# flash4242/Promptable-Counterfactual-GAN

Hardware: AMD Instinct MI355X
Metric: images/sec (G+D step) MNIST-28 cDCGAN bs512 @1/2/4/8 MI355X; % MFMA roofline (higher is better)
Workload: dtype f32

## Files before the change

include/pcgan_hip.h:

```cpp
#ifndef PCGAN_HIP_H
#define PCGAN_HIP_H

#include <stddef.h>
#include <stdint.h>

#ifdef __cplusplus
extern "C" {
#endif

typedef void* pcg_stream_t;

typedef enum pcg_status {
  PCG_OK = 0,
  PCG_ERR_INVALID = -1,
  PCG_ERR_WORKSPACE = -2,
  PCG_ERR_LAUNCH = -3,
  PCG_ERR_UNSUPPORTED = -4
} pcg_status;

typedef enum pcg_act {
  PCG_ACT_NONE = 0,
  PCG_ACT_RELU = 1,
  PCG_ACT_LRELU = 2,
  PCG_ACT_TANH = 3,
// ... 408 lines not shown
  int32_t B;
  const float* const* w_stored;
  const float* a1; const float* a2; const float* a3; const float* a4;
  float* dx;
} pcg_house_cls_bwd_args;
int pcg_house_classifier_fwd(const pcg_house_cls_fwd_args* args, const pcg_sn_bwd_batch* rider , pcg_stream_t stream);
int pcg_house_classifier_bwd(const pcg_house_cls_bwd_args* args, const pcg_sn_fwd_batch* rider , pcg_stream_t stream);

typedef struct pcg_house_cf_eval_args {
  int64_t N; int32_t T, group, clamp_cls, mask_rows;
  const float* g_flat; int32_t nG;
  const float* bn_mean[10]; const float* bn_var[10];
  float bn_eps, tau, res_scale;
  int32_t col_src[17];
  const float* norm_vals;
  const float* const* c_w_kmajor; const float* const* c_bias;
  const float* x; const int64_t* y;
  const int64_t* target; const float* mask; const float* noise;
  float* cont; float* logits; int32_t* chosen;
  float* masked; float* x_cf; float* x_cf_raw;
  float* logits_cf; float* logits_x;
  int64_t* pred_cf; int64_t* pred_x;
  float* gain;
  float* tile_sums; float* class_sums; float* class_counts;
} pcg_house_cf_eval_args;
int pcg_house_cf_eval(const pcg_house_g_desc* desc, const pcg_house_cf_eval_args* args, pcg_stream_t stream);

enum { PCG_MASK_SHARED = 0,
       PCG_MASK_PER_ROW = 1,
       PCG_MASK_PER_QUERY = 2 };

typedef struct pcg_patch_mask_bits_args {
  const uint64_t* bits;
  float* mask;
  int32_t n, H, W, ps;
} pcg_patch_mask_bits_args;
int pcg_patch_mask_bits(const pcg_patch_mask_bits_args* args, pcg_stream_t stream);

typedef struct pcg_mnist_cf_entry_args {
  const float* x;
  const float* table;
  const float* mask;
  const int64_t* target;
  float* out;
  int32_t B, T, HW, K, mask_mode, q0, nq;
} pcg_mnist_cf_entry_args;
int pcg_mnist_cf_entry(const pcg_mnist_cf_entry_args* args, pcg_stream_t stream);

typedef struct pcg_mnist_cf_tail_args {
  const float* c;
  const float* x;
  const float* mask;
  float* x_cf;
  float* raw; float* masked;
  float* sums;
  float scale;
  int32_t B, T, HW, mask_mode, q0, nq;
} pcg_mnist_cf_tail_args;
int pcg_mnist_cf_tail(const pcg_mnist_cf_tail_args* args, pcg_stream_t stream);

#define PCG_MNIST_CF_GROUP_SUMS 8
typedef struct pcg_mnist_cf_score_args {
  const float* logits_cf;
  const float* logits_orig;
  const int64_t* target;
  const int64_t* y_true;
  const float* tail_sums;
  int64_t* pred; float* conf; float* p_target; float* p_true; float* p_orig_true; float* flip;
  float* group_sums;
  int32_t B, T, K, ld, group_rows, q0, nq;
} pcg_mnist_cf_score_args;
int pcg_mnist_cf_score(const pcg_mnist_cf_score_args* args, pcg_stream_t stream);

int pcg_house_losses(const float* d_real, const float* d_fake, const float* d_fake_g, int64_t n, const float* g_cls, const float* am,
                     const float* pen, float lambda_cls, float w_reg, float lambda_mask, float w_reg_log, float* out5, pcg_stream_t stream);

typedef struct pcg_house_res_fwd_args {
  const float* cont; int32_t ncont;
  const float* samples; const int32_t* seg_dev; int32_t T;
  const float* norm; const float* x; const float* mask;
  const int32_t* col_src;
  int32_t D, B;
  float* res; float* masked; float* x_cf; float* partial512; int32_t* ticket; float* pen_out; float* am_out;
} pcg_house_res_fwd_args;
typedef struct pcg_house_res_bwd_args {
  const float* res; const float* masked; const float* mask; const float* gx_a; const float* gx_b;
  float w_pen, w_am;
  int32_t ncont; const int32_t* cont_idx_dev; const int32_t* seg_dev; int32_t S, T;
  const int32_t* cat_idx_dev; const float* norm;
  int32_t D, B;
  float* dcont; float* dsamples;
} pcg_house_res_bwd_args;
typedef struct pcg_house_loss_args {
  const float* d_real; const float* d_fake; const float* d_fake_g; int32_t n;
  const float* g_cls;
  const float* am; const float* pen;
  float lambda_cls, w_reg, lambda_mask, w_reg_log;
  const float* ce_row_loss;
  int32_t n_ce;
  float* out6;
} pcg_house_loss_args;
typedef struct pcg_house_diag_args {
  const float* logits_cf; const float* logits_orig;
  const int64_t* src_rows;
  const int64_t* target_y; const float* masked;
  int32_t B, nc, D;
  float eps;
  float* out4;
  double* acc;
} pcg_house_diag_args;
int pcg_house_residual_fwd(const pcg_house_res_fwd_args* args, const pcg_sn_fwd_batch* rider , pcg_stream_t stream);
int pcg_house_residual_bwd(const pcg_house_res_bwd_args* args, const pcg_house_loss_args* losses ,
                           const pcg_house_diag_args* diag , pcg_stream_t stream);
int pcg_house_diag(const pcg_house_diag_args* args, pcg_stream_t stream);
int pcg_house_draws(int64_t* target_y, int32_t B, int32_t num_classes, const int64_t* y, uint64_t offset_target, float* mask, int32_t D,
                    const int32_t* zero_cols, int32_t n_zero_cols, uint64_t offset_mask, float* noise, int32_t T, uint64_t offset_noise,
                    uint64_t seed, float* onehot_target, float* onehot_y, pcg_stream_t stream);
int pcg_house_draws_counter(int64_t* target_y, int32_t B, int32_t num_classes, const int64_t* y, float* mask, int32_t D,
                            const int32_t* zero_cols, int32_t n_zero_cols, float* noise, int32_t T, uint64_t seed, float* onehot_target,
                            float* onehot_y, uint64_t* counter, pcg_stream_t stream);
int pcg_house_batch_draws_counter(int64_t* target_y, int32_t B, int32_t num_classes, const float* X, const int64_t* Y,
                                  const int64_t* perm, int64_t n_perm, int64_t n_rows, float* x_out, int64_t* y_out,
                                  int64_t* src_out , float* mask, int32_t D, const int32_t* zero_cols, int32_t n_zero_cols,
                                  float* noise, int32_t T, uint64_t seed, float* onehot_target , float* onehot_y ,
                                  uint64_t* counter, pcg_stream_t stream);

int pcg_dp_barrier(pcg_stream_t stream);
int32_t pcg_dp_rccl_version(void);

#define PCG_DP_UNIQUE_ID_BYTES 128
int pcg_dp_unique_id(void* id_out );
int pcg_dp_init(const void* id , int32_t rank, int32_t world);
int32_t pcg_dp_world(void);
int32_t pcg_dp_rank(void);
pcg_stream_t pcg_dp_side_stream(void);
int pcg_dp_allreduce(float* buf, int64_t n, pcg_stream_t stream);
int pcg_dp_allreduce_begin(float* buf, int64_t n, int32_t slot, pcg_stream_t producer_stream);
int pcg_dp_record(int32_t slot);
int pcg_dp_allreduce_wait(int32_t slot, pcg_stream_t consumer_stream);
int pcg_dp_allreduce_sum_f64(double* buf, int64_t n, pcg_stream_t stream);
int pcg_dp_broadcast(void* buf, int64_t nbytes, int32_t root, pcg_stream_t stream);
int pcg_dp_sync_batchnorm(int32_t enable);
int pcg_dp_shutdown(void);

int pcg_tune_set(const char* name, int32_t value);

int pcg_conv_plan_describe(const pcg_conv_geom* g, int32_t op, int32_t assume_scratch, char* out, size_t out_bytes);
size_t pcg_conv_scratch_parts_bytes(void);
size_t pcg_conv_scratch_arrivals_bytes(void);
int pcg_conv_set_scratch(pcg_stream_t stream, void* parts, size_t parts_bytes, void* arrivals, size_t arrivals_bytes);
int pcg_conv_reset_scratch(pcg_stream_t stream);
size_t pcg_conv_pixtab_bytes(const pcg_conv_geom* g);
int pcg_conv_pixtab_register(const pcg_conv_geom* g, void* host_out, size_t bytes, const void* device_table);
int pcg_debug_stamp_buffer(void* buf, int64_t bytes);

typedef struct pcg_moons_cf_desc {
  int32_t hidden, clf_hidden, B, N;
  int32_t nG, nD, nC, nG_adam, nD_adam;
  int32_t g_off[14], d_off[8], c_off[6];
  double lr_G, lr_D, beta1, beta2, adam_eps;
  float bn_eps, bn_momentum, sn_eps, slope;
  float lambda_cls, lambda_l1, lambda_l2, lambda_mask;
} pcg_moons_cf_desc;

typedef struct pcg_moons_cf_train_args {
  const float* X; const int64_t* Y;
  const int64_t* rows;
  const int64_t* target_y;
  const float* mask;
  float* g_flat; float* d_flat; const float* c_flat;
  float* g_exp_avg; float* g_exp_avg_sq; int64_t* g_step;
  float* d_exp_avg; float* d_exp_avg_sq; int64_t* d_step;
  float* bn_mean[3]; float* bn_var[3]; int64_t* bn_nbt[3];
  float* sn_u[4]; float* sn_v[4];
  float* logs;
  float* scratch; size_t scratch_bytes;
} pcg_moons_cf_train_args;

size_t pcg_moons_cf_scratch_bytes(const pcg_moons_cf_desc* desc, int32_t forward);
int pcg_moons_cf_train_steps(const pcg_moons_cf_desc* desc, const pcg_moons_cf_train_args* args, int32_t n_steps, pcg_stream_t stream);

typedef struct pcg_moons_cf_fwd_args {
  int32_t which, train, B;
  const float* x; const float* onehot; const float* mask;
  float* params;
  float* bn_mean[3]; float* bn_var[3]; int64_t* bn_nbt[3];
  float* sn_u[4]; float* sn_v[4];
  float* out0; float* out1;
  float* scratch; size_t scratch_bytes;
} pcg_moons_cf_fwd_args;
int pcg_moons_cf_forward(const pcg_moons_cf_desc* desc, const pcg_moons_cf_fwd_args* args, pcg_stream_t stream);

typedef struct pcg_moons_cf_eval_args {
  int64_t N; int32_t M, T, group;
  const float* x; const int64_t* y;
  const float* masks;
  const int64_t* target; const float* row_mask;
  const float* g_flat; const float* c_flat;
  const float* bn_mean[3]; const float* bn_var[3];
  float* raw; float* masked; float* x_cf;
  float* logits_cf; float* logits_x;
  int64_t* pred_cf; int64_t* pred_x;
  float* gain;
  float* sums;
} pcg_moons_cf_eval_args;
int pcg_moons_cf_eval(const pcg_moons_cf_desc* desc, const pcg_moons_cf_eval_args* args, pcg_stream_t stream);

typedef struct {
  const float* gamma;
  const float* beta;
  float* running_mean;
  float* running_var;
  int64_t* num_batches_tracked;
  float* save_mean;
  float* save_invstd;
  float* xhat;
  float eps;
  float momentum;
  int32_t training;
} pcg_dense_bn;
typedef struct {
  const float* xhat;
  const float* gamma;
  const float* invstd;
  float* dgamma;
  float* dbeta;
  int32_t accumulate;
} pcg_dense_bn_bwd;
int pcg_dense_rows_fwd(const float* x, const float* W, const float* bias , int32_t R, int32_t I, int32_t O,
                       const pcg_dense_bn* bn , int act, float slope, float* y, pcg_stream_t stream);
int pcg_dense_rows_dgrad(const float* dz, const float* W, int32_t R, int32_t O, int32_t I, int below_act, float below_slope,
                         const float* y_below , const pcg_dense_bn_bwd* bn , float* dx,
                         pcg_stream_t stream);
int pcg_dense_rows_wgrad(const float* dz, const float* x, int32_t R, int32_t O, int32_t I, float* dW, float* db ,
                         int accumulate, pcg_stream_t stream);

typedef struct pcg_moons_gan_desc {
  int32_t hidden, z_dim, label_dim, B, N;
  int32_t nG, nD, nG_adam, nD_adam;
  int32_t g_off[4], d_off[4];
  double lr_G, lr_D, beta1, beta2, adam_eps;
} pcg_moons_gan_desc;

typedef struct pcg_moons_gan_train_args {
  const float* X; const int64_t* Y;
  const int64_t* rows;
  const float* z;
  const int64_t* labels;
  float* g_flat; float* d_flat;
  float* g_exp_avg; float* g_exp_avg_sq; int64_t* g_step;
  float* d_exp_avg; float* d_exp_avg_sq; int64_t* d_step;
  float* logs;
  float* scratch; size_t scratch_bytes;
} pcg_moons_gan_train_args;

size_t pcg_moons_gan_scratch_bytes(const pcg_moons_gan_desc* desc);
int pcg_moons_gan_train_steps(const pcg_moons_gan_desc* desc, const pcg_moons_gan_train_args* args, int32_t n_steps, pcg_stream_t stream);

typedef struct pcg_moons_gan_fwd_args {
  int32_t which; int64_t R;
  const float* x; const float* onehot; const float* params;
  float* out;
} pcg_moons_gan_fwd_args;
int pcg_moons_gan_forward(const pcg_moons_gan_desc* desc, const pcg_moons_gan_fwd_args* args, pcg_stream_t stream);

int32_t pcg_calib_mfma_blocks(int32_t rounds);
size_t pcg_calib_mfma_workspace_bytes(int32_t rounds);
int pcg_calib_mfma(int32_t iters, int32_t rounds, void* workspace, size_t workspace_bytes, double* flop_out ,
                   uint64_t** stamps_out , pcg_stream_t stream);
int pcg_calib_copy(const void* src, void* dst, int64_t nbytes, pcg_stream_t stream);

#ifdef __cplusplus
}
#endif
#endif
```

promptable-counterfactual-gan_amd/_lib.py:

```python
import ctypes
import os

import torch

_HERE = os.path.dirname(os.path.abspath(__file__))
LIB_PATH = os.environ.get("PCG_LIB") or os.path.join(_HERE, "libpcgan_hip.so")

PCG_OK = 0
ACT_NONE, ACT_RELU, ACT_LRELU, ACT_TANH, ACT_SIGMOID = 0, 1, 2, 3, 4


class PcgError(RuntimeError):
    pass


class ConvGeom(ctypes.Structure):

    _fields_ = [(n, ctypes.c_int32) for n in ("B", "IH", "IW", "Cin", "OH", "OW", "Cout", "KH", "KW", "stride", "pad")]

    def key(self):
        return tuple(getattr(self, n) for n, _ in self._fields_)


_I, _P = ctypes.c_int32, ctypes.c_void_p
# ... 45 lines not shown


class MoonsCfFwdArgs(ctypes.Structure):
    _fields_ = ([(n, _I) for n in ("which", "train", "B")] + [(n, _P) for n in ("x", "onehot", "mask", "params")] +
                [("bn_mean", _P * 3), ("bn_var", _P * 3), ("bn_nbt", _P * 3), ("sn_u", _P * 4), ("sn_v", _P * 4)] +
                [("out0", _P), ("out1", _P), ("scratch", _P), ("scratch_bytes", ctypes.c_size_t)])


class MoonsCfEvalArgs(ctypes.Structure):
    _fields_ = ([("N", ctypes.c_int64), ("M", _I), ("T", _I), ("group", _I)] +
                [(n, _P) for n in ("x", "y", "masks", "target", "row_mask", "g_flat", "c_flat")] + [("bn_mean", _P * 3), ("bn_var", _P * 3)] +
                [(n, _P) for n in ("raw", "masked", "x_cf", "logits_cf", "logits_x", "pred_cf", "pred_x", "gain", "sums")])


class HouseCfEvalArgs(ctypes.Structure):
    _fields_ = ([("N", ctypes.c_int64)] + [(n, _I) for n in ("T", "group", "clamp_cls", "mask_rows")] + [("g_flat", _P), ("nG", _I)] +
                [("bn_mean", _P * 10), ("bn_var", _P * 10)] + [(n, ctypes.c_float) for n in ("bn_eps", "tau", "res_scale")] +
                [("col_src", _I * 17), ("norm_vals", _P), ("c_w_kmajor", ctypes.POINTER(ctypes.c_void_p)), ("c_bias", ctypes.POINTER(ctypes.c_void_p))] +
                [(n, _P) for n in ("x", "y", "target", "mask", "noise", "cont", "logits", "chosen", "masked", "x_cf", "x_cf_raw", "logits_cf",
                                   "logits_x", "pred_cf", "pred_x", "gain", "tile_sums", "class_sums", "class_counts")])


class PatchMaskBitsArgs(ctypes.Structure):
    _fields_ = [("bits", _P), ("mask", _P)] + [(n, _I) for n in ("n", "H", "W", "ps")]


class MnistCfEntryArgs(ctypes.Structure):
    _fields_ = [(n, _P) for n in ("x", "table", "mask", "target", "out")] + [(n, _I) for n in ("B", "T", "HW", "K", "mask_mode", "q0", "nq")]


class MnistCfTailArgs(ctypes.Structure):
    _fields_ = ([(n, _P) for n in ("c", "x", "mask", "x_cf", "raw", "masked", "sums")] + [("scale", ctypes.c_float)] +
                [(n, _I) for n in ("B", "T", "HW", "mask_mode", "q0", "nq")])


class MnistCfScoreArgs(ctypes.Structure):
    _fields_ = ([(n, _P) for n in ("logits_cf", "logits_orig", "target", "y_true", "tail_sums", "pred", "conf", "p_target", "p_true",
                                   "p_orig_true", "flip", "group_sums")] + [(n, _I) for n in ("B", "T", "K", "ld", "group_rows", "q0", "nq")])


MASK_SHARED, MASK_PER_ROW, MASK_PER_QUERY = 0, 1, 2
MNIST_CF_GROUP_SUMS = 8


class MoonsGanDesc(ctypes.Structure):
    _fields_ = ([(n, _I) for n in ("hidden", "z_dim", "label_dim", "B", "N", "nG", "nD", "nG_adam", "nD_adam")] +
                [("g_off", _I * 4), ("d_off", _I * 4)] + [(n, ctypes.c_double) for n in ("lr_G", "lr_D", "beta1", "beta2", "adam_eps")])


class MoonsGanTrainArgs(ctypes.Structure):
    _fields_ = ([(n, _P) for n in ("X", "Y", "rows", "z", "labels", "g_flat", "d_flat", "g_exp_avg", "g_exp_avg_sq", "g_step",
                                   "d_exp_avg", "d_exp_avg_sq", "d_step", "logs", "scratch")] + [("scratch_bytes", ctypes.c_size_t)])


class MoonsGanFwdArgs(ctypes.Structure):
    _fields_ = [("which", _I), ("R", ctypes.c_int64)] + [(n, _P) for n in ("x", "onehot", "params", "out")]


class DenseBn(ctypes.Structure):
    _fields_ = ([(n, _P) for n in ("gamma", "beta", "running_mean", "running_var", "num_batches_tracked", "save_mean", "save_invstd", "xhat")] +
                [("eps", ctypes.c_float), ("momentum", ctypes.c_float), ("training", _I)])


class DenseBnBwd(ctypes.Structure):
    _fields_ = [(n, _P) for n in ("xhat", "gamma", "invstd", "dgamma", "dbeta")] + [("accumulate", _I)]


_PP, _PI, _F = ctypes.POINTER(ctypes.c_void_p), ctypes.POINTER(ctypes.c_int32), ctypes.c_float


class SnFwdBatch(ctypes.Structure):
    _fields_ = ([("n", _I), ("reps", _I), ("power_iteration", _I), ("eps", _F), ("w_orig", _PP), ("out_features", _PI), ("in_features", _PI)] +
                [(n, _PP) for n in ("u", "v", "w_bar", "sigma", "u_used", "v_used")])


class SnBwdBatch(ctypes.Structure):
    _fields_ = [("n", _I), ("passes", _I), ("dw_bar", _PP), ("w_bar", _PP), ("out_features", _PI), ("in_features", _PI), ("u", _PP), ("v", _PP),
                ("sigma", _PP), ("dw_orig", _PP), ("accumulate", _PI), ("db_dst", _PP), ("db_src", _PP)]


class HouseCriticFwdArgs(ctypes.Structure):
    _fields_ = ([(n, _I) for n in ("n_pass", "B", "D", "NC")] + [("slope", _F)] +
                [(n, _PP) for n in ("x", "onehot", "w_bar", "bias", "a0", "a1", "a2", "a3", "out")])


class HouseCriticBwdArgs(ctypes.Structure):
    _fields_ = ([(n, _I) for n in ("n_pass", "B", "D")] + [("slope", _F)] +
                [(n, _PP) for n in ("dout", "w_bar", "a1", "a2", "a3", "d3", "d2", "d1", "dx")])


class HouseClsFwdArgs(ctypes.Structure):
    _fields_ = ([("x", _P), ("B", _I), ("w_kmajor", _PP), ("bias", _PP)] + [(n, _P) for n in ("a1", "a2", "a3", "a4", "logits", "ce_target")] +
                [("ce_grad_scale", _F), ("ce_dlogits", _P), ("ce_row_loss", _P)])


class HouseClsBwdArgs(ctypes.Structure):
    _fields_ = [("dlogits", _P), ("B", _I), ("w_stored", _PP)] + [(n, _P) for n in ("a1", "a2", "a3", "a4", "dx")]


class HouseResFwdArgs(ctypes.Structure):
    _fields_ = ([("cont", _P), ("ncont", _I), ("samples", _P), ("seg_dev", _P), ("T", _I), ("norm", _P), ("x", _P), ("mask", _P), ("col_src", _PI),
                 ("D", _I), ("B", _I)] + [(n, _P) for n in ("res", "masked", "x_cf", "partial512", "ticket", "pen_out", "am_out")])


class HouseResBwdArgs(ctypes.Structure):
    _fields_ = ([(n, _P) for n in ("res", "masked", "mask", "gx_a", "gx_b")] + [("w_pen", _F), ("w_am", _F), ("ncont", _I), ("cont_idx_dev", _P),
                ("seg_dev", _P), ("S", _I), ("T", _I), ("cat_idx_dev", _P), ("norm", _P), ("D", _I), ("B", _I), ("dcont", _P), ("dsamples", _P)])


class HouseLossArgs(ctypes.Structure):
    _fields_ = ([("d_real", _P), ("d_fake", _P), ("d_fake_g", _P), ("n", _I), ("g_cls", _P), ("am", _P), ("pen", _P)] +
                [(n, _F) for n in ("lambda_cls", "w_reg", "lambda_mask", "w_reg_log")] + [("ce_row_loss", _P), ("n_ce", _I), ("out6", _P)])


class HouseDiagArgs(ctypes.Structure):
    _fields_ = ([(n, _P) for n in ("logits_cf", "logits_orig", "src_rows", "target_y", "masked")] + [("B", _I), ("nc", _I), ("D", _I), ("eps", _F),
                ("out4", _P), ("acc", _P)])


STRUCTS = {"pcg_conv_geom": ConvGeom, "pcg_in_xform": InXform, "pcg_wgrad_item": WgradItem, "pcg_sn_fwd_batch": SnFwdBatch,
           "pcg_sn_bwd_batch": SnBwdBatch, "pcg_house_g_desc": HouseGDesc, "pcg_house_g_fwd_args": HouseGFwdArgs,
           "pcg_house_g_bwd_args": HouseGBwdArgs, "pcg_house_critic_fwd_args": HouseCriticFwdArgs,
           "pcg_house_critic_bwd_args": HouseCriticBwdArgs, "pcg_house_cls_fwd_args": HouseClsFwdArgs, "pcg_house_cls_bwd_args": HouseClsBwdArgs,
           "pcg_house_res_fwd_args": HouseResFwdArgs, "pcg_house_res_bwd_args": HouseResBwdArgs, "pcg_house_loss_args": HouseLossArgs,
           "pcg_house_diag_args": HouseDiagArgs, "pcg_moons_cf_desc": MoonsCfDesc, "pcg_moons_cf_train_args": MoonsCfTrainArgs,
           "pcg_moons_cf_fwd_args": MoonsCfFwdArgs, "pcg_moons_cf_eval_args": MoonsCfEvalArgs,
           "pcg_house_cf_eval_args": HouseCfEvalArgs, "pcg_patch_mask_bits_args": PatchMaskBitsArgs,
           "pcg_mnist_cf_entry_args": MnistCfEntryArgs, "pcg_mnist_cf_tail_args": MnistCfTailArgs,
           "pcg_mnist_cf_score_args": MnistCfScoreArgs, "pcg_dense_bn": DenseBn,
           "pcg_dense_bn_bwd": DenseBnBwd, "pcg_moons_gan_desc": MoonsGanDesc, "pcg_moons_gan_train_args": MoonsGanTrainArgs,
           "pcg_moons_gan_fwd_args": MoonsGanFwdArgs}

_c = ctypes
_vp, _f, _i, _i64, _sz = _c.c_void_p, _c.c_float, _c.c_int, _c.c_int64, _c.c_size_t
_d = _c.c_double
_i32 = _c.c_int32
_gp = _c.POINTER(ConvGeom)
_xp = _c.POINTER(InXform)

PROTOTYPES = {
    "pcg_abi_version": (_i, []),
    "pcg_abi_struct_bytes": (_sz, [_c.c_char_p]),
    "pcg_last_error": (_c.c_char_p, []),
    "pcg_target_arch": (_c.c_char_p, []),
    "pcg_tune_set": (_i, [_c.c_char_p, _i32]),
    "pcg_debug_stamp_buffer": (_i, [_vp, _i64]),
    "pcg_conv_plan_describe": (_i, [_c.POINTER(ConvGeom), _i32, _i32, _c.c_char_p, _sz]),
    "pcg_conv_scratch_parts_bytes": (_sz, []),
    "pcg_conv_scratch_arrivals_bytes": (_sz, []),
    "pcg_conv_set_scratch": (_i, [_vp, _vp, _sz, _vp, _sz]),
    "pcg_conv_reset_scratch": (_i, [_vp]),
    "pcg_conv_pixtab_bytes": (_sz, [_gp]),
    "pcg_conv_pixtab_register": (_i, [_gp, _vp, _sz, _vp]),
    "pcg_conv2d_fwd_bn_g": (_i, [_gp, _vp, _vp, _vp, _vp, _f, _f, _vp, _vp, _vp, _vp, _vp, _i32, _vp, _sz, _vp]),
    "pcg_bn_apply_act_g": (_i, [_vp, _i64, _i32, _vp, _vp, _vp, _vp, _i, _f, _vp, _i32, _vp]),
    "pcg_conv2d_dgrad_bn_phases": (_i32, [_gp]),
    "pcg_conv2d_dgrad_bnbwd_g": (_i, [_gp, _vp, _vp, _vp, _vp, _vp, _vp, _vp, _i, _f, _vp, _vp, _sz, _i32, _vp]),
    "pcg_bn_bwd_partial_g_workspace_bytes": (_sz, [_i32, _i32]),
    "pcg_bn_bwd_partial_g": (_i, [_vp, _vp, _i64, _i32, _vp, _vp, _vp, _vp, _i32, _i32, _vp, _vp, _vp, _i, _i32, _vp, _sz, _vp]),
    "pcg_bn_act_bwd_g_workspace_bytes": (_sz, [_i64, _i32, _i32]),
    "pcg_bn_act_bwd_premask_g": (_i, [_vp, _vp, _i64, _i32, _vp, _vp, _vp, _vp, _i, _f, _vp, _vp, _vp, _i, _i32, _vp, _sz, _vp]),
    "pcg_bce_pair": (_i, [_vp, _i64, _f, _f, _vp, _vp, _vp, _vp, _vp, _vp]),
    "pcg_conv2d_fwd_bnbwd_thin_ok": (_i32, [_gp]),
    "pcg_conv2d_fwd_bnbwd_thin_workspace_bytes": (_sz, [_gp]),
    "pcg_conv2d_fwd_bnbwd_thin": (_i, [_gp, _vp, _vp, _vp, _vp, _vp, _vp, _vp, _i, _f, _vp, _vp, _vp, _i, _vp, _sz, _vp]),
    "pcg_conv2d_bnin_full_ok": (_i32, [_gp, _i32]),
    "pcg_conv2d_fwd_bnin_full": (_i, [_gp, _vp, _vp, _vp, _vp, _vp, _i, _f, _i32, _vp, _vp, _i, _f, _vp, _vp]),
    "pcg_conv2d_wgrad_bnin_full": (_i, [_gp, _vp, _vp, _vp, _vp, _vp, _i, _f, _i32, _vp, _vp, _i, _vp, _sz, _vp]),
    "pcg_conv_precision_set": (_i, [_i32]),
    "pcg_conv_precision_get": (_i32, []),
    "pcg_slab_defer_begin": (_i, [_vp]),
    "pcg_slab_defer_flush": (_i, [_vp]),
    "pcg_slab_defer_pending": (_i32, []),
    "pcg_conv2d_dgrad_bnbwd_full_ok": (_i32, [_gp, _i32]),
    "pcg_conv2d_dgrad_bnbwd_full_workspace_bytes": (_sz, [_gp, _i32]),
    "pcg_conv2d_dgrad_bnbwd_full": (_i, [_gp, _vp, _vp, _vp, _vp, _vp, _vp, _vp, _i, _f, _vp, _vp, _vp, _i, _i32, _vp, _sz, _vp]),
    "pcg_calib_mfma_blocks": (_i32, [_i32]),
    "pcg_calib_mfma_workspace_bytes": (_sz, [_i32]),
    "pcg_calib_mfma": (_i, [_i32, _i32, _vp, _sz, _c.POINTER(_d), _c.POINTER(_c.c_uint64), _vp]),
    "pcg_calib_copy": (_i, [_vp, _vp, _i64, _vp]),
    "pcg_conv2d_fwd_workspace_bytes": (_sz, [_gp]),
    "pcg_conv2d_dgrad_workspace_bytes": (_sz, [_gp]),
    "pcg_conv2d_fwd": (_i, [_gp, _vp, _vp, _vp, _vp, _vp, _sz, _vp]),
    "pcg_conv2d_dgrad": (_i, [_gp, _vp, _vp, _vp, _vp, _vp, _sz, _vp]),
    "pcg_conv2d_fwd_act": (_i, [_gp, _vp, _vp, _vp, _i, _f, _vp, _vp, _sz, _vp]),
    "pcg_conv2d_dgrad_act": (_i, [_gp, _vp, _vp, _vp, _i, _f, _vp, _vp, _sz, _vp]),
    "pcg_conv2d_fwd_bn_workspace_bytes": (_sz, [_gp]),
    "pcg_conv2d_dgrad_bn_workspace_bytes": (_sz, [_gp]),
    "pcg_conv2d_fwd_bn": (_i, [_gp, _vp, _vp, _vp, _vp, _f, _f, _vp, _vp, _vp, _vp, _vp, _vp, _sz, _vp]),
    "pcg_conv2d_dgrad_bn": (_i, [_gp, _vp, _vp, _vp, _vp, _f, _f, _vp, _vp, _vp, _vp, _vp, _vp, _sz, _vp]),
    "pcg_conv2d_dgrad_mask": (_i, [_gp, _vp, _vp, _vp, _i, _f, _vp, _vp, _sz, _vp]),
    "pcg_conv2d_dgrad_mask_thin_ok": (_i32, [_gp]),
    "pcg_conv2d_xf_thin_ok": (_i32, [_gp]),
    "pcg_conv2d_fwd_add_mask": (_i, [_gp, _vp, _vp, _vp, _vp, _i, _f, _vp, _vp]),
    "pcg_conv2d_dgrad_add_mask": (_i, [_gp, _vp, _vp, _vp, _vp, _i, _f, _vp, _vp]),
    "pcg_conv2d_fwd_mask": (_i, [_gp, _vp, _vp, _vp, _i, _f, _vp, _vp, _sz, _vp]),
    "pcg_conv2d_dgrad_bnbwd": (_i, [_gp, _vp, _vp, _vp, _vp, _vp, _vp, _vp, _i, _f, _vp, _vp, _sz, _vp]),
    "pcg_conv2d_fwd_bnbwd": (_i, [_gp, _vp, _vp, _vp, _vp, _vp, _vp, _vp, _i, _f, _vp, _vp, _sz, _vp]),
    "pcg_conv2d_dgrad_add": (_i, [_gp, _vp, _vp, _vp, _vp, _vp, _sz, _vp]),
    "pcg_conv2d_fwd_bn_partial_rows": (_c.c_int32, [_gp]),
    "pcg_conv2d_dgrad_bn_partial_rows": (_c.c_int32, [_gp]),
    "pcg_bn_bwd_partial_workspace_bytes": (_sz, [_c.c_int32]),
    "pcg_bn_bwd_partial": (_i, [_vp, _vp, _i64, _c.c_int32, _vp, _vp, _vp, _vp, _c.c_int32, _vp, _vp, _vp, _i, _vp, _sz, _vp]),
    "pcg_conv2d_fwd_bn_xf": (_i, [_gp, _vp, _xp, _vp, _vp, _vp, _f, _f, _vp, _vp, _vp, _vp, _vp, _vp, _vp, _vp, _vp, _sz, _vp]),
    "pcg_conv2d_dgrad_bn_xf": (_i, [_gp, _vp, _xp, _vp, _vp, _vp, _f, _f, _vp, _vp, _vp, _vp, _vp, _vp, _vp, _vp, _vp, _sz, _vp]),
    "pcg_conv2d_fwd_xf": (_i, [_gp, _vp, _xp, _vp, _vp, _i, _f, _vp, _vp, _sz, _vp]),
    "pcg_conv2d_dgrad_xf": (_i, [_gp, _vp, _xp, _vp, _vp, _i, _f, _vp, _vp, _sz, _vp]),
    "pcg_conv2d_wgrad_xf": (_i, [_gp, _vp, _xp, _vp, _xp, _vp, _i, _vp, _sz, _vp]),
    "pcg_bn_train_stats_coef": (_i, [_vp, _i64, _c.c_int32, _f, _f, _vp, _vp, _vp, _vp, _vp, _vp, _vp, _vp, _vp, _sz, _vp]),
    "pcg_bn_db_workspace_bytes": (_sz, [_i64, _c.c_int32]),
    "pcg_bn_act_bwd_db": (_i, [_vp, _vp, _vp, _i64, _c.c_int32, _vp, _vp, _vp, _vp, _i, _f, _f, _vp, _vp, _vp, _i, _vp, _i, _vp, _sz, _vp]),
    "pcg_bn_bwd_partial_db_workspace_bytes": (_sz, [_c.c_int32]),
    "pcg_bn_bwd_partial_db": (_i, [_vp, _vp, _i64, _c.c_int32, _vp, _vp, _vp, _vp, _c.c_int32, _f, _vp, _vp, _vp, _i, _vp, _i, _vp, _sz, _vp]),
    "pcg_conv2d_dgrad_add_bnsum": (_i, [_gp, _vp, _vp, _vp, _vp, _vp, _vp, _f, _vp, _vp, _sz, _vp]),
    "pcg_conv2d_fwd_add": (_i, [_gp, _vp, _vp, _vp, _vp, _vp, _sz, _vp]),
    "pcg_conv2d_fwd_add_bnsum": (_i, [_gp, _vp, _vp, _vp, _vp, _vp, _vp, _f, _vp, _vp, _sz, _vp]),
    "pcg_conv_weight_adjoint": (_i, [_vp, _vp, _i32, _i32, _i32, _i32, _vp]),
    "pcg_conv_weight_adjoint_many": (_i, [_vp, _vp, _i32, _i32, _i32, _i32, _i32, _vp]),
    "pcg_house_losses": (_i, [_vp, _vp, _vp, _i64, _vp, _vp, _vp, _f, _f, _f, _f, _vp, _vp]),
    "pcg_dp_unique_id": (_i, [_vp]),
    "pcg_dp_init": (_i, [_vp, _i32, _i32]),
    "pcg_dp_world": (_i32, []),
    "pcg_dp_rank": (_i32, []),
    "pcg_dp_side_stream": (_vp, []),
    "pcg_dp_allreduce": (_i, [_vp, _i64, _vp]),
    "pcg_dp_allreduce_begin": (_i, [_vp, _i64, _i32, _vp]),
    "pcg_dp_record": (_i, [_i32]),
    "pcg_dp_allreduce_wait": (_i, [_i32, _vp]),
    "pcg_dp_allreduce_sum_f64": (_i, [_vp, _i64, _vp]),
    "pcg_dp_broadcast": (_i, [_vp, _i64, _i32, _vp]),
    "pcg_dp_sync_batchnorm": (_i, [_i32]),
    "pcg_dp_barrier": (_i, [_vp]),
    "pcg_dp_rccl_version": (_i32, []),
    "pcg_dp_shutdown": (_i, []),
    "pcg_conv2d_wgrad_workspace_bytes": (_sz, [_gp]),
    "pcg_conv2d_wgrad": (_i, [_gp, _vp, _vp, _vp, _i, _vp, _sz, _vp]),
    "pcg_colsum_workspace_bytes": (_sz, [_i64, _c.c_int32]),
    "pcg_colsum": (_i, [_vp, _i64, _c.c_int32, _vp, _i, _vp, _sz, _vp]),
    "pcg_bn_workspace_bytes": (_sz, [_i64, _c.c_int32]),
    "pcg_bn_train_stats": (_i, [_vp, _i64, _c.c_int32, _f, _f, _vp, _vp, _vp, _vp, _vp, _vp, _sz, _vp]),
    "pcg_bn_apply_act": (_i, [_vp, _i64, _c.c_int32, _vp, _vp, _f, _vp, _vp, _i, _f, _vp, _f, _vp, _vp]),
    "pcg_bn_act_bwd": (_i, [_vp, _vp, _vp, _i64, _c.c_int32, _vp, _vp, _vp, _i, _f, _f, _vp, _vp, _vp, _i, _vp, _sz, _vp]),
    "pcg_bn_act_bwd_premask": (_i, [_vp, _vp, _i64, _c.c_int32, _vp, _vp, _vp, _vp, _i, _f, _f, _vp, _vp, _vp, _i, _vp, _sz, _vp]),
    "pcg_embed_concat_fwd": (_i, [_vp, _vp, _vp, _vp, _vp, _c.c_int32, _c.c_int32, _c.c_int32, _c.c_int32, _vp]),
    "pcg_embed_concat_bwd": (_i, [_vp, _vp, _vp, _vp, _c.c_int32, _c.c_int32, _c.c_int32, _c.c_int32, _i, _vp]),
    "pcg_embed_table_grad": (_i, [_vp, _vp, _vp, _i32, _i32, _i32, _i32, _i32, _i, _vp]),
    "pcg_gather_channel": (_i, [_vp, _vp, _i32, _i32, _i32, _vp]),
    "pcg_axpby": (_i, [_vp, _f, _vp, _f, _vp, _i64, _vp]),
    "pcg_scale_mask_fwd": (_i, [_vp, _vp, _f, _vp, _vp, _i64, _vp]),
    "pcg_scale_mask_bwd": (_i, [_vp, _vp, _vp, _f, _vp, _i64, _vp]),
    "pcg_clamp_add_fwd": (_i, [_vp, _vp, _f, _f, _vp, _i64, _vp]),
    "pcg_clamp_add_bwd": (_i, [_vp, _vp, _vp, _f, _f, _vp, _i64, _vp]),
    "pcg_abs_mean_workspace_bytes": (_sz, []),
    "pcg_abs_mean_fwd": (_i, [_vp, _vp, _i, _i64, _vp, _vp, _sz, _vp]),
    "pcg_abs_mean_bwd": (_i, [_vp, _vp, _i, _i64, _vp, _f, _vp, _i, _vp]),
    "pcg_avgpool_fwd": (_i, [_vp, _vp, _c.c_int32, _c.c_int32, _c.c_int32, _vp]),
    "pcg_avgpool_bwd": (_i, [_vp, _vp, _c.c_int32, _c.c_int32, _c.c_int32, _vp]),
    "pcg_cross_entropy_fwd_bwd": (_i, [_vp, _vp, _c.c_int32, _c.c_int32, _f, _vp, _vp, _vp, _vp]),
    "pcg_act_fwd": (_i, [_vp, _i64, _i, _f, _vp, _vp]),
    "pcg_act_bwd": (_i, [_vp, _vp, _i64, _i, _f, _vp, _vp]),
    "pcg_bce_fwd_bwd": (_i, [_vp, _vp, _f, _i64, _f, _vp, _vp, _vp, _vp]),
    "pcg_bce_logits_fwd_bwd": (_i, [_vp, _f, _i64, _f, _vp, _vp, _vp, _vp]),
    "pcg_adam_step": (_i, [_vp, _vp, _vp, _vp, _i64, _d, _d, _d, _d, _d, _i, _i64, _vp]),
    "pcg_adam_step_capturable": (_i, [_vp, _vp, _vp, _vp, _i64, _d, _d, _d, _d, _d, _i, _vp, _vp, _vp]),
    "pcg_patch_mask": (_i, [_vp, _c.c_int32, _c.c_int32, _c.c_int32, _c.c_int32, _c.c_int32, _c.c_uint64, _c.c_uint64, _vp]),
    "pcg_randint": (_i, [_vp, _i64, _c.c_int32, _c.c_int32, _vp, _c.c_uint64, _c.c_uint64, _vp]),
    "pcg_randn": (_i, [_vp, _i64, _f, _f, _c.c_uint64, _c.c_uint64, _vp]),
    "pcg_fill": (_i, [_vp, _i64, _f, _vp]),
    "pcg_add_bias_rows": (_i, [_vp, _i64, _i32, _vp, _vp]),
    "pcg_sumsq": (_i, [_vp, _i64, _vp, _i, _vp]),
    "pcg_norm_sum": (_i, [_vp, _vp, _i32, _vp, _vp]),
    "pcg_instnorm_fwd": (_i, [_vp, _i32, _i32, _i32, _vp, _vp, _f, _i, _f, _vp, _vp, _vp, _vp]),
    "pcg_instnorm_bwd": (_i, [_vp, _vp, _i32, _i32, _i32, _vp, _vp, _vp, _vp, _vp, _vp, _vp]),
    "pcg_instnorm_bwd_bwd": (_i, [_vp, _vp, _vp, _i32, _i32, _i32, _vp, _vp, _vp, _vp, _vp, _vp, _vp]),
    "pcg_instnorm_bwd_fused": (_i, [_vp, _vp, _f, _vp, _i32, _i32, _i32, _vp, _vp, _vp, _vp, _vp, _vp, _vp, _vp, _vp, _vp]),
    "pcg_instnorm_bwd_bwd_act": (_i, [_vp, _vp, _vp, _i32, _i32, _i32, _vp, _vp, _vp, _vp, _f, _vp, _vp, _vp, _vp]),
    "pcg_rowsum3": (_i, [_i32, _vp, _vp, _i, _vp, _vp, _i, _vp, _vp, _i, _i32, _i32, _vp]),
    "pcg_nhwc_to_nchw_flat": (_i, [_vp, _vp, _i32, _i32, _i32, _i, _vp]),
    "pcg_interpolate": (_i, [_vp, _vp, _vp, _vp, _i32, _i32, _vp]),
    "pcg_interpolate_stack": (_i, [_vp, _vp, _vp, _vp, _i32, _i32, _vp]),
    "pcg_gradient_penalty_fwd": (_i, [_vp, _i32, _i32, _f, _vp, _vp, _vp]),
    "pcg_gradient_penalty_bwd": (_i, [_vp, _vp, _vp, _i32, _i32, _f, _vp, _vp]),
    "pcg_rand_uniform": (_i, [_vp, _i64, _c.c_uint64, _c.c_uint64, _vp]),
    "pcg_cross_entropy_weighted_fwd_bwd": (_i, [_vp, _vp, _vp, _i32, _i32, _f, _vp, _vp, _vp, _vp]),
    "pcg_dropout_apply": (_i, [_vp, _vp, _i64, _i32, _i32, _f, _vp, _vp]),
    "pcg_rand_bernoulli": (_i, [_vp, _i64, _f, _c.c_uint64, _c.c_uint64, _vp]),
    "pcg_resize8_normalize": (_i, [_vp, _i32, _i32, _i32, _i32, _i32, _vp, _vp, _i32, _vp, _vp, _i32, _f, _f, _vp, _vp]),
    "pcg_house_g_fwd": (_i, [_c.POINTER(HouseGDesc), _c.POINTER(HouseGFwdArgs), _vp]),
    "pcg_house_g_bwd": (_i, [_c.POINTER(HouseGDesc), _c.POINTER(HouseGBwdArgs), _vp]),
    "pcg_weighted_sum_fwd": (_i, [_i32, _vp, _vp, _vp, _vp]),
    "pcg_weighted_sum_bwd": (_i, [_i32, _vp, _vp, _vp, _vp]),
    "pcg_cf_metrics": (_i, [_vp, _vp, _vp, _vp, _i32, _i32, _vp, _vp]),
    "pcg_gemm": (_i, [_i, _i, _i32, _i32, _i32, _vp, _i32, _vp, _i32, _vp, _i32, _vp, _i, _vp]),
    "pcg_linear_wgrad_workspace_bytes": (_sz, [_i32, _i32, _i32]),
    "pcg_linear_wgrad_ticket_count": (_i32, []),
    "pcg_linear_wgrad": (_i, [_vp, _i32, _vp, _i32, _i32, _i32, _i32, _vp, _vp, _i, _i, _vp, _sz, _vp, _vp]),
    "pcg_spectral_norm_fwd_batched": (_i, [_c.POINTER(SnFwdBatch), _vp]),
    "pcg_spectral_norm_bwd_batched": (_i, [_c.POINTER(SnBwdBatch), _vp]),
    "pcg_house_critic_fwd": (_i, [_c.POINTER(HouseCriticFwdArgs), _vp]),
    "pcg_house_critic_bwd": (_i, [_c.POINTER(HouseCriticBwdArgs), _vp]),
    "pcg_house_classifier_fwd": (_i, [_c.POINTER(HouseClsFwdArgs), _c.POINTER(SnBwdBatch), _vp]),
    "pcg_house_classifier_bwd": (_i, [_c.POINTER(HouseClsBwdArgs), _c.POINTER(SnFwdBatch), _vp]),
    "pcg_house_cf_eval": (_i, [_c.POINTER(HouseGDesc), _c.POINTER(HouseCfEvalArgs), _vp]),
    "pcg_patch_mask_bits": (_i, [_c.POINTER(PatchMaskBitsArgs), _vp]),
    "pcg_mnist_cf_entry": (_i, [_c.POINTER(MnistCfEntryArgs), _vp]),
    "pcg_mnist_cf_tail": (_i, [_c.POINTER(MnistCfTailArgs), _vp]),
# ... 75 lines not shown
```

promptable-counterfactual-gan_amd/csrc/conv_igemm.hip:

```cpp
#include <string.h>
#include <mutex>
#include "conv_loaders.h"
#include "conv_pixtab.h"
#include "thin_conv.h"

namespace pcg {
namespace {

__device__ __forceinline__ int wave_id() { return __builtin_amdgcn_readfirstlane((int)(threadIdx.x >> 6)); }

__device__ __forceinline__ void prio_entry(const ConvP& p) { if (p.edge_prio & 1) __builtin_amdgcn_s_setprio(3); }
__device__ __forceinline__ void prio_epilogue(const ConvP& p) { if (p.edge_prio & 2) __builtin_amdgcn_s_setprio(3); }

__device__ __forceinline__ int epi_group_off(const ConvP& p, int m_block) {
  return p.epi.group_rows > 0 ? __builtin_amdgcn_readfirstlane(m_block / p.epi.group_rows) * p.N : 0;
}

template <class Cfg, bool XF>
__global__ void __launch_bounds__(IG_THREADS, Cfg::MINW) conv_fwd_kernel(ConvP p) {
  extern __shared__ __attribute__((aligned(16))) float smem[];
  prio_entry(p);
  const uint32_t tile = xcd_remap(blockIdx.x, gridDim.x);
  const int mt = tile / p.tilesN, nt = tile % p.tilesN;
  const int m_block = mt * Cfg::BM, n_block = nt * Cfg::BN;
  const int kt_begin = blockIdx.y * p.ktiles_per_split;
  int ktiles = p.ktiles - kt_begin;
  if (ktiles > p.ktiles_per_split) ktiles = p.ktiles_per_split;

  if (wave_id() >= 4) {
    const int tid = threadIdx.x - IG_LOADERS;
    FwdALoader<Cfg::BM, XF> la(p, m_block, tid);
    FwdBLoader<Cfg::BN> lb(p, n_block, tid);
    if (kt_begin) { la.seek(kt_begin); lb.seek(kt_begin); }
    igemm_produce<Cfg>(la, lb, ktiles, smem, tid, ClockStamp{p.stamps, p.stamp_slots});
    return;
  }
  f32x16 acc[Cfg::TM][Cfg::TN];
  ClockStamp cs{p.stamps, p.stamp_slots};
  cs.phase(0);
  igemm_consume<Cfg, true, true>(ktiles, acc, smem, cs);
  prio_epilogue(p);
  float* out = p.out + (size_t)blockIdx.y * (size_t)p.M * (size_t)p.N;
#ifdef PCG_ABL_NO_EPILOGUE
  if (acc[0][0][0] == 12345.678f) out[0] = acc[0][0][1];
  return;
#endif
  igemm_store_tile<Cfg>(acc, smem, n_block, p.N, blockIdx.y == 0 ? p.bias : nullptr, [&](int row) -> float* {
    const int m = m_block + row;
    return m < p.M ? out + (size_t)m * p.N + n_block : nullptr;
  }, p.stat_partial ? p.stat_partial + (size_t)mt * Cfg::WAVES_M * 2 * p.N : nullptr, p.act, p.slope, &p.epi, epi_group_off(p, m_block));
  cs.phase(3);
}

template <class Cfg, bool XF>
__global__ void __launch_bounds__(IG_THREADS, Cfg::MINW) conv_dgrad_kernel(ConvP p, DgradPhases phases) {
  extern __shared__ __attribute__((aligned(16))) float smem[];
  __shared__ int rowpix[Cfg::BM];
  prio_entry(p);
  uint32_t bx = blockIdx.x, py = blockIdx.y;
  if (phases.interleave) {
    const uint32_t l = xcd_remap(blockIdx.x, gridDim.x);
    py = l % (uint32_t)phases.interleave; bx = l / (uint32_t)phases.interleave;
  }
  const PhaseInfo& f = phases.p[py];
  const int tilesM = (f.Mp + Cfg::BM - 1) / Cfg::BM;
  const uint32_t ntiles = (uint32_t)tilesM * p.tilesN;
  if (bx >= ntiles) return;
  const uint32_t tile = phases.interleave ? bx : xcd_remap(bx, ntiles);
  const int mt = tile / p.tilesN, nt = tile % p.tilesN;
  const int m_block = mt * Cfg::BM, n_block = nt * Cfg::BN;
  const int ktiles = f.nth * f.ntw * ((p.Cout + IG_BK - 1) / IG_BK);

  if (wave_id() >= 4) {
    const int tid = threadIdx.x - IG_LOADERS;
    for (int r = tid; r < Cfg::BM; r += IG_LOADERS) {
      const int m = m_block + r;
      int pix = -1;
      if (m < f.Mp) {
        uint32_t t, cc, b, aa;
        f.dPHw.divmod((uint32_t)m, t, cc);
        f.dPHh.divmod(t, b, aa);
        pix = ((int)b * p.IH + (int)aa * p.stride + f.ph) * p.IW + (int)cc * p.stride + f.pw;
      }
      rowpix[r] = pix;
    }
    DgradALoader<Cfg::BM, XF> la(p, f, m_block, tid);
    DgradBLoader<Cfg::BN> lb(p, f, n_block, tid);
    igemm_produce<Cfg>(la, lb, ktiles, smem, tid, ClockStamp{p.stamps, p.stamp_slots});
    return;
  }
  f32x16 acc[Cfg::TM][Cfg::TN];
  ClockStamp cs{p.stamps, p.stamp_slots};
  cs.phase(0);
  igemm_consume<Cfg, true, false>(ktiles, acc, smem, cs);
  prio_epilogue(p);
  igemm_store_tile<Cfg>(acc, smem, n_block, p.N, p.bias, [&](int row) -> float* {
    const int pix = rowpix[row];
    return pix >= 0 ? p.out + (size_t)pix * p.Cin + n_block : nullptr;
  }, p.stat_partial ? p.stat_partial + (size_t)(f.prow0 + mt * Cfg::WAVES_M) * 2 * p.N : nullptr, p.act, p.slope, &p.epi, epi_group_off(p, m_block));
  cs.phase(3);
}

struct SkPlan {
  int dp_tiles, sk_tiles, sk_blocks, ktiles;
  float* parts;
  int* arrivals;
};
struct SkSeg { int tile, kt_begin, nkt, nparts, first_block; };

__device__ __forceinline__ int sk_start(int g, const SkPlan& sk) {
  return __builtin_amdgcn_readfirstlane((int)((uint32_t)g * (uint32_t)(sk.sk_tiles * sk.ktiles) / (uint32_t)sk.sk_blocks));
}
__device__ __forceinline__ int sk_owner(int x, const SkPlan& sk) {
  return __builtin_amdgcn_readfirstlane((int)((((uint32_t)x + 1u) * (uint32_t)sk.sk_blocks - 1u) / (uint32_t)(sk.sk_tiles * sk.ktiles)));
}
__device__ __forceinline__ int sk_segments(const SkPlan& sk, SkSeg& s0, SkSeg& s1) {
  const int b = blockIdx.x;
  if (b < sk.dp_tiles) { s0 = SkSeg{(int)xcd_remap((uint32_t)b, (uint32_t)sk.dp_tiles), 0, sk.ktiles, 1, 0}; return 1; }
  const int g = (int)xcd_remap((uint32_t)(b - sk.dp_tiles), (uint32_t)sk.sk_blocks), KT = sk.ktiles;
  const int it0 = sk_start(g, sk), it1 = sk_start(g + 1, sk);
  const int j0 = __builtin_amdgcn_readfirstlane(it0 / KT), e0 = it1 < (j0 + 1) * KT ? it1 : (j0 + 1) * KT;
  auto fill = [&](SkSeg& sg, int j, int from, int to) {
    const int f = sk_owner(j * KT, sk), l = sk_owner((j + 1) * KT - 1, sk);
    sg = SkSeg{sk.dp_tiles + j, from - j * KT, to - from, l - f + 1, f};
  };
  fill(s0, j0, it0, e0);
  if (it1 <= e0) return 1;
  fill(s1, j0 + 1, e0, it1);
  return 2;
}
#if defined(__HIP_DEVICE_COMPILE__) && !defined(__gfx950__)
#error "stream-K partial-tile exchange (sc1 stores + relaxed agent-scope counters) is written for gfx950 only"
#endif
__device__ __forceinline__ void sk_store4(rsrc_t r, uint32_t off, float a, float b, float c, float d) {
  const u32x4 v = {__float_as_uint(a), __float_as_uint(b), __float_as_uint(c), __float_as_uint(d)};
  __builtin_amdgcn_raw_buffer_store_b128(v, r, off, 0, 16);
}
__device__ __forceinline__ float4 sk_load4(rsrc_t r, uint32_t off) {
  const u32x4 v = __builtin_amdgcn_raw_buffer_load_b128(r, off, 0, 16);
  return make_float4(__uint_as_float(v.x), __uint_as_float(v.y), __uint_as_float(v.z), __uint_as_float(v.w));
}
template <class Cfg, class FirstOf>
__device__ __forceinline__ bool sk_combine_core(float* parts, int* arrivals, int nblocks, int g, int j, int nparts, int first_block,
                                                FirstOf first_of, f32x16 (&acc)[Cfg::TM][Cfg::TN]) {
  if (nparts == 1) return true;
  constexpr uint32_t TILE_BYTES = Cfg::BM * Cfg::BN * 4;
  auto slot_of = [&](int blk) { return (uint32_t)(2 * blk + (first_of(blk) ? 0 : 1)); };
  const rsrc_t rs = make_rsrc(parts, (uint32_t)(2 * nblocks) * TILE_BYTES);
  const uint32_t toff = threadIdx.x * 16u;
  const uint32_t mine = slot_of(g) * TILE_BYTES + toff;
#pragma unroll
  for (int i = 0; i < Cfg::TM; ++i)
#pragma unroll
    for (int jj = 0; jj < Cfg::TN; ++jj)
#pragma unroll
      for (int q = 0; q < 4; ++q)
        sk_store4(rs, mine + (uint32_t)(((i * Cfg::TN + jj) * 4 + q) * IG_LOADERS * 16),
                  acc[i][jj][4 * q], acc[i][jj][4 * q + 1], acc[i][jj][4 * q + 2], acc[i][jj][4 * q + 3]);
  asm volatile("s_waitcnt vmcnt(0)" ::: "memory");
  int* cnt = arrivals + j * 4 + (int)(threadIdx.x >> 6);
  int old = 0;
  if ((threadIdx.x & 63) == 0) old = __hip_atomic_fetch_add(cnt, 1, __ATOMIC_RELAXED, __HIP_MEMORY_SCOPE_AGENT);
  old = __builtin_amdgcn_readfirstlane(old);
  if (old != nparts - 1) return false;
  if ((threadIdx.x & 63) == 0) __hip_atomic_store(cnt, 0, __ATOMIC_RELAXED, __HIP_MEMORY_SCOPE_AGENT);
#pragma unroll
  for (int i = 0; i < Cfg::TM; ++i)
#pragma unroll
    for (int jj = 0; jj < Cfg::TN; ++jj)
#pragma unroll
      for (int r = 0; r < 16; ++r) acc[i][jj][r] = 0.f;
  for (int k = 0; k < nparts; ++k) {
    const uint32_t src = slot_of(first_block + k) * TILE_BYTES + toff;
#pragma unroll
    for (int i = 0; i < Cfg::TM; ++i)
#pragma unroll
      for (int jj = 0; jj < Cfg::TN; ++jj)
#pragma unroll
        for (int q = 0; q < 4; ++q) {
          const float4 v = sk_load4(rs, src + (uint32_t)(((i * Cfg::TN + jj) * 4 + q) * IG_LOADERS * 16));
          acc[i][jj][4 * q] += v.x; acc[i][jj][4 * q + 1] += v.y; acc[i][jj][4 * q + 2] += v.z; acc[i][jj][4 * q + 3] += v.w;
        }
  }
  return true;
}
template <class Cfg>
__device__ __forceinline__ bool sk_combine(const SkPlan& sk, const SkSeg& sg, f32x16 (&acc)[Cfg::TM][Cfg::TN]) {
  const int g = (int)xcd_remap((uint32_t)((int)blockIdx.x - sk.dp_tiles), (uint32_t)sk.sk_blocks), j = sg.tile - sk.dp_tiles, KT = sk.ktiles;
  return sk_combine_core<Cfg>(sk.parts, sk.arrivals, sk.sk_blocks, g, j, sg.nparts, sg.first_block,
                              [&](int blk) { return sk_start(blk, sk) >= j * KT; }, acc);
}

template <class Cfg, bool XF>
__device__ __forceinline__ void fwd_sk_segment(const ConvP& p, const SkPlan& sk, const SkSeg& sg, float* smem) {
  const int mt = __builtin_amdgcn_readfirstlane(sg.tile / p.tilesN), nt = sg.tile - mt * p.tilesN;
  const int m_block = mt * Cfg::BM, n_block = nt * Cfg::BN;
  if (wave_id() >= 4) {
    const int tid = threadIdx.x - IG_LOADERS;
    FwdALoader<Cfg::BM, XF> la(p, m_block, tid);
    FwdBLoader<Cfg::BN> lb(p, n_block, tid);
    if (sg.kt_begin) { la.seek(sg.kt_begin); lb.seek(sg.kt_begin); }
    igemm_produce<Cfg>(la, lb, sg.nkt, smem, tid, ClockStamp{nullptr, 0});
    return;
  }
  f32x16 acc[Cfg::TM][Cfg::TN];
  igemm_consume<Cfg, true, true>(sg.nkt, acc, smem);
  if (sk_combine<Cfg>(sk, sg, acc))
    igemm_store_tile<Cfg>(acc, smem, n_block, p.N, p.bias, [&](int row) -> float* {
      const int m = m_block + row;
      return m < p.M ? p.out + (size_t)m * p.N + n_block : nullptr;
    }, p.stat_partial ? p.stat_partial + (size_t)mt * Cfg::WAVES_M * 2 * p.N : nullptr, p.act, p.slope, &p.epi, epi_group_off(p, m_block));
}
template <class Cfg, bool XF>
__global__ void __launch_bounds__(IG_THREADS, Cfg::MINW) conv_fwd_sk_kernel(ConvP p, SkPlan sk) {
  extern __shared__ __attribute__((aligned(16))) float smem[];
  SkSeg s0, s1{};
  const int nseg = sk_segments(sk, s0, s1);
  fwd_sk_segment<Cfg, XF>(p, sk, s0, smem);
  if (nseg == 1) return;
  lds_barrier();
  fwd_sk_segment<Cfg, XF>(p, sk, s1, smem);
}

template <class Cfg, bool XF>
__device__ __forceinline__ void dgrad_sk_segment(const ConvP& p, const DgradPhases& phases, const SkPlan& sk, const SkSeg& sg, int tiles_per_phase,
                                                 float* smem, int* rowpix) {
  const int py = __builtin_amdgcn_readfirstlane(sg.tile / tiles_per_phase), tile = sg.tile - py * tiles_per_phase;
  const PhaseInfo& f = phases.p[py];
  const int mt = __builtin_amdgcn_readfirstlane(tile / p.tilesN), nt = tile - mt * p.tilesN;
  const int m_block = mt * Cfg::BM, n_block = nt * Cfg::BN;
  if (wave_id() >= 4) {
    const int tid = threadIdx.x - IG_LOADERS;
    for (int r = tid; r < Cfg::BM; r += IG_LOADERS) {
      const int m = m_block + r;
      int pix = -1;
      if (m < f.Mp) {
        uint32_t t, cc, b, aa;
        f.dPHw.divmod((uint32_t)m, t, cc);
        f.dPHh.divmod(t, b, aa);
        pix = ((int)b * p.IH + (int)aa * p.stride + f.ph) * p.IW + (int)cc * p.stride + f.pw;
      }
      rowpix[r] = pix;
    }
    DgradALoader<Cfg::BM, XF> la(p, f, m_block, tid);
    DgradBLoader<Cfg::BN> lb(p, f, n_block, tid);
    if (sg.kt_begin) { la.seek(sg.kt_begin); lb.seek(sg.kt_begin); }
    igemm_produce<Cfg>(la, lb, sg.nkt, smem, tid, ClockStamp{nullptr, 0});
    return;
  }
  f32x16 acc[Cfg::TM][Cfg::TN];
  igemm_consume<Cfg, true, false>(sg.nkt, acc, smem);
  if (sk_combine<Cfg>(sk, sg, acc))
    igemm_store_tile<Cfg>(acc, smem, n_block, p.N, p.bias, [&](int row) -> float* {
      const int pix = rowpix[row];
      return pix >= 0 ? p.out + (size_t)pix * p.Cin + n_block : nullptr;
    }, p.stat_partial ? p.stat_partial + (size_t)(f.prow0 + mt * Cfg::WAVES_M) * 2 * p.N : nullptr, p.act, p.slope, &p.epi, epi_group_off(p, m_block));
}
template <class Cfg, bool XF>
__global__ void __launch_bounds__(IG_THREADS, Cfg::MINW) conv_dgrad_sk_kernel(ConvP p, DgradPhases phases, SkPlan sk, int tiles_per_phase) {
  extern __shared__ __attribute__((aligned(16))) float smem[];
  __shared__ int rowpix[Cfg::BM];
  SkSeg s0, s1{};
  const int nseg = sk_segments(sk, s0, s1);
  dgrad_sk_segment<Cfg, XF>(p, phases, sk, s0, tiles_per_phase, smem, rowpix);
  if (nseg == 1) return;
  lds_barrier();
  dgrad_sk_segment<Cfg, XF>(p, phases, sk, s1, tiles_per_phase, smem, rowpix);
}

template <class Cfg, bool XFA, bool XFB, bool TAB = false>
__global__ void __launch_bounds__(IG_THREADS, 4) conv_wgrad_kernel(ConvP p, int ktiles_total, int ktiles_per_split, int tiles,
                                                                   int slice_major) {
  extern __shared__ __attribute__((aligned(16))) float smem[];
  prio_entry(p);
  uint32_t tile, split;
  if (slice_major) {
    const uint32_t l = xcd_remap(blockIdx.x, gridDim.x);
    split = l / (uint32_t)tiles; tile = l - split * (uint32_t)tiles;
  } else {
    tile = xcd_remap(blockIdx.x, gridDim.x); split = blockIdx.y;
  }
  const int mt = tile / p.tilesN, nt = tile % p.tilesN;
  const int m_block = mt * Cfg::BM, n_block = nt * Cfg::BN;
  const int kt_begin = split * ktiles_per_split;
  int ktiles = ktiles_total - kt_begin;
  if (ktiles > ktiles_per_split) ktiles = ktiles_per_split;

  if (wave_id() >= 4) {
    const int tid = threadIdx.x - IG_LOADERS;
    WgradALoader<Cfg::BM, XFA> la(p, m_block, kt_begin, tid);
    WgradBLoader<Cfg::BN, XFB, TAB> lb(p, n_block, kt_begin, tid);
    igemm_produce<Cfg>(la, lb, ktiles, smem, tid, ClockStamp{p.stamps, p.stamp_slots});
    return;
  }
  f32x16 acc[Cfg::TM][Cfg::TN];
  igemm_consume<Cfg, false, false>(ktiles, acc, smem, ClockStamp{p.stamps, p.stamp_slots});
  prio_epilogue(p);
  float* slab = p.out + (size_t)split * (size_t)p.M * (size_t)p.N;
  igemm_store_tile<Cfg>(acc, smem, n_block, p.N, nullptr, [&](int row) -> float* {
    const int m = m_block + row;
    return m < p.M ? slab + (size_t)m * p.N + n_block : nullptr;
  });
}


struct SkNPlan {
  int nph, blocks, total;
  int tile0[5], it0[5], kt[4];
  float* parts; int* arrivals;
};
__device__ __forceinline__ int skn_start(int g, const SkNPlan& sk) {
  return __builtin_amdgcn_readfirstlane((int)((uint32_t)g * (uint32_t)sk.total / (uint32_t)sk.blocks));
}
__device__ __forceinline__ int skn_owner(int x, const SkNPlan& sk) {
  return __builtin_amdgcn_readfirstlane((int)((((uint32_t)x + 1u) * (uint32_t)sk.blocks - 1u) / (uint32_t)sk.total));
}
struct SkNSeg { int py, tin, t_begin, e, kt_begin, nkt, fb, nparts, mt, nt; };
__device__ __forceinline__ SkNSeg skn_segment(int it, int it1, const SkNPlan& sk, int tilesN) {
  SkNSeg s;
  s.py = 0;
  if (sk.nph > 1 && it >= sk.it0[1]) s.py = 1;
  if (sk.nph > 2 && it >= sk.it0[2]) s.py = 2;
  if (sk.nph > 3 && it >= sk.it0[3]) s.py = 3;
  const int KT = sk.kt[s.py], local = it - sk.it0[s.py];
  s.tin = __builtin_amdgcn_readfirstlane(local / KT);
  s.t_begin = sk.it0[s.py] + s.tin * KT;
  const int t_end = s.t_begin + KT;
  s.e = it1 < t_end ? it1 : t_end;
  s.kt_begin = it - s.t_begin; s.nkt = s.e - it;
  s.fb = skn_owner(s.t_begin, sk); s.nparts = skn_owner(t_end - 1, sk) - s.fb + 1;
  s.mt = __builtin_amdgcn_readfirstlane(s.tin / tilesN); s.nt = s.tin - s.mt * tilesN;
  return s;
}
template <class Cfg, bool XF>
__global__ void __launch_bounds__(IG_THREADS, Cfg::MINW) conv_dgrad_skn_kernel(ConvP p, DgradPhases phases, SkNPlan sk) {
  extern __shared__ __attribute__((aligned(16))) float smem[];
  __shared__ int rowpix[Cfg::BM];
  const int g = (int)xcd_remap(blockIdx.x, (uint32_t)sk.blocks);
  const int it1 = skn_start(g + 1, sk);
  if (wave_id() >= 4) {
    const int tid = threadIdx.x - IG_LOADERS;
#pragma unroll 1
    for (int it = skn_start(g, sk); it < it1;) {
      const SkNSeg sg = skn_segment(it, it1, sk, p.tilesN);
      const PhaseInfo& f = phases.p[sg.py];
      const int m_block = sg.mt * Cfg::BM, n_block = sg.nt * Cfg::BN;
      for (int r = tid; r < Cfg::BM; r += IG_LOADERS) {
        const int m = m_block + r;
        int pix = -1;
        if (m < f.Mp) {
          uint32_t t, cc, b, aa;
          f.dPHw.divmod((uint32_t)m, t, cc);
          f.dPHh.divmod(t, b, aa);
          pix = ((int)b * p.IH + (int)aa * p.stride + f.ph) * p.IW + (int)cc * p.stride + f.pw;
        }
        rowpix[r] = pix;
      }
      DgradALoader<Cfg::BM, XF> la(p, f, m_block, tid);
      DgradBLoader<Cfg::BN> lb(p, f, n_block, tid);
      if (sg.kt_begin) { la.seek(sg.kt_begin); lb.seek(sg.kt_begin); }
      igemm_produce<Cfg>(la, lb, sg.nkt, smem, tid, ClockStamp{nullptr, 0});
      it = sg.e;
      if (it < it1) lds_barrier();
    }
    return;
  }
#pragma unroll 1
  for (int it = skn_start(g, sk); it < it1;) {
    const SkNSeg sg = skn_segment(it, it1, sk, p.tilesN);
    const PhaseInfo& f = phases.p[sg.py];
    const int m_block = sg.mt * Cfg::BM, n_block = sg.nt * Cfg::BN;
    {
      f32x16 acc[Cfg::TM][Cfg::TN];
      igemm_consume<Cfg, true, false>(sg.nkt, acc, smem);
      const int t_begin = sg.t_begin;
      if (sk_combine_core<Cfg>(sk.parts, sk.arrivals, sk.blocks, g, sk.tile0[sg.py] + sg.tin, sg.nparts, sg.fb,
                               [&](int blk) { return skn_start(blk, sk) >= t_begin; }, acc))
        igemm_store_tile<Cfg>(acc, smem, n_block, p.N, p.bias, [&](int row) -> float* {
          const int pix = rowpix[row];
          return pix >= 0 ? p.out + (size_t)pix * p.Cin + n_block : nullptr;
        }, p.stat_partial ? p.stat_partial + (size_t)(f.prow0 + sg.mt * Cfg::WAVES_M) * 2 * p.N : nullptr, p.act, p.slope, &p.epi, epi_group_off(p, m_block));
    }
    it = sg.e;
    if (it < it1) lds_barrier();
  }
}

template <class Cfg, bool XFA, bool XFB, bool TAB>
__device__ __forceinline__ void wgrad_sk_segment(const ConvP& p, const SkPlan& sk, const SkSeg& sg, float* smem) {
  const int mt = __builtin_amdgcn_readfirstlane(sg.tile / p.tilesN), nt = sg.tile - mt * p.tilesN;
  const int m_block = mt * Cfg::BM, n_block = nt * Cfg::BN;
  if (wave_id() >= 4) {
    const int tid = threadIdx.x - IG_LOADERS;
    WgradALoader<Cfg::BM, XFA> la(p, m_block, sg.kt_begin, tid);
    WgradBLoader<Cfg::BN, XFB, TAB> lb(p, n_block, sg.kt_begin, tid);
    igemm_produce<Cfg>(la, lb, sg.nkt, smem, tid, ClockStamp{nullptr, 0});
    return;
  }
  f32x16 acc[Cfg::TM][Cfg::TN];
  igemm_consume<Cfg, false, false>(sg.nkt, acc, smem);
  if (sk_combine<Cfg>(sk, sg, acc))
    igemm_store_tile<Cfg>(acc, smem, n_block, p.N, nullptr, [&](int row) -> float* {
      const int m = m_block + row;
      return m < p.M ? p.out + (size_t)m * p.N + n_block : nullptr;
    }, nullptr, PCG_ACT_NONE, 0.f, &p.epi);
}
template <class Cfg, bool XFA, bool XFB, bool TAB = false>
__global__ void __launch_bounds__(IG_THREADS, 4) conv_wgrad_sk_kernel(ConvP p, SkPlan sk) {
  extern __shared__ __attribute__((aligned(16))) float smem[];
  SkSeg s0, s1{};
  const int nseg = sk_segments(sk, s0, s1);
  wgrad_sk_segment<Cfg, XFA, XFB, TAB>(p, sk, s0, smem);
  if (nseg == 1) return;
  lds_barrier();
  wgrad_sk_segment<Cfg, XFA, XFB, TAB>(p, sk, s1, smem);
}

using Cfg64x192 = TileCfg<64, 192, 2, 2>;
template <class Cfg, bool TAB = false>
__global__ void __launch_bounds__(IG_THREADS, 4) conv_wgrad192_kernel(ConvP p, int ktiles_total, int ktiles_per_split, int tiles,
                                                                      int slice_major) {
  static_assert(Cfg::BM == 64 && Cfg::BN == 192, "the 192-column weight-gradient tile");
  extern __shared__ __attribute__((aligned(16))) float smem[];
  prio_entry(p);
  uint32_t tile, split;
  if (slice_major) {
    const uint32_t l = xcd_remap(blockIdx.x, gridDim.x);
    split = l / (uint32_t)tiles; tile = l - split * (uint32_t)tiles;
  } else {
    tile = xcd_remap(blockIdx.x, gridDim.x); split = blockIdx.y;
  }
  const int mt = tile / p.tilesN, nt = tile % p.tilesN;
  const int m_block = mt * Cfg::BM, n_block = nt * Cfg::BN;
  const int kt_begin = split * ktiles_per_split;
  int ktiles = ktiles_total - kt_begin;
  if (ktiles > ktiles_per_split) ktiles = ktiles_per_split;
  if (wave_id() >= 4) {
    const int tid = threadIdx.x - IG_LOADERS;
    WgradALoader<Cfg::BM, false> la(p, m_block, kt_begin, tid);
    WgradBLoader192<TAB> lb(p, n_block, kt_begin, tid);
    igemm_produce<Cfg>(la, lb, ktiles, smem, tid);
    return;
  }
  f32x16 acc[Cfg::TM][Cfg::TN];
  igemm_consume<Cfg, false, false>(ktiles, acc, smem, ClockStamp{p.stamps, p.stamp_slots});
  prio_epilogue(p);
  float* slab = p.out + (size_t)split * (size_t)p.M * (size_t)p.N;
  igemm_store_tile<Cfg>(acc, smem, n_block, p.N, nullptr, [&](int row) -> float* {
    const int m = m_block + row;
    return m < p.M ? slab + (size_t)m * p.N + n_block : nullptr;
  });
}

__global__ void __launch_bounds__(256) col2im_kernel(const float4* __restrict__ dcol, float4* __restrict__ dx, const float* __restrict__ bias,
                                                     int B, int IH, int IW, int CQ, int OH, int OW, int KH, int KW, int stride, int pad,
                                                     FastDiv dCQ, FastDiv dIW, FastDiv dIH, int act, float neg) {
  const uint32_t total = (uint32_t)B * IH * IW * CQ;
  for (uint32_t idx = blockIdx.x * 256u + threadIdx.x; idx < total; idx += gridDim.x * 256u) {
    uint32_t pix, cq, t, iw, b, ih;
    dCQ.divmod(idx, pix, cq);
    dIW.divmod(pix, t, iw);
    dIH.divmod(t, b, ih);
    float4 acc = bias ? *reinterpret_cast<const float4*>(bias + 4 * cq) : make_float4(0.f, 0.f, 0.f, 0.f);
    for (int kh = 0; kh < KH; ++kh) {
      const int th = (int)ih + pad - kh;
      if (th < 0 || th % stride) continue;
      const int oh = th / stride;
      if (oh >= OH) continue;
      for (int kw = 0; kw < KW; ++kw) {
        const int tw = (int)iw + pad - kw;
        if (tw < 0 || tw % stride) continue;
        const int ow = tw / stride;
        if (ow >= OW) continue;
        const float4 v = dcol[((size_t)(((int)b * OH + oh) * OW + ow) * (KH * KW) + (kh * KW + kw)) * CQ + cq];
        acc.x += v.x; acc.y += v.y; acc.z += v.z; acc.w += v.w;
      }
    }
    if (act != PCG_ACT_NONE) {
      acc.x = act_neg_scale(acc.x, neg); acc.y = act_neg_scale(acc.y, neg); acc.z = act_neg_scale(acc.z, neg); acc.w = act_neg_scale(acc.w, neg);
    }
    dx[idx] = acc;
  }
}

using Cfg128x128 = TileCfg<128, 128, 2, 2>;
#ifndef PCG_TILE64_SWZ
#define PCG_TILE64_SWZ 1
#endif
using Cfg128x64P = TileCfg<128, 64, 2, 2>;
#if PCG_TILE64_SWZ
using Cfg128x64 = TileCfg<128, 64, 2, 2, true, 6, 1>;
#else
using Cfg128x64 = Cfg128x64P;
#endif

template <class C>
using Bf16Twin = TileCfg<C::BM, C::BN, C::WAVES_M, C::WAVES_N, false, C::MINW, C::PF, true>;


int check_geom(const pcg_conv_geom* g) {
  PCG_REQUIRE(g != nullptr, "conv geometry is null");
  PCG_REQUIRE(g->B > 0 && g->IH > 0 && g->IW > 0 && g->Cin > 0 && g->OH > 0 && g->OW > 0 && g->Cout > 0,
              "conv geometry: non-positive extent");
  PCG_REQUIRE(g->KH > 0 && g->KW > 0 && g->stride > 0 && g->pad >= 0, "conv geometry: bad kernel/stride/pad");
  PCG_REQUIRE(g->OH == (g->IH + 2 * g->pad - g->KH) / g->stride + 1 && g->OW == (g->IW + 2 * g->pad - g->KW) / g->stride + 1,
              "conv geometry: OH/OW inconsistent with IH/IW, kernel %dx%d stride %d pad %d", g->KH, g->KW, g->stride, g->pad);
  PCG_REQUIRE((int64_t)g->B * g->IH * g->IW * g->Cin * 4 < (1ll << 31) && (int64_t)g->B * g->OH * g->OW * g->Cout * 4 < (1ll << 31) &&
                  (int64_t)g->Cout * g->KH * g->KW * g->Cin * 4 < (1ll << 31),
              "conv geometry: an operand tensor reaches 2 GiB (32-bit buffer offsets); split the batch");
  PCG_REQUIRE(g->KH * g->KW <= 32, "conv geometry: more than 32 taps (%dx%d) unsupported", g->KH, g->KW);
  return PCG_OK;
}

struct Tune { int edge_prio = -1, dgrad_swz3 = -1, wgrad_rounds = -1, korder = -1, wgrad_order = -1, dgrad_interleave = -1, fwd_splits = -1, stream_k = -1, sk_blocks = -1, dgrad_gemm = -1, t64 = -1, wgrad_pixtab = -1; unsigned long long* stamps = nullptr; int stamp_slots = 0; };
Tune g_tune;

ConvP make_params(const pcg_conv_geom* g) {
  ConvP p{};
  static const int korder_env = getenv("PCG_KORDER") ? atoi(getenv("PCG_KORDER")) : 1;
  p.korder = g_tune.korder >= 0 ? g_tune.korder : korder_env;
  static const int edge_env = getenv("PCG_EDGE_PRIO") ? atoi(getenv("PCG_EDGE_PRIO")) : 2;
  p.edge_prio = g_tune.edge_prio >= 0 ? g_tune.edge_prio : edge_env;
  p.stamps = g_tune.stamps; p.stamp_slots = g_tune.stamp_slots;
  p.B = g->B; p.IH = g->IH; p.IW = g->IW; p.Cin = g->Cin; p.OH = g->OH; p.OW = g->OW; p.Cout = g->Cout;
  p.KH = g->KH; p.KW = g->KW; p.stride = g->stride; p.pad = g->pad;
  p.dOW = FastDiv((uint32_t)g->OW);
  p.dOH = FastDiv((uint32_t)g->OH);
  p.dOHW = FastDiv((uint32_t)(g->OH * g->OW));
  p.x_bytes = (uint32_t)((int64_t)g->B * g->IH * g->IW * g->Cin * 4);
  p.dy_bytes = (uint32_t)((int64_t)g->B * g->OH * g->OW * g->Cout * 4);
  p.w_bytes = (uint32_t)((int64_t)g->Cout * g->KH * g->KW * g->Cin * 4);
  return p;
}

int set_xform(const char* who, const pcg_in_xform* xf, int C, ConvP* p) {
  if (!xf || !xf->scale) return PCG_OK;
  PCG_REQUIRE(xf->shift != nullptr, "%s: input transform without shift", who);
  PCG_REQUIRE(xf->act == PCG_ACT_NONE || xf->act == PCG_ACT_RELU || xf->act == PCG_ACT_LRELU,
              "%s: input transform activation %d is not none / ReLU / LeakyReLU", who, xf->act);
  PCG_REQUIRE(C % 4 == 0 && (((uintptr_t)xf->scale | (uintptr_t)xf->shift) & 15) == 0,
              "%s: input transform needs a channel count %% 4 == 0 and 16-byte aligned scale / shift", who);
  p->in_sc = xf->scale; p->in_sh = xf->shift; p->in_neg = act_neg_of(xf->act, xf->slope); p->in_c_bytes = (uint32_t)C * 4u;
  return PCG_OK;
}

template <class Cfg, bool AK, bool BK_>
constexpr size_t smem_bytes() {
  constexpr int a = igemm_smem_floats<Cfg, AK, BK_>(), b = epilogue_smem_floats<Cfg>();
  return sizeof(float) * (size_t)(a > b ? a : b);
}

template <class K>
int set_smem(K kernel, size_t bytes) {
  hipError_t e = hipFuncSetAttribute(reinterpret_cast<const void*>(kernel), hipFuncAttributeMaxDynamicSharedMemorySize, (int)bytes);
  if (e != hipSuccess) { set_error("hipFuncSetAttribute(max dynamic LDS=%zu): %s", bytes, hipGetErrorString(e)); return PCG_ERR_LAUNCH; }
  return PCG_OK;
}

constexpr int SK_MAX_BLOCKS = 512, SK_MAX_TILES = 4096;
constexpr size_t SK_PARTS_BYTES = (size_t)2 * SK_MAX_BLOCKS * 128 * 128 * sizeof(float);
constexpr size_t SK_ARRIVALS_BYTES = (size_t)SK_MAX_TILES * 4 * sizeof(int);
struct SkScratch { int device; hipStream_t stream; float* parts; int* arrivals; };
SkScratch g_sk_scratch[64];
int g_sk_scratch_n = 0;
std::mutex g_sk_mutex;
int current_device() { int d = 0; return hipGetDevice(&d) == hipSuccess ? d : 0; }
bool sk_scratch_of(hipStream_t s, SkPlan* sk) {
  const int dev = current_device();
  std::lock_guard<std::mutex> lock(g_sk_mutex);
  for (int i = 0; i < g_sk_scratch_n; ++i)
    if (g_sk_scratch[i].stream == s && g_sk_scratch[i].device == dev) {
      if (sk) { sk->parts = g_sk_scratch[i].parts; sk->arrivals = g_sk_scratch[i].arrivals; }
      return true;
    }
  return false;
}
struct PixTabReg { int device, IH, IW, OH, OW, stride, pad, KH, KW, Cin; const uint32_t* tab; };
constexpr int PIXTAB_MAX = 256;
PixTabReg g_pixtab[PIXTAB_MAX];
int g_pixtab_n = 0;
std::mutex g_pixtab_mutex;
bool pixtab_same(const PixTabReg& r, int dev, const pcg_conv_geom* g) {
  return r.device == dev && r.IH == g->IH && r.IW == g->IW && r.OH == g->OH && r.OW == g->OW && r.stride == g->stride && r.pad == g->pad &&
         r.KH == g->KH && r.KW == g->KW && r.Cin == g->Cin;
}
const uint32_t* pixtab_of(const pcg_conv_geom* g) {
  static const int env = getenv("PCG_WGRAD_PIXTAB") ? atoi(getenv("PCG_WGRAD_PIXTAB")) : 1;
  if (!(g_tune.wgrad_pixtab >= 0 ? g_tune.wgrad_pixtab : env)) return nullptr;
  std::lock_guard<std::mutex> lock(g_pixtab_mutex);
  if (g_pixtab_n == 0) return nullptr;
  const int dev = current_device();
  for (int i = 0; i < g_pixtab_n; ++i)
    if (pixtab_same(g_pixtab[i], dev, g)) return g_pixtab[i].tab;
  return nullptr;
}
int sk_mode() {
  static const int env = getenv("PCG_STREAM_K") ? atoi(getenv("PCG_STREAM_K")) : 1;
  return g_tune.stream_k >= 0 ? g_tune.stream_k : env;
}
bool plan_sk_shape(int tiles, int ktiles, SkPlan* sk) {
  const int mode = sk_mode();
  if (mode == 3) {
    sk->dp_tiles = tiles; sk->sk_tiles = 0; sk->sk_blocks = 0; sk->ktiles = ktiles;
    return true;
  }
  if (mode == 0 || ktiles < 8) return false;
  const int dp = tiles / 512 * 512, r = tiles - dp;
  if (r == 0 || r > SK_MAX_TILES || (int64_t)r * ktiles * 512 >= (1ll << 31)) return false;
  const double t_dp = (r <= 256 ? 2.2 : 3.5) * ktiles + 6.0;
  double best = 1e30;
  int bg = 0;
  for (int G = 512; G >= 64; G >>= 1) {
    if (g_tune.sk_blocks > 0 && G != g_tune.sk_blocks) continue;
    if (G < r) break;
    const int it = ceil_div(r * ktiles, G);
    if (it < 4) continue;
    const int parts = ceil_div(ktiles, it) + 1;
    if (parts > 8) continue;
    const double t = it * (G == 512 ? 3.5 : 2.2) + 2 * 12.0 + 3.0 + 1.5 * parts;
    if (t < best) { best = t; bg = G; }
  }
  if (!bg || (mode == 1 && best > 0.9 * t_dp)) return false;
  sk->dp_tiles = dp; sk->sk_tiles = r; sk->sk_blocks = bg; sk->ktiles = ktiles;
  return true;
}
bool plan_sk(int tiles, int ktiles, hipStream_t s, SkPlan* sk) { return plan_sk_shape(tiles, ktiles, sk) && sk_scratch_of(s, sk); }
bool have_sk_scratch() {
  if (sk_mode() == 0) return false;
  const int dev = current_device();
  std::lock_guard<std::mutex> lock(g_sk_mutex);
  for (int i = 0; i < g_sk_scratch_n; ++i) if (g_sk_scratch[i].device == dev) return true;
  return false;
}
int stream_has_sk(hipStream_t s) { return sk_mode() != 0 && sk_scratch_of(s, nullptr) ? 1 : 0; }

template <class Cfg, bool XF>
int launch_fwd_x(ConvP p, int splits, hipStream_t s) {
  p.tilesN = ceil_div(p.N, Cfg::BN);
  const int tilesM = ceil_div(p.M, Cfg::BM);
  constexpr size_t smem = smem_bytes<Cfg, true, true>();
  if constexpr (Cfg::BM == 128 && Cfg::BN == 128) {
    SkPlan sk{};
    if (splits == 1 && plan_sk(tilesM * p.tilesN, p.ktiles, s, &sk)) {
      static int once_sk = set_smem(conv_fwd_sk_kernel<Cfg, XF>, smem);
      if (once_sk != PCG_OK) return once_sk;
      hipLaunchKernelGGL((conv_fwd_sk_kernel<Cfg, XF>), dim3((unsigned)(sk.dp_tiles + sk.sk_blocks)), dim3(IG_THREADS), smem, s, p, sk);
      return launch_status("conv_fwd_sk_kernel");
    }
  }
  static int once = set_smem(conv_fwd_kernel<Cfg, XF>, smem);
  if (once != PCG_OK) return once;
  hipLaunchKernelGGL((conv_fwd_kernel<Cfg, XF>), dim3((unsigned)tilesM * p.tilesN, splits), dim3(IG_THREADS), smem, s, p);
  return launch_status("conv_fwd_kernel");
}
template <class Cfg>
int launch_fwd(const ConvP& p, int splits, hipStream_t s) {
  if (conv_bf16()) return p.in_sc ? launch_fwd_x<Bf16Twin<Cfg>, true>(p, splits, s) : launch_fwd_x<Bf16Twin<Cfg>, false>(p, splits, s);
  return p.in_sc ? launch_fwd_x<Cfg, true>(p, splits, s) : launch_fwd_x<Cfg, false>(p, splits, s);
}

struct FwdPlan { int splits, ktiles_per_split; };
FwdPlan plan_fwd(const pcg_conv_geom* g, int have_sk = -1) {
  if (have_sk < 0) have_sk = have_sk_scratch() ? 1 : 0;
  const int M = g->B * g->OH * g->OW, N = g->Cout;
  const int tiles = ceil_div(M, 128) * ceil_div(N, N > 64 ? 128 : 64);
  const int ktiles = g->KH * g->KW * ceil_div(g->Cin, IG_BK);
  FwdPlan f{1, ktiles};
  if (g_tune.fwd_splits > 0) {
    f.ktiles_per_split = ceil_div(ktiles, g_tune.fwd_splits);
    f.splits = ceil_div(ktiles, f.ktiles_per_split);
    return f;
  }
  if (tiles > 256 && tiles < 448 && ktiles >= 32 && !have_sk) {
    int best = 1;
    double bc = 2.0;
    for (int s = 2; s <= 4; ++s) {
      const double c = (double)ceil_div(tiles * s, 256) / s + 0.1 * s;
      if (c < bc - 1e-9) { bc = c; best = s; }
    }
    f.ktiles_per_split = ceil_div(ktiles, best);
    f.splits = ceil_div(ktiles, f.ktiles_per_split);
    return f;
  }
  if (tiles > 96 || ktiles < 32) return f;
  int splits = ceil_div(tiles >= 48 ? 512 : 384, tiles);
  if (splits > ktiles / 8) splits = ktiles / 8;
  if (splits < 2) return f;
  f.ktiles_per_split = ceil_div(ktiles, splits);
  f.splits = ceil_div(ktiles, f.ktiles_per_split);
  return f;
}

bool plan_skn_shape(const DgradPhases& ph, int nphases, int BM, int tilesN, int Cout, SkNPlan* sn) {
  if (sk_mode() == 0 || nphases < 2) return false;
  sn->nph = nphases;
  bool ok = true;
  int tiles = 0, total = 0, ktmax = 0;
  for (int i = 0; i < nphases && ok; ++i) {
    const int kt = ph.p[i].nth * ph.p[i].ntw * ceil_div(Cout, IG_BK), t = ceil_div(ph.p[i].Mp, BM) * tilesN;
    ok = ph.p[i].nth > 0 && ph.p[i].ntw > 0 && ph.p[i].Mp > 0 && kt > 0;
    sn->tile0[i] = tiles; sn->it0[i] = total; sn->kt[i] = kt;
    tiles += t; total += t * kt;
    if (kt > ktmax) ktmax = kt;
  }
  sn->tile0[nphases] = tiles; sn->it0[nphases] = total;
  int blocks = total / 512 >= 16 ? 512 : 256;
  if (g_tune.sk_blocks > 0) blocks = g_tune.sk_blocks;
  ok = ok && tiles <= SK_MAX_TILES && blocks <= SK_MAX_BLOCKS && total / blocks >= 8 && (int64_t)total * blocks < (1ll << 31) &&
       ktmax <= 8 * (total / blocks) && (sk_mode() == 2 || g_tune.sk_blocks > 0 || total >= 48 * tiles);
  sn->blocks = blocks; sn->total = total;
  return ok;
}

template <class Cfg, bool XF>
int launch_dgrad_x(ConvP p, const DgradPhases& ph, int nphases, int maxMp, hipStream_t s) {
  p.tilesN = ceil_div(p.N, Cfg::BN);
  const int tilesM = ceil_div(maxMp, Cfg::BM);
  constexpr size_t smem = smem_bytes<Cfg, true, false>();
  if constexpr (Cfg::BM == 128 && Cfg::BN == 128) {
    bool uniform = true;
    for (int i = 0; i < nphases; ++i)
      uniform = uniform && ph.p[i].Mp == ph.p[0].Mp && ph.p[i].nth * ph.p[i].ntw == ph.p[0].nth * ph.p[0].ntw && ph.p[i].nth > 0 && ph.p[i].ntw > 0;
    if (!uniform && nphases > 1 && sk_mode() != 0) {
      SkNPlan sn{};
      SkPlan scratch{};
      if (plan_skn_shape(ph, nphases, Cfg::BM, p.tilesN, p.Cout, &sn) && sk_scratch_of(s, &scratch)) {
        sn.parts = scratch.parts; sn.arrivals = scratch.arrivals;
        static int once_sn = set_smem(conv_dgrad_skn_kernel<Cfg, XF>, smem);
        if (once_sn != PCG_OK) return once_sn;
        DgradPhases phs = ph;
        phs.interleave = 0;
        hipLaunchKernelGGL((conv_dgrad_skn_kernel<Cfg, XF>), dim3((unsigned)sn.blocks), dim3(IG_THREADS), smem, s, p, phs, sn);
        return launch_status("conv_dgrad_skn_kernel");
      }
    }
    SkPlan sk{};
    const int tpp = tilesM * p.tilesN;
    if (uniform && plan_sk(tpp * nphases, ph.p[0].nth * ph.p[0].ntw * ceil_div(p.Cout, IG_BK), s, &sk)) {
      static int once_sk = set_smem(conv_dgrad_sk_kernel<Cfg, XF>, smem);
      if (once_sk != PCG_OK) return once_sk;
      DgradPhases phs = ph;
      phs.interleave = 0;
      hipLaunchKernelGGL((conv_dgrad_sk_kernel<Cfg, XF>), dim3((unsigned)(sk.dp_tiles + sk.sk_blocks)), dim3(IG_THREADS), smem, s, p, phs, sk, tpp);
      return launch_status("conv_dgrad_sk_kernel");
    }
  }
  static int once = set_smem(conv_dgrad_kernel<Cfg, XF>, smem);
  if (once != PCG_OK) return once;
  static const int il_env0 = getenv("PCG_DGRAD_INTERLEAVE") ? atoi(getenv("PCG_DGRAD_INTERLEAVE")) : 1;
  const int il_env = g_tune.dgrad_interleave >= 0 ? g_tune.dgrad_interleave : il_env0;
  DgradPhases phl = ph;
  bool same = nphases > 1 && il_env && p.w_bytes <= (1u << 20);
  for (int i = 1; i < nphases; ++i) same = same && ph.p[i].Mp == ph.p[0].Mp;
  phl.interleave = same ? nphases : 0;
  if (same)
    hipLaunchKernelGGL((conv_dgrad_kernel<Cfg, XF>), dim3((unsigned)tilesM * p.tilesN * nphases), dim3(IG_THREADS), smem, s, p, phl);
  else
    hipLaunchKernelGGL((conv_dgrad_kernel<Cfg, XF>), dim3((unsigned)tilesM * p.tilesN, nphases), dim3(IG_THREADS), smem, s, p, phl);
  return launch_status("conv_dgrad_kernel");
}
template <class Cfg>
int launch_dgrad(const ConvP& p, const DgradPhases& ph, int nphases, int maxMp, hipStream_t s) {
  if (conv_bf16())
    return p.in_sc ? launch_dgrad_x<Bf16Twin<Cfg>, true>(p, ph, nphases, maxMp, s) : launch_dgrad_x<Bf16Twin<Cfg>, false>(p, ph, nphases, maxMp, s);
  return p.in_sc ? launch_dgrad_x<Cfg, true>(p, ph, nphases, maxMp, s) : launch_dgrad_x<Cfg, false>(p, ph, nphases, maxMp, s);
}

struct WgradPlan { int splits, ktiles_total, ktiles_per_split, tiles; bool narrow, wide192; };

WgradPlan plan_wgrad(const pcg_conv_geom* g) {
  WgradPlan w{};
  const int M = g->Cout, N = g->KH * g->KW * g->Cin;
  w.narrow = (M <= 64);
  static const int t192_env = getenv("PCG_WGRAD_192") ? atoi(getenv("PCG_WGRAD_192")) : 1;
  w.wide192 = w.narrow && t192_env && N % 192 == 0 && (N % 128) != 0;
  const int BM = w.narrow ? 64 : 128;
  w.tiles = ceil_div(M, BM) * (w.wide192 ? N / 192 : ceil_div(N, 128));
  const int64_t K = (int64_t)g->B * g->OH * g->OW;
  w.ktiles_total = (int)ceil_div64(K, IG_BK);
  const int slots = 512 * (g_tune.wgrad_rounds > 0 ? g_tune.wgrad_rounds : 1);
  int splits = w.tiles <= slots ? slots / w.tiles : 1;
  const int max_splits = w.ktiles_total / 8 > 0 ? w.ktiles_total / 8 : 1;
  if (splits > max_splits) splits = max_splits;
  if (splits < 1) splits = 1;
  auto cost = [&](int s, int* s_eff) {
    const int kps = ceil_div(w.ktiles_total, s), se = ceil_div(w.ktiles_total, kps);
    const int n = ceil_div(w.tiles * se, 256);
    *s_eff = se;
    return (double)n * kps * (w.wide192 ? 1.5 : w.narrow ? 1.0 : 1.95) * (n == 1 ? 1.2 : 1.0) + (double)se * M * N * 8.0 / 4.0e6;
  };
  int se = 0;
  const double c0 = cost(splits, &se);
  double cb = c0;
  int sb = splits;
  for (int s = 1; s <= max_splits && s <= 64; ++s) {
    const double c = cost(s, &se);
    if (se == s && c < cb * 0.98) { cb = c; sb = s; }
  }
  if (cb < 0.95 * c0) splits = sb;
  w.ktiles_per_split = ceil_div(w.ktiles_total, splits);
  w.splits = ceil_div(w.ktiles_total, w.ktiles_per_split);
  return w;
}

}
}

using namespace pcg;

extern "C" size_t pcg_conv2d_fwd_workspace_bytes(const pcg_conv_geom* g) {
  if (check_geom(g) != PCG_OK) return 0;
  if (thin_is_cin(g) || thin_is_cout(g)) return thin_conv_fwd_workspace_bytes(g);
  const FwdPlan f = plan_fwd(g);
  return f.splits > 1 ? (size_t)f.splits * g->B * g->OH * g->OW * g->Cout * sizeof(float) : 0;
}
static bool dgrad_as_gemm(const pcg_conv_geom* g, int have_sk = -1) {
  if (have_sk < 0) have_sk = have_sk_scratch() ? 1 : 0;
  if (thin_is_cin(g) || thin_is_cout(g)) return false;
  if (g_tune.dgrad_gemm == 0) return false;
  if (g_tune.dgrad_gemm < 0 && have_sk && g->stride == 2) {
    int64_t phase_macs = 0;
    for (int a = 0; a < 2; ++a)
      for (int b = 0; b < 2; ++b) {
        const int PHh = a < g->IH ? (g->IH - a + 1) / 2 : 0, PHw = b < g->IW ? (g->IW - b + 1) / 2 : 0;
        const int kh0 = (a + g->pad) % 2, kw0 = (b + g->pad) % 2;
        const int nth = kh0 < g->KH ? (g->KH - kh0 + 1) / 2 : 0, ntw = kw0 < g->KW ? (g->KW - kw0 + 1) / 2 : 0;
        phase_macs += (int64_t)PHh * PHw * nth * ntw;
      }
    if (phase_macs * 20 <= (int64_t)g->OH * g->OW * g->KH * g->KW * 19) return false;
  }
  if (g->stride < 2 || (g->KH % g->stride == 0 && g->KW % g->stride == 0)) return false;
  if (g->Cout < 512 || g->Cin % 4 || g->Cout % 4) return false;
  const int64_t bytes = (int64_t)g->B * g->OH * g->OW * g->KH * g->KW * g->Cin * 4;
  return bytes < (1ll << 31);
}
static size_t dgrad_gemm_bytes(const pcg_conv_geom* g) { return (size_t)g->B * g->OH * g->OW * g->KH * g->KW * g->Cin * sizeof(float); }

extern "C" size_t pcg_conv_scratch_parts_bytes(void) { return pcg::SK_PARTS_BYTES; }
extern "C" size_t pcg_conv_scratch_arrivals_bytes(void) { return pcg::SK_ARRIVALS_BYTES; }
extern "C" int pcg_conv_set_scratch(pcg_stream_t stream, void* parts, size_t parts_bytes, void* arrivals, size_t arrivals_bytes) {
  using namespace pcg;
  hipStream_t s = (hipStream_t)stream;
  const int dev = current_device();
  std::lock_guard<std::mutex> lock(g_sk_mutex);
  int at = -1;
  for (int i = 0; i < g_sk_scratch_n; ++i) if (g_sk_scratch[i].stream == s && g_sk_scratch[i].device == dev) at = i;
  if (!parts) {
    if (at >= 0) g_sk_scratch[at] = g_sk_scratch[--g_sk_scratch_n];
    return PCG_OK;
  }
  PCG_REQUIRE(arrivals != nullptr && parts_bytes >= SK_PARTS_BYTES && arrivals_bytes >= SK_ARRIVALS_BYTES,
              "pcg_conv_set_scratch: parts %zu B (need %zu), arrivals %zu B (need %zu)", parts_bytes, SK_PARTS_BYTES, arrivals_bytes, SK_ARRIVALS_BYTES);
  PCG_REQUIRE((((uintptr_t)parts) & 15) == 0 && (((uintptr_t)arrivals) & 3) == 0, "pcg_conv_set_scratch: misaligned scratch");
  if (at < 0) {
    PCG_REQUIRE(g_sk_scratch_n < 64, "pcg_conv_set_scratch: more than 64 streams with scratch");
    at = g_sk_scratch_n++;
  }
  g_sk_scratch[at] = SkScratch{dev, s, (float*)parts, (int*)arrivals};
  return PCG_OK;
}
extern "C" int pcg_conv_reset_scratch(pcg_stream_t stream) {
  using namespace pcg;
  SkPlan sk{};
  if (!sk_scratch_of((hipStream_t)stream, &sk)) return PCG_OK;
  hipError_t e = hipMemsetAsync(sk.arrivals, 0, SK_ARRIVALS_BYTES, (hipStream_t)stream);
  if (e != hipSuccess) { set_error("pcg_conv_reset_scratch: %s", hipGetErrorString(e)); return PCG_ERR_LAUNCH; }
  return PCG_OK;
}

extern "C" size_t pcg_conv_pixtab_bytes(const pcg_conv_geom* g) {
  if (check_geom(g) != PCG_OK) return 0;
  return pcg::pixtab_entries(g->OH, g->OW) * 2 * sizeof(uint32_t);
}
extern "C" int pcg_conv_pixtab_register(const pcg_conv_geom* g, void* host_out, size_t bytes, const void* device_table) {
  using namespace pcg;
  if (int e = check_geom(g)) return e;
  if (host_out) {
    PCG_REQUIRE(bytes >= pcg_conv_pixtab_bytes(g) && (((uintptr_t)host_out) & 3) == 0, "pcg_conv_pixtab_register: host buffer %zu B (need %zu), 4-byte aligned",
                bytes, pcg_conv_pixtab_bytes(g));
    pixtab_build(g->IH, g->IW, g->OH, g->OW, g->stride, g->pad, g->KH, g->KW, g->Cin, static_cast<uint32_t*>(host_out));
    if (!device_table) return PCG_OK;
  }
  PCG_REQUIRE((((uintptr_t)device_table) & 7) == 0, "pcg_conv_pixtab_register: misaligned table");
  const int dev = current_device();
  std::lock_guard<std::mutex> lock(g_pixtab_mutex);
  int at = -1;
  for (int i = 0; i < g_pixtab_n; ++i) if (pixtab_same(g_pixtab[i], dev, g)) at = i;
  if (!device_table) {
    if (at >= 0) g_pixtab[at] = g_pixtab[--g_pixtab_n];
    return PCG_OK;
  }
  if (at < 0) {
    PCG_REQUIRE(g_pixtab_n < PIXTAB_MAX, "pcg_conv_pixtab_register: more than %d geometries with a table", PIXTAB_MAX);
    at = g_pixtab_n++;
  }
  g_pixtab[at] = PixTabReg{dev, g->IH, g->IW, g->OH, g->OW, g->stride, g->pad, g->KH, g->KW, g->Cin, static_cast<const uint32_t*>(device_table)};
  return PCG_OK;
}

extern "C" size_t pcg_conv2d_dgrad_workspace_bytes(const pcg_conv_geom* g) {
  if (check_geom(g) != PCG_OK) return 0;
  if (thin_is_cin(g) || thin_is_cout(g)) return thin_conv_dgrad_workspace_bytes(g);
  return dgrad_as_gemm(g) ? dgrad_gemm_bytes(g) : 0;
}

namespace pcg {
int launch_bn_stats_finalize(const double* partial, int nparts, int64_t rows, int C, float eps, float momentum, float* save_mean,
                             float* save_invstd, float* running_mean, float* running_var, int64_t* nbt, hipStream_t s,
                             bool has_presum_tail, const float* gamma = nullptr, const float* beta = nullptr, float* coef = nullptr);
size_t bn_partial_buffer_bytes(int nparts, int C);
int launch_bn_stats_finalize_g(const double* partial, int nparts, int nphases, int groups, int64_t rows_per_group, int C, float eps,
// ... 527 lines not shown
  }
  if constexpr (!TAB) {
    if (p.pixtab) return launch_wgrad_sk_x<Cfg, XFA, XFB, true>(p, sk, s);
  }
  constexpr size_t smem = smem_bytes<Cfg, false, false>();
  static int once = set_smem(conv_wgrad_sk_kernel<Cfg, XFA, XFB, TAB>, smem);
  if (once != PCG_OK) return once;
  hipLaunchKernelGGL((conv_wgrad_sk_kernel<Cfg, XFA, XFB, TAB>), dim3((unsigned)(sk.dp_tiles + sk.sk_blocks)), dim3(IG_THREADS), smem, s, p, sk);
  return launch_status("conv_wgrad_sk_kernel");
}
template <class Cfg, bool TAB = false>
static int launch_wgrad192(const ConvP& p, const WgradPlan& wp, int slice_major, hipStream_t s) {
  if constexpr (!TAB) {
    if (p.pixtab) return launch_wgrad192<Cfg, true>(p, wp, slice_major, s);
  }
  constexpr size_t smem = smem_bytes<Cfg, false, false>();
  static int once = set_smem(conv_wgrad192_kernel<Cfg, TAB>, smem);
  if (once != PCG_OK) return once;
  hipLaunchKernelGGL((conv_wgrad192_kernel<Cfg, TAB>), slice_major ? dim3((unsigned)wp.tiles * wp.splits) : dim3((unsigned)wp.tiles, wp.splits),
                     dim3(IG_THREADS), smem, s, p, wp.ktiles_total, wp.ktiles_per_split, wp.tiles, slice_major);
  return launch_status("conv_wgrad192_kernel");
}
template <class Cfg>
static int launch_wgrad(const ConvP& p, const WgradPlan& wp, int slice_major, int xf_side, hipStream_t s) {
  if constexpr (!Cfg::BF16) {
    if (conv_bf16()) return launch_wgrad<Bf16Twin<Cfg>>(p, wp, slice_major, xf_side, s);
  }
  if (xf_side == 1) return launch_wgrad_x<Cfg, false, true>(p, wp, slice_major, s);
  if (xf_side == 2) return launch_wgrad_x<Cfg, true, false>(p, wp, slice_major, s);
  return launch_wgrad_x<Cfg, false, false>(p, wp, slice_major, s);
}

extern "C" int pcg_conv2d_wgrad_xf(const pcg_conv_geom* g, const float* x, const pcg_in_xform* xf_x, const float* dy,
                                   const pcg_in_xform* xf_dy, float* dw, int accumulate, void* workspace, size_t workspace_bytes,
                                   pcg_stream_t stream) {
  if (int e = check_geom(g)) return e;
  PCG_REQUIRE(x && dy && dw, "pcg_conv2d_wgrad: null pointer");
  const bool hx = xf_x && xf_x->scale, hy = xf_dy && xf_dy->scale;
  PCG_REQUIRE(!(hx && hy), "pcg_conv2d_wgrad_xf: at most one operand can carry an input transform");
  if (thin_is_cin(g) || thin_is_cout(g)) {
    PCG_REQUIRE(!hx && (!hy || thin_conv_xf_ok(g)), "pcg_conv2d_wgrad: input transforms on the MFMA path (Cin > 3 and Cout > 3) and, on the dy side, on the thin forms of pcg_conv2d_xf_thin_ok only");
    PCG_REQUIRE(!hy || (xf_dy->act == PCG_ACT_NONE || xf_dy->act == PCG_ACT_RELU || xf_dy->act == PCG_ACT_LRELU), "pcg_conv2d_wgrad: transform activation %d", hy ? xf_dy->act : 0);
    const ThinXf tx{hy ? xf_dy->scale : nullptr, hy ? xf_dy->shift : nullptr, hy ? act_neg_of(xf_dy->act, xf_dy->slope) : 1.f};
    return thin_conv_wgrad(g, x, dy, dw, accumulate, workspace, workspace_bytes, (hipStream_t)stream, &tx);
  }
  PCG_REQUIRE(g->Cin % 4 == 0 && g->Cout % 4 == 0, "pcg_conv2d_wgrad: Cin=%d and Cout=%d must be multiples of 4", g->Cin, g->Cout);
  const WgradPlan wp = plan_wgrad(g);
  const size_t need = pcg_conv2d_wgrad_workspace_bytes(g);
  if (workspace == nullptr || workspace_bytes < need) {
    set_error("pcg_conv2d_wgrad: workspace %zu B < required %zu B", workspace_bytes, need);
    return PCG_ERR_WORKSPACE;
  }
  PCG_REQUIRE(((uintptr_t)workspace & 15) == 0 && ((uintptr_t)dw & 15) == 0, "pcg_conv2d_wgrad: workspace/dw must be 16-byte aligned");
  ConvP p = make_params(g);
  p.x = x; p.dy = dy; p.out = (float*)workspace;
  p.M = g->Cout; p.N = g->KH * g->KW * g->Cin;
  p.tilesN = ceil_div(p.N, 128);
  p.pixtab = pixtab_of(g);
  if (int e = hx ? set_xform("pcg_conv2d_wgrad_xf", xf_x, g->Cin, &p) : set_xform("pcg_conv2d_wgrad_xf", xf_dy, g->Cout, &p)) return e;
  hipStream_t s = (hipStream_t)stream;
  static const int order_env0 = getenv("PCG_WGRAD_ORDER") ? atoi(getenv("PCG_WGRAD_ORDER")) : -1;
  const int order_env = g_tune.wgrad_order >= 0 ? g_tune.wgrad_order : order_env0;
  const int slice_major = order_env >= 0 ? order_env : (wp.tiles <= 8 ? 1 : 0);
  const int side = hx ? 1 : hy ? 2 : 0;
  if (!wp.narrow && !wp.wide192 && wp.tiles > 96 && sk_mode() != 0) {
    SkPlan sk{};
    bool take = plan_sk(wp.tiles, wp.ktiles_total, s, &sk);
    if (!take && wp.splits == 1) { sk = SkPlan{wp.tiles, 0, 0, wp.ktiles_total, nullptr, nullptr}; take = true; }
    if (take) {
      p.out = dw;
      if (accumulate) { p.epi.mode = EPI_ADD; p.epi.neg = 1.f; p.epi.delta_bytes = 0; }
      return side == 1 ? launch_wgrad_sk_x<Cfg128x128, false, true>(p, sk, s)
           : side == 2 ? launch_wgrad_sk_x<Cfg128x128, true, false>(p, sk, s) : launch_wgrad_sk_x<Cfg128x128, false, false>(p, sk, s);
    }
  }
  int rc;
  if (wp.wide192 && side == 0) {
    p.tilesN = p.N / 192;
    rc = conv_bf16() ? launch_wgrad192<Bf16Twin<Cfg64x192>>(p, wp, slice_major, s) : launch_wgrad192<Cfg64x192>(p, wp, slice_major, s);
  } else {
    WgradPlan wq = wp;
    if (wp.wide192) {
      wq.wide192 = false;
      wq.tiles = ceil_div(p.M, 64) * ceil_div(p.N, 128);
    }
    rc = wq.narrow ? launch_wgrad<TileCfg<64, 128, 1, 4>>(p, wq, slice_major, side, s) : launch_wgrad<Cfg128x128>(p, wq, slice_major, side, s);
  }
  if (rc != PCG_OK) return rc;
  const size_t n = (size_t)p.M * p.N;
  return launch_slab_reduce((const float*)workspace, dw, n, n, wp.splits, accumulate, s, true);
}

extern "C" int pcg_conv2d_wgrad(const pcg_conv_geom* g, const float* x, const float* dy, float* dw, int accumulate,
                                void* workspace, size_t workspace_bytes, pcg_stream_t stream) {
  return pcg_conv2d_wgrad_xf(g, x, nullptr, dy, nullptr, dw, accumulate, workspace, workspace_bytes, stream);
}

extern "C" int pcg_conv_plan_describe(const pcg_conv_geom* g, int32_t op, int32_t assume_scratch, char* out, size_t out_bytes) {
  if (int e = check_geom(g)) return e;
  PCG_REQUIRE(out && out_bytes > 0 && op >= 0 && op <= 2, "pcg_conv_plan_describe: bad arguments");
  const int have = assume_scratch ? (sk_mode() != 0 ? 1 : 0) : (have_sk_scratch() ? 1 : 0);
  char buf[512];
  buf[0] = 0;
  auto say = [&](const char* fmt, auto... a) { snprintf(buf + strlen(buf), sizeof(buf) - strlen(buf), fmt, a...); };
  if (thin_is_cin(g) || thin_is_cout(g)) {
    say("%s", "thin (Cin or Cout <= 3): no matrix-core launch");
  } else if (op == 0) {
    const int M = g->B * g->OH * g->OW, N = g->Cout, kt = g->KH * g->KW * ceil_div(g->Cin, IG_BK);
    const FwdPlan f = plan_fwd(g, have);
    SkPlan sk{};
    if (N <= 64) say("128x64 tiles: %d", ceil_div(M, 128));
    else if (fwd_use_t64(M, N, f.splits)) say("64x128 tiles: %d", ceil_div(M, 64) * ceil_div(N, 128));
    else if (f.splits == 1 && have && plan_sk_shape(ceil_div(M, 128) * ceil_div(N, 128), kt, &sk))
      say("stream-K: %d whole tiles + %d tiles x %d k-tiles over %d ranges", sk.dp_tiles, sk.sk_tiles, kt, sk.sk_blocks);
    else if (f.splits > 1) say("128x128 tiles: %d x %d K-slices of %d k-tiles (slabs)", ceil_div(M, 128) * ceil_div(N, 128), f.splits, f.ktiles_per_split);
    else say("128x128 tiles: %d", ceil_div(M, 128) * ceil_div(N, 128));
  } else if (op == 1) {
    if (dgrad_as_gemm(g, have)) {
      const int M = g->B * g->OH * g->OW, N = g->KH * g->KW * g->Cin, kt = ceil_div(g->Cout, IG_BK), tiles = ceil_div(M, 128) * ceil_div(N, 128);
      SkPlan sk{};
      say("%s", "GEMM + col2im: ");
      if (have && plan_sk_shape(tiles, kt, &sk)) say("stream-K: %d whole tiles + %d tiles x %d k-tiles over %d ranges", sk.dp_tiles, sk.sk_tiles, kt, sk.sk_blocks);
      else say("128x128 tiles: %d", tiles);
    } else {
      DgradPhases ph{};
      int maxMp = 0;
      const int nph = build_phases(g, &ph, &maxMp);
      const int N = g->Cin, tilesN = ceil_div(N, N > 64 ? 128 : 64);
      bool uniform = true;
      for (int i = 0; i < nph; ++i)
        uniform = uniform && ph.p[i].Mp == ph.p[0].Mp && ph.p[i].nth * ph.p[i].ntw == ph.p[0].nth * ph.p[0].ntw && ph.p[i].nth > 0 && ph.p[i].ntw > 0;
      SkNPlan sn{};
      SkPlan sk{};
      say("%d phase%s: ", nph, nph == 1 ? "" : "s");
      if (N > 64 && have && !uniform && plan_skn_shape(ph, nph, 128, tilesN, g->Cout, &sn))
        say("stream-K over unequal phases: %d tiles, %d k-tile iterations over %d ranges", sn.tile0[nph], sn.total, sn.blocks);
      else if (N > 64 && have && uniform && nph > 0 &&
               plan_sk_shape(ceil_div(maxMp, 128) * tilesN * nph, ph.p[0].nth * ph.p[0].ntw * ceil_div(g->Cout, IG_BK), &sk))
        say("stream-K: %d whole tiles + %d tiles over %d ranges", sk.dp_tiles, sk.sk_tiles, sk.sk_blocks);
      else say("%s tiles: %d per phase", N > 64 ? "128x128" : "128x64", ceil_div(maxMp, 128) * tilesN);
    }
  } else {
    const WgradPlan w = plan_wgrad(g);
    SkPlan sk{};
    if (!w.narrow && !w.wide192 && w.tiles > 96 && have && plan_sk_shape(w.tiles, w.ktiles_total, &sk))
      say("stream-K: %d whole tiles + %d tiles x %d k-tiles over %d ranges, dw written by the epilogue", sk.dp_tiles, sk.sk_tiles, w.ktiles_total, sk.sk_blocks);
    else if (!w.narrow && !w.wide192 && w.tiles > 96 && w.splits == 1 && sk_mode() != 0) say("128x128 tiles: %d, dw written by the epilogue", w.tiles);
    else say("%s tiles: %d x %d K-slices of %d k-tiles (slabs + slab_reduce)", w.wide192 ? "64x192" : w.narrow ? "64x128" : "128x128", w.tiles, w.splits, w.ktiles_per_split);
  }
  snprintf(out, out_bytes, "%s", buf);
  return PCG_OK;
}

extern "C" int pcg_tune_set(const char* name, int32_t value) {
  PCG_REQUIRE(name != nullptr, "pcg_tune_set: null name");
  if (!strcmp(name, "korder")) g_tune.korder = value;
  else if (!strcmp(name, "edge_prio")) g_tune.edge_prio = value;
  else if (!strcmp(name, "dgrad_swz3")) g_tune.dgrad_swz3 = value;
  else if (!strcmp(name, "wgrad_rounds")) g_tune.wgrad_rounds = value;
  else if (!strcmp(name, "wgrad_order")) g_tune.wgrad_order = value;
  else if (!strcmp(name, "dgrad_interleave")) g_tune.dgrad_interleave = value;
  else if (!strcmp(name, "fwd_splits")) g_tune.fwd_splits = value;
  else if (!strcmp(name, "stream_k")) g_tune.stream_k = value;
  else if (!strcmp(name, "sk_blocks")) g_tune.sk_blocks = value;
  else if (!strcmp(name, "dgrad_gemm")) g_tune.dgrad_gemm = value;
  else if (!strcmp(name, "t64")) g_tune.t64 = value;
  else if (!strcmp(name, "wgrad_pixtab")) g_tune.wgrad_pixtab = value;
  else {
    set_error("pcg_tune_set: unknown switch '%s' (korder, edge_prio, dgrad_swz3, wgrad_rounds, wgrad_order, dgrad_interleave, fwd_splits, "
              "stream_k, sk_blocks, dgrad_gemm, t64); the loader switch wgrad_pixtab is accepted as well", name);
    return PCG_ERR_INVALID;
  }
  return PCG_OK;
}

extern "C" int pcg_debug_stamp_buffer(void* buf, int64_t bytes) {
  g_tune.stamps = static_cast<unsigned long long*>(buf);
  g_tune.stamp_slots = buf ? (int)(bytes / 16) : 0;
#ifdef PCG_CLOCK_STAMP
  return 1;
#else
  return 0;
#endif
}
```

promptable-counterfactual-gan_amd/csrc/conv_loaders.h:

```cpp
#pragma once
#include "igemm_core.h"

namespace pcg {

__device__ __forceinline__ uint32_t tap_mask(int lo_h, int hi_h, int nh, int lo_w, int hi_w, int nw) {
  lo_h = lo_h < 0 ? 0 : lo_h; hi_h = hi_h > nh ? nh : hi_h;
  lo_w = lo_w < 0 ? 0 : lo_w; hi_w = hi_w > nw ? nw : hi_w;
  if (lo_h >= hi_h || lo_w >= hi_w) return 0u;
  const uint32_t rowbits = ((1u << (hi_w - lo_w)) - 1u) << lo_w;
  uint32_t m = 0;
  for (int a = lo_h; a < hi_h; ++a) m |= rowbits << (a * nw);
  return (hi_w - lo_w) >= 32 ? 0xFFFFFFFFu : m;
}

struct ConvP {
  const float* x;
  const float* w;
  const float* bias;
  float* out;
  const float* dy;
  double* stat_partial;
  int act; float slope;
  EpiAux epi;
  const float* in_sc; const float* in_sh; float in_neg; uint32_t in_c_bytes;
// ... 159 lines not shown
struct FwdBLoader {
  static constexpr bool KMAJOR = true, XFORM = false;
  static constexpr int ROWS = ROWS_, NV = ROWS_ / 32;
  rsrc_t rs;
  uint32_t base[NV];
  int Cin, KW, kq4;
  FwdKIter it;

  __device__ __forceinline__ FwdBLoader(const ConvP& p, int n_block, int tid) {
    rs = make_rsrc(p.w, p.w_bytes);
    Cin = p.Cin; KW = p.KW; kq4 = (tid & 7) * 4;
    it.init(p);
    const int r0 = tid >> 3;
    const int Ktot = p.KH * p.KW * p.Cin;
#pragma unroll
    for (int i = 0; i < NV; ++i) {
      const int n = n_block + r0 + 32 * i;
      base[i] = n < p.N ? (uint32_t)((n * Ktot + kq4) * 4) : OOB_OFF;
    }
  }
  __device__ __forceinline__ void seek(int kt) { it.seek(kt); }
  __device__ __forceinline__ void load_next(float4 (&v)[NV]) {
    const int ci0 = it.ci0;
    const uint32_t delta = (uint32_t)(((it.kh() * KW + it.kw()) * Cin + ci0) * 4);
    const bool kok = kq4 < Cin - ci0;
#pragma unroll
    for (int i = 0; i < NV; ++i) v[i] = buf_load4(rs, kok ? base[i] + delta : OOB_OFF);
    it.advance();
  }
  __device__ __forceinline__ void transform(float4 (&)[NV]) {}
};

struct DgradTapIter {
  int Cout, nth, ntw, jw, co0, jh, mode;
  __device__ __forceinline__ void init(int Cout_, int nth_, int ntw_, int mode_) {
    Cout = Cout_; nth = nth_; ntw = ntw_; mode = mode_; jh = 0; jw = 0; co0 = 0;
  }
  __device__ __forceinline__ void advance() {
    if (mode == 0) {
      co0 += IG_BK;
      if (co0 >= Cout) { co0 = 0; if (++jw == ntw) { jw = 0; ++jh; } }
    } else {
      if (++jw < ntw) return;
      jw = 0;
      if (++jh < nth) return;
      jh = 0;
      co0 += IG_BK;
    }
  }
  __device__ __forceinline__ void seek(int kt) {
    const int ntaps = nth * ntw;
    int tap;
    if (mode == 0) {
      const int nchunks = (Cout + IG_BK - 1) / IG_BK;
      tap = kt / nchunks;
      co0 = (kt - tap * nchunks) * IG_BK;
    } else {
      const int c = kt / ntaps;
      tap = kt - c * ntaps;
      co0 = c * IG_BK;
    }
    jh = tap / ntw; jw = tap - jh * ntw;
  }
};

template <int ROWS_, bool XF = false>
struct DgradALoader {
  static constexpr bool KMAJOR = true, XFORM = XF;
  static constexpr int ROWS = ROWS_, NV = ROWS_ / 32;
  rsrc_t rs;
  uint32_t base[NV], mask[NV];
  int OW, Cout, kq4;
  DgradTapIter it;
  XfK xf;

  __device__ __forceinline__ DgradALoader(const ConvP& p, const PhaseInfo& f, int m_block, int tid) {
    if constexpr (XF) xf.init(p);
    rs = make_rsrc(p.dy, p.dy_bytes);
    OW = p.OW; Cout = p.Cout;
    kq4 = (tid & 7) * 4;
    const int r0 = tid >> 3;
#pragma unroll
    for (int i = 0; i < NV; ++i) {
      const int m = m_block + r0 + 32 * i;
      uint32_t mk = 0, bs = OOB_OFF;
      if (m < f.Mp) {
        uint32_t t, cc, b, aa;
        f.dPHw.divmod((uint32_t)m, t, cc);
        f.dPHh.divmod(t, b, aa);
        const int oh0 = (int)aa + f.dh0, ow0 = (int)cc + f.dw0;
        bs = (uint32_t)(((((int)b * p.OH + oh0) * OW + ow0) * Cout + kq4) * 4);
        mk = tap_mask(oh0 - p.OH + 1, oh0 + 1, f.nth, ow0 - OW + 1, ow0 + 1, f.ntw);
      }
      base[i] = bs; mask[i] = mk;
    }
    it.init(Cout, f.nth, f.ntw, p.korder);
  }
  __device__ __forceinline__ void seek(int kt) { it.seek(kt); }
  __device__ __forceinline__ void load_next(float4 (&v)[NV]) {
    const int tap = it.jh * it.ntw + it.jw;
    const uint32_t delta = (uint32_t)((it.co0 - (it.jh * OW + it.jw) * Cout) * 4);
    const bool kok = kq4 < Cout - it.co0;
    uint32_t okbits = 0;
#pragma unroll
    for (int i = 0; i < NV; ++i) {
      const bool ok = kok && ((mask[i] >> tap) & 1u);
      v[i] = buf_load4(rs, ok ? base[i] + delta : OOB_OFF);
      if constexpr (XF) okbits |= (ok ? 1u : 0u) << i;
    }
    if constexpr (XF) { xf.ok = okbits; xf.fetch((uint32_t)((it.co0 + kq4) * 4), kok); }
    it.advance();
  }
  __device__ __forceinline__ void transform(float4 (&v)[NV]) {
    if constexpr (XF) {
#pragma unroll
      for (int i = 0; i < NV; ++i) v[i] = xf_apply(v[i], xf.sc, xf.sh, xf.neg, (xf.ok >> i) & 1u);
    }
  }
};

template <int ROWS_>
struct DgradBLoader {
  static constexpr bool KMAJOR = false, XFORM = false;
  static constexpr int ROWS = ROWS_, NV = ROWS_ / 32;
  static constexpr int C4 = ROWS_ / 4, KR = IG_LOADERS / C4;
  rsrc_t rs;
  uint32_t base[NV];
  int Cin, KHKW, KW, stride, kh0, kw0, kr0;
  DgradTapIter it;

  __device__ __forceinline__ DgradBLoader(const ConvP& p, const PhaseInfo& f, int n_block, int tid) {
    rs = make_rsrc(p.w, p.w_bytes);
    Cin = p.Cin; KHKW = p.KH * p.KW; KW = p.KW; stride = p.stride; kh0 = f.kh0; kw0 = f.kw0;
    const int c4 = tid % C4;
    kr0 = tid / C4;
    const int n = n_block + 4 * c4;
#pragma unroll
    for (int i = 0; i < NV; ++i)
      base[i] = n < p.N ? (uint32_t)(((mn_krow<NV>(kr0, i) * KHKW) * Cin + n) * 4) : OOB_OFF;
    it.init(p.Cout, f.nth, f.ntw, p.korder);
  }
  __device__ __forceinline__ void seek(int kt) { it.seek(kt); }
  __device__ __forceinline__ void load_next(float4 (&v)[NV]) {
    const int tap = (kh0 + stride * it.jh) * KW + kw0 + stride * it.jw;
    const uint32_t delta = (uint32_t)(((it.co0 * KHKW + tap) * Cin) * 4);
    const int krem = it.Cout - it.co0;
#pragma unroll
    for (int i = 0; i < NV; ++i) v[i] = buf_load4(rs, mn_krow<NV>(kr0, i) < krem ? base[i] + delta : OOB_OFF);
    it.advance();
  }
  __device__ __forceinline__ void transform(float4 (&)[NV]) {}
};

template <int ROWS_, bool XF = false>
struct WgradALoader {
  static constexpr bool KMAJOR = false, XFORM = XF;
  static constexpr int ROWS = ROWS_, NV = ROWS_ / 32;
  static constexpr int C4 = ROWS_ / 4, KR = IG_LOADERS / C4;
  rsrc_t rs;
  uint32_t base[NV];
  int Cout, K, q0, kr0;
  float4 sc, sh; float neg; uint32_t okb; bool mok;

  __device__ __forceinline__ WgradALoader(const ConvP& p, int m_block, int kt_begin, int tid) {
    rs = make_rsrc(p.dy, p.dy_bytes);
    Cout = p.Cout; K = p.B * p.OH * p.OW;
    const int c4 = tid % C4;
    kr0 = tid / C4;
    const int m = m_block + 4 * c4;
    mok = m < p.M;
#pragma unroll
    for (int i = 0; i < NV; ++i) base[i] = mok ? (uint32_t)((mn_krow<NV>(kr0, i) * Cout + m) * 4) : OOB_OFF;
    q0 = kt_begin * IG_BK;
    if constexpr (XF) {
      neg = p.in_neg; okb = 0;
      sc = mok ? *reinterpret_cast<const float4*>(p.in_sc + m) : make_float4(0.f, 0.f, 0.f, 0.f);
      sh = mok ? *reinterpret_cast<const float4*>(p.in_sh + m) : make_float4(0.f, 0.f, 0.f, 0.f);
    }
  }
  __device__ __forceinline__ void load_next(float4 (&v)[NV]) {
    const uint32_t delta = (uint32_t)(q0 * Cout * 4);
    const int krem = K - q0;
    uint32_t okbits = 0;
#pragma unroll
    for (int i = 0; i < NV; ++i) {
      const bool ok = mn_krow<NV>(kr0, i) < krem;
      v[i] = buf_load4(rs, ok ? base[i] + delta : OOB_OFF);
      if constexpr (XF) okbits |= ((ok && mok) ? 1u : 0u) << i;
    }
    if constexpr (XF) okb = okbits;
    q0 += IG_BK;
  }
  __device__ __forceinline__ void transform(float4 (&v)[NV]) {
    if constexpr (XF) {
#pragma unroll
      for (int i = 0; i < NV; ++i) v[i] = xf_apply(v[i], sc, sh, neg, (okb >> i) & 1u);
    }
  }
};

typedef uint32_t u32x16 __attribute__((ext_vector_type(16)));
typedef u32x16 u32x16_dw __attribute__((aligned(4)));
struct PixDesc8 {
  struct Tile {
    u32x16 d; uint32_t base; int qd, K;
    __device__ __forceinline__ uint32_t off(int j) const { return base + d[2 * j]; }
    __device__ __forceinline__ uint32_t mask(int j) const { return qd + j < K ? d[2 * j + 1] : 0u; }
  };
  const __attribute__((address_space(4))) uint32_t* tab;
  FastDiv dOHW;
  uint32_t img_bytes;
  Tile t;
  __device__ __forceinline__ void init(const ConvP& p) {
    tab = (const __attribute__((address_space(4))) uint32_t*)p.pixtab;
    dOHW = p.dOHW; img_bytes = (uint32_t)(p.IH * p.IW * p.Cin * 4); t.K = p.B * p.OH * p.OW;
  }
  __device__ __forceinline__ void fetch(int qw) {
    qw = __builtin_amdgcn_readfirstlane(qw);
    uint32_t img, r;
    dOHW.divmod((uint32_t)qw, img, r);
    t.base = img * img_bytes; t.qd = qw;
    t.d = *reinterpret_cast<const __attribute__((address_space(4))) u32x16_dw*>(tab + 2 * r);
  }
  __device__ __forceinline__ static void landed() { __builtin_amdgcn_s_waitcnt(0xC07F); }
};
__device__ __forceinline__ uint32_t pick4(uint32_t a, uint32_t b, uint32_t c, uint32_t d, bool g1, bool g2) {
  return g2 ? (g1 ? d : c) : (g1 ? b : a);
}
__device__ __forceinline__ void pick_desc4(const PixDesc8::Tile& pd, int h, bool g1, bool g2, uint32_t& off, uint32_t& mask) {
  off = pick4(pd.off(h), pd.off(2 + h), pd.off(4 + h), pd.off(6 + h), g1, g2);
  mask = pick4(pd.mask(h), pd.mask(2 + h), pd.mask(4 + h), pd.mask(6 + h), g1, g2);
}

template <int ROWS_, bool XF = false, bool TAB = false>
struct WgradBLoader {
  static constexpr bool KMAJOR = false, XFORM = XF;
  static constexpr int ROWS = ROWS_, NV = ROWS_ / 32;
  static constexpr int C4 = ROWS_ / 4, KR = IG_LOADERS / C4;
  static constexpr bool SCALAR_PIX = C4 == 32;
  rsrc_t rs;
  int IH, IW, Cin, stride, K, q0, kr0, OH, OW, dh, dw, ci;
  int lane_off;
  bool nok;
  FastDiv dOW, dOH;
  float4 sc, sh; float neg; uint32_t okb;
  static_assert(!TAB || SCALAR_PIX, "the table loader is written for 128-column tiles");
  PixDesc8 pd;
  int qw0;
  uint32_t tab_off;
  uint32_t himask, tb_lo, tb_hi;

  __device__ __forceinline__ WgradBLoader(const ConvP& p, int n_block, int kt_begin, int tid) {
    rs = make_rsrc(p.x, p.x_bytes);
    IH = p.IH; IW = p.IW; Cin = p.Cin; stride = p.stride; K = p.B * p.OH * p.OW;
    dOW = p.dOW; dOH = p.dOH;
    const int c4 = tid % C4;
    const int n = n_block + 4 * c4;
    nok = n < p.N;
    const int tap = nok ? n / Cin : 0;
    ci = nok ? n - tap * Cin : 0;
    const int kh = tap / p.KW, kw = tap - kh * p.KW;
    dh = kh - p.pad; dw = kw - p.pad;
    lane_off = ((dh * IW + dw) * Cin + ci) * 4;
    q0 = kt_begin * IG_BK; kr0 = tid / C4; OH = p.OH; OW = p.OW;
    if constexpr (TAB) {
      pd.init(p);
      himask = (tid & 32) ? 0xFFFFFFFFu : 0u;
      const uint32_t tapbit = nok ? 1u << tap : 0u;
      tab_off = (uint32_t)(((kh * IW + kw) * Cin + ci) * 4);
      qw0 = __builtin_amdgcn_readfirstlane(8 * (tid >> 6));
      tb_lo = tapbit & ~himask; tb_hi = tapbit & himask;
      pd.fetch(q0 + qw0);
      PixDesc8::landed();
    }
    if constexpr (XF) {
      neg = p.in_neg; okb = 0;
      sc = nok ? *reinterpret_cast<const float4*>(p.in_sc + ci) : make_float4(0.f, 0.f, 0.f, 0.f);
      sh = nok ? *reinterpret_cast<const float4*>(p.in_sh + ci) : make_float4(0.f, 0.f, 0.f, 0.f);
    }
  }
  __device__ __forceinline__ void load_next(float4 (&v)[NV]) {
    uint32_t okbits = 0;
    if constexpr (TAB) {
      const PixDesc8::Tile cur = pd.t;
      pd.fetch(q0 + IG_BK + qw0);
      __builtin_amdgcn_sched_barrier(0);
#pragma unroll
      for (int i = 0; i < NV; ++i) {
        const uint32_t off = cur.off(i) + tab_off + (himask & (cur.off(NV + i) - cur.off(i)));
        const bool ok = ((cur.mask(i) & tb_lo) | (cur.mask(NV + i) & tb_hi)) != 0u;
        v[i] = buf_load4(rs, ok ? off : OOB_OFF);
        if constexpr (XF) okbits |= (ok ? 1u : 0u) << i;
      }
      PixDesc8::landed();
    } else if constexpr (SCALAR_PIX) {
      const bool hi = (threadIdx.x & 32) != 0;
      const int qw = __builtin_amdgcn_readfirstlane(q0 + NV * (kr0 & ~1));
      uint32_t t, ow[2], b[2], oh[2];
#pragma unroll
      for (int h = 0; h < 2; ++h) {
        dOW.divmod((uint32_t)(qw + NV * h), t, ow[h]);
        dOH.divmod(t, b[h], oh[h]);
      }
#pragma unroll
      for (int i = 0; i < NV; ++i) {
        int pix[2], ihs[2], iws[2];
// ... 124 lines not shown
```

promptable-counterfactual-gan_amd/csrc/igemm_core.h:

```cpp
#pragma once
#include "pcg_common.h"

namespace pcg {

typedef float f32x16 __attribute__((ext_vector_type(16)));

typedef unsigned int u32x4 __attribute__((ext_vector_type(4)));
using rsrc_t = __amdgpu_buffer_rsrc_t;
constexpr uint32_t OOB_OFF = 0x80000000u;

__device__ __forceinline__ rsrc_t make_rsrc(const void* p, uint32_t bytes) {
  return __builtin_amdgcn_make_buffer_rsrc(const_cast<void*>(p), 0, bytes, 0x00020000);
}
__device__ __forceinline__ float4 buf_load4(rsrc_t r, uint32_t off) {
  const u32x4 v = __builtin_amdgcn_raw_buffer_load_b128(r, off, 0, 0);
  return make_float4(__uint_as_float(v.x), __uint_as_float(v.y), __uint_as_float(v.z), __uint_as_float(v.w));
}

constexpr int IG_LOADERS = 256;
constexpr int IG_THREADS = 512;
constexpr int IG_BK = 32;
#ifndef PCG_PREFETCH_DEPTH
#define PCG_PREFETCH_DEPTH 2
#endif
#ifndef PCG_CONSUMER_PRIO
#define PCG_CONSUMER_PRIO 2
#endif
#ifndef PCG_CONSUMER_ALTERNATE
#define PCG_CONSUMER_ALTERNATE 256
#endif
#ifndef PCG_PRODUCER_PRIO
#define PCG_PRODUCER_PRIO 3
#endif
constexpr int IG_LDK = IG_BK + 4;

template <int NV>
__device__ __forceinline__ constexpr int mn_krow(int kr0, int i) { return NV * kr0 + i; }

template <int BM_, int BN_, int WAVES_M_, int WAVES_N_, bool SWZ_ = false, int MINW_ = 4, int PF_ = PCG_PREFETCH_DEPTH, bool BF16_ = false>
struct TileCfg {
  static constexpr int BM = BM_, BN = BN_, WAVES_M = WAVES_M_, WAVES_N = WAVES_N_;
  static constexpr bool SWZ = SWZ_;
  static constexpr bool BF16 = BF16_;
  static constexpr int MINW = MINW_, PF = PF_;
  static constexpr int WTM = BM / WAVES_M, WTN = BN / WAVES_N;
  static constexpr int TM = WTM / 32, TN = WTN / 32;
  static_assert(WAVES_M * WAVES_N == 4, "4 consumer waves per block");
  static_assert(WTM % 32 == 0 && WTN % 32 == 0, "wave tile must be a multiple of the 32x32 MFMA tile");
};

typedef __bf16 bf16x8 __attribute__((ext_vector_type(8)));
typedef __bf16 bf16x2 __attribute__((ext_vector_type(2)));
constexpr int IG_LDB = IG_BK + 8;
__device__ __forceinline__ uint32_t pack_bf16x2(float lo, float hi) {
  const bf16x2 v = {(__bf16)lo, (__bf16)hi};
  return __builtin_bit_cast(uint32_t, v);
}

template <int ROWS, bool KMAJOR, bool SWZ = false, bool BF = false>
struct LdsImage;

template <int ROWS, bool KMAJOR, bool SWZ>
struct LdsImage<ROWS, KMAJOR, SWZ, true> {
  static constexpr int FLOATS = ROWS * IG_LDB / 2;
  static constexpr int NV = ROWS / 32;
  __device__ static __forceinline__ void store(float* lds, const float4 (&v)[NV], int tid) {
    char* base = reinterpret_cast<char*>(lds);
    if constexpr (KMAJOR) {
      const int kq = tid & 7, r0 = tid >> 3;
#pragma unroll
      for (int p = 0; p < NV; ++p)
        *reinterpret_cast<uint2*>(base + (r0 + 32 * p) * (2 * IG_LDB) + 8 * kq) = make_uint2(pack_bf16x2(v[p].x, v[p].y), pack_bf16x2(v[p].z, v[p].w));
    } else if constexpr (IG_LOADERS % (ROWS / 4) == 0) {
      constexpr int C4 = ROWS / 4;
      const int c4 = tid % C4, kr0 = tid / C4;
      static_assert((IG_LOADERS / C4) * NV == IG_BK && (NV == 2 || NV == 4), "bf16 MN-major image: 2 or 4 k-rows per loader thread");
      char* col = base + 4 * c4 * (2 * IG_LDB) + 2 * NV * kr0;
      if constexpr (NV == 4) {
        *reinterpret_cast<uint2*>(col) = make_uint2(pack_bf16x2(v[0].x, v[1].x), pack_bf16x2(v[2].x, v[3].x));
        *reinterpret_cast<uint2*>(col + 2 * IG_LDB) = make_uint2(pack_bf16x2(v[0].y, v[1].y), pack_bf16x2(v[2].y, v[3].y));
        *reinterpret_cast<uint2*>(col + 4 * IG_LDB) = make_uint2(pack_bf16x2(v[0].z, v[1].z), pack_bf16x2(v[2].z, v[3].z));
        *reinterpret_cast<uint2*>(col + 6 * IG_LDB) = make_uint2(pack_bf16x2(v[0].w, v[1].w), pack_bf16x2(v[2].w, v[3].w));
      } else {
        *reinterpret_cast<uint32_t*>(col) = pack_bf16x2(v[0].x, v[1].x);
        *reinterpret_cast<uint32_t*>(col + 2 * IG_LDB) = pack_bf16x2(v[0].y, v[1].y);
        *reinterpret_cast<uint32_t*>(col + 4 * IG_LDB) = pack_bf16x2(v[0].z, v[1].z);
        *reinterpret_cast<uint32_t*>(col + 6 * IG_LDB) = pack_bf16x2(v[0].w, v[1].w);
      }
    } else {
      static_assert(ROWS % 64 == 0, "bf16 MN-major image: ROWS must divide the loader threads or be a multiple of 64");
      const int c4 = tid & 15, kr0 = tid >> 4;
#pragma unroll
      for (int s = 0; s < ROWS / 64; ++s) {
        char* col = base + (64 * s + 4 * c4) * (2 * IG_LDB) + 4 * kr0;
        *reinterpret_cast<uint32_t*>(col) = pack_bf16x2(v[2 * s].x, v[2 * s + 1].x);
        *reinterpret_cast<uint32_t*>(col + 2 * IG_LDB) = pack_bf16x2(v[2 * s].y, v[2 * s + 1].y);
        *reinterpret_cast<uint32_t*>(col + 4 * IG_LDB) = pack_bf16x2(v[2 * s].z, v[2 * s + 1].z);
        *reinterpret_cast<uint32_t*>(col + 6 * IG_LDB) = pack_bf16x2(v[2 * s].w, v[2 * s + 1].w);
      }
    }
  }
  __device__ static __forceinline__ void frag(const float* lds, int row0, int ks, int li, int lh, bf16x8& f) {
    f = *reinterpret_cast<const bf16x8*>(reinterpret_cast<const char*>(lds) + (row0 + li) * (2 * IG_LDB) + 32 * ks + 16 * lh);
  }
};

template <int ROWS, bool KMAJOR, bool SWZ>
struct LdsImage<ROWS, KMAJOR, SWZ, false> {
  static constexpr int LDM = ROWS + 4;
  static constexpr int LDKS = (KMAJOR && SWZ) ? IG_BK : IG_LDK;
  static constexpr int FLOATS = KMAJOR ? ROWS * LDKS : IG_BK * LDM;
  static constexpr int NV = ROWS / 32;

  __device__ static __forceinline__ void store(float* lds, const float4 (&v)[NV], int tid) {
    if constexpr (KMAJOR && SWZ) {
      const int kq = tid & 7, r0 = tid >> 3;
#pragma unroll
      for (int p = 0; p < NV; ++p)
        *reinterpret_cast<float4*>(lds + (r0 + 32 * p) * IG_BK + 4 * (kq ^ ((r0 >> 1) & 7))) = v[p];
    } else if constexpr (KMAJOR) {
      const int kq = tid & 7, r0 = tid >> 3;
#pragma unroll
      for (int p = 0; p < NV; ++p)
        *reinterpret_cast<float4*>(lds + (r0 + 32 * p) * IG_LDK + 4 * kq) = v[p];
    } else if constexpr (IG_LOADERS % (ROWS / 4) == 0) {
      constexpr int C4 = ROWS / 4;
      constexpr int KR = IG_LOADERS / C4;
      const int c4 = tid % C4, kr0 = tid / C4;
      static_assert(KR * NV == IG_BK, "MN-major image: loader threads x loads must cover the k-tile");
#pragma unroll
      for (int p = 0; p < NV; ++p)
        *reinterpret_cast<float4*>(lds + mn_krow<NV>(kr0, p) * LDM + 4 * c4) = v[p];
    } else {
      static_assert(ROWS % 64 == 0, "MN-major image: ROWS must divide the loader threads or be a multiple of 64");
      const int c4 = tid & 15, kr0 = tid >> 4;
#pragma unroll
      for (int s = 0; s < ROWS / 64; ++s)
#pragma unroll
        for (int h = 0; h < 2; ++h)
          *reinterpret_cast<float4*>(lds + mn_krow<2>(kr0, h) * LDM + 64 * s + 4 * c4) = v[2 * s + h];
    }
  }
  __device__ static __forceinline__ void frag(const float* lds, int row0, int ks, int li, int lh, float (&f)[4]) {
    if constexpr (KMAJOR && SWZ) {
      const int row = row0 + li;
      const float4 q = *reinterpret_cast<const float4*>(lds + row * IG_BK + 4 * ((2 * ks + lh) ^ ((row >> 1) & 7)));
      f[0] = q.x; f[1] = q.y; f[2] = q.z; f[3] = q.w;
    } else if constexpr (KMAJOR) {
      const float4 q = *reinterpret_cast<const float4*>(lds + (row0 + li) * IG_LDK + 8 * ks + 4 * lh);
      f[0] = q.x; f[1] = q.y; f[2] = q.z; f[3] = q.w;
    } else {
      const float* p = lds + (8 * ks + 4 * lh) * LDM + row0 + li;
      f[0] = p[0]; f[1] = p[LDM]; f[2] = p[2 * LDM]; f[3] = p[3 * LDM];
    }
  }
};

__device__ __forceinline__ int acc_row(int r, int lh) { return (r & 3) + 8 * (r >> 2) + 4 * lh; }

__device__ __forceinline__ void lds_barrier() {
  asm volatile("s_waitcnt lgkmcnt(0)" ::: "memory");
  __builtin_amdgcn_s_barrier();
  asm volatile("" ::: "memory");
}

template <class Cfg, bool AK, bool BK_>
constexpr int igemm_smem_floats() {
  return 2 * (LdsImage<Cfg::BM, AK, Cfg::SWZ, Cfg::BF16>::FLOATS + LdsImage<Cfg::BN, BK_, Cfg::SWZ, Cfg::BF16>::FLOATS);
}

struct ClockStamp {
  unsigned long long* out; int slots;
#ifdef PCG_CLOCK_STAMP
  unsigned long long t0, r0;
  __device__ __forceinline__ void begin() { t0 = __builtin_amdgcn_s_memtime(); r0 = __builtin_amdgcn_s_memrealtime(); }
  __device__ __forceinline__ void end() {
    const unsigned long long t1 = __builtin_amdgcn_s_memtime(), r1 = __builtin_amdgcn_s_memrealtime();
    const int b = blockIdx.x + gridDim.x * blockIdx.y;
    if (out && threadIdx.x == 0 && b < slots) { out[2 * b] = t1 - t0; out[2 * b + 1] = r1 - r0; }
  }
  __device__ __forceinline__ void phase(int k) {
    const int b = blockIdx.x + gridDim.x * blockIdx.y;
    if (out && threadIdx.x == 0 && b < slots / 8) out[(size_t)slots + (size_t)b * 4 + k] = __builtin_amdgcn_s_memrealtime();
  }
  unsigned long long bar_acc, bar_t, sec_acc[3], sec_t;
  __device__ __forceinline__ void sec_begin() { sec_t = __builtin_amdgcn_s_memtime(); }
  __device__ __forceinline__ void sec_end(int k) { const unsigned long long t = __builtin_amdgcn_s_memtime(); sec_acc[k] += t - sec_t; sec_t = t; }
  __device__ __forceinline__ void bar_begin() { bar_t = __builtin_amdgcn_s_memtime(); }
  __device__ __forceinline__ void bar_end() { bar_acc += __builtin_amdgcn_s_memtime() - bar_t; }
  __device__ __forceinline__ void bar_init() { bar_acc = 0; sec_acc[0] = sec_acc[1] = sec_acc[2] = 0; }
  __device__ __forceinline__ void bar_flush(int who, unsigned long long loop_cycles) {
    const int b = blockIdx.x + gridDim.x * blockIdx.y;
    if (out && (threadIdx.x & 63) == 0 && b < slots / 8) {
      out[(size_t)slots + (size_t)slots / 2 + (size_t)b * 4 + 2 * who] = bar_acc;
      out[(size_t)slots + (size_t)slots / 2 + (size_t)b * 4 + 2 * who + 1] = loop_cycles;
      if (who == 1 && b < slots / 16) {
        out[(size_t)slots + (size_t)slots / 2 + (size_t)slots / 4 + (size_t)b * 2] = sec_acc[0] | (sec_acc[2] << 32);
        out[(size_t)slots + (size_t)slots / 2 + (size_t)slots / 4 + (size_t)b * 2 + 1] = sec_acc[1];
      }
    }
  }
#else
  __device__ __forceinline__ void begin() {}
  __device__ __forceinline__ void end() {}
  __device__ __forceinline__ void phase(int) {}
  __device__ __forceinline__ void bar_begin() {}
  __device__ __forceinline__ void bar_end() {}
  __device__ __forceinline__ void bar_init() {}
  __device__ __forceinline__ void bar_flush(int, unsigned long long) {}
  __device__ __forceinline__ void sec_begin() {}
  __device__ __forceinline__ void sec_end(int) {}
#endif
};

template <class Cfg, class LA, class LB>
__device__ __forceinline__ void igemm_produce(LA& la, LB& lb, int ktiles, float* smem, int tid, ClockStamp cs = ClockStamp{nullptr, 0}) {
  using IA = LdsImage<Cfg::BM, LA::KMAJOR, Cfg::SWZ, Cfg::BF16>;
  using IB = LdsImage<Cfg::BN, LB::KMAJOR, Cfg::SWZ, Cfg::BF16>;
  static_assert(LA::ROWS == Cfg::BM && LB::ROWS == Cfg::BN, "loader/tile mismatch");
  float* As = smem;
  float* Bs = smem + 2 * IA::FLOATS;
  if (PCG_PRODUCER_PRIO) __builtin_amdgcn_s_setprio(PCG_PRODUCER_PRIO);
  if constexpr (Cfg::PF == 2 && !LA::XFORM && !LB::XFORM) {
  float4 ra[2][IA::NV], rb[2][IB::NV];
  if (ktiles > 0) {
    la.load_next(ra[0]); lb.load_next(rb[0]);
    if (ktiles > 1) { la.load_next(ra[1]); lb.load_next(rb[1]); }
    la.transform(ra[0]); lb.transform(rb[0]);
    IA::store(As, ra[0], tid);
    IB::store(Bs, rb[0], tid);
    if (ktiles > 2) { la.load_next(ra[0]); lb.load_next(rb[0]); }
  }
  lds_barrier();
  cs.bar_init();
#ifdef PCG_CLOCK_STAMP
  const unsigned long long loop_t0 = __builtin_amdgcn_s_memtime();
#endif
  int kt = 0;
  for (; kt + 4 < ktiles; kt += 2) {
    cs.sec_begin();
#ifdef PCG_CLOCK_STAMP
    asm volatile("s_waitcnt vmcnt(8)" ::: "memory");
    cs.sec_end(2);
#endif
    IA::store(As + IA::FLOATS, ra[1], tid);
    IB::store(Bs + IB::FLOATS, rb[1], tid);
    cs.sec_end(0);
    la.load_next(ra[1]); lb.load_next(rb[1]);
    cs.sec_end(1);
    cs.bar_begin(); lds_barrier(); cs.bar_end();
    cs.sec_begin();
#ifdef PCG_CLOCK_STAMP
    asm volatile("s_waitcnt vmcnt(8)" ::: "memory");
    cs.sec_end(2);
#endif
    IA::store(As, ra[0], tid);
    IB::store(Bs, rb[0], tid);
    cs.sec_end(0);
    la.load_next(ra[0]); lb.load_next(rb[0]);
    cs.sec_end(1);
    cs.bar_begin(); lds_barrier(); cs.bar_end();
  }
  for (; kt + 1 < ktiles; kt += 2) {
    la.transform(ra[1]); lb.transform(rb[1]);
    IA::store(As + IA::FLOATS, ra[1], tid);
    IB::store(Bs + IB::FLOATS, rb[1], tid);
    if (kt + 3 < ktiles) { la.load_next(ra[1]); lb.load_next(rb[1]); }
    cs.bar_begin(); lds_barrier(); cs.bar_end();
    if (kt + 2 < ktiles) {
      la.transform(ra[0]); lb.transform(rb[0]);
      IA::store(As, ra[0], tid);
      IB::store(Bs, rb[0], tid);
    }
    if (kt + 4 < ktiles) { la.load_next(ra[0]); lb.load_next(rb[0]); }
    cs.bar_begin(); lds_barrier(); cs.bar_end();
  }
  if (kt < ktiles) lds_barrier();
#ifdef PCG_CLOCK_STAMP
  cs.bar_flush(1, __builtin_amdgcn_s_memtime() - loop_t0);
#endif
  } else {
  float4 ra[IA::NV], rb[IB::NV];
  if (ktiles > 0) {
    la.load_next(ra);
    lb.load_next(rb);
    la.transform(ra); lb.transform(rb);
    IA::store(As, ra, tid);
    IB::store(Bs, rb, tid);
    if (ktiles > 1) {
      la.load_next(ra);
      lb.load_next(rb);
    }
  }
  lds_barrier();
  int nxt = 1;
  for (int kt = 0; kt < ktiles; ++kt) {
#ifndef PCG_ABL_PRODUCER_IDLE
    if (kt + 1 < ktiles) {
      la.transform(ra); lb.transform(rb);
      IA::store(As + nxt * IA::FLOATS, ra, tid);
      IB::store(Bs + nxt * IB::FLOATS, rb, tid);
    }
    if (kt + 2 < ktiles) {
      la.load_next(ra);
      lb.load_next(rb);
    }
#endif
    lds_barrier();
    nxt ^= 1;
  }
  }
}

template <bool BF> struct MmaFrag { float v[4]; };
template <> struct MmaFrag<true> { bf16x8 v; };

template <class Cfg, bool AK, bool BK_>
__device__ __forceinline__ void igemm_consume(int ktiles, f32x16 (&acc)[Cfg::TM][Cfg::TN], const float* smem, ClockStamp cs = ClockStamp{nullptr, 0}) {
  using IA = LdsImage<Cfg::BM, AK, Cfg::SWZ, Cfg::BF16>;
  using IB = LdsImage<Cfg::BN, BK_, Cfg::SWZ, Cfg::BF16>;
  constexpr int KG = IG_BK / (Cfg::BF16 ? 16 : 8);
  const float* As = smem;
  const float* Bs = smem + 2 * IA::FLOATS;
  const int lane = threadIdx.x & 63, wave = threadIdx.x >> 6;
  const int wm = wave / Cfg::WAVES_N, wn = wave % Cfg::WAVES_N;
  const int li = lane & 31, lh = lane >> 5;
  const int arow = wm * Cfg::WTM, brow = wn * Cfg::WTN;
#pragma unroll
  for (int i = 0; i < Cfg::TM; ++i)
#pragma unroll
    for (int j = 0; j < Cfg::TN; ++j)
#pragma unroll
      for (int r = 0; r < 16; ++r) acc[i][j][r] = 0.f;

  MmaFrag<Cfg::BF16> a[2][Cfg::TM], b[2][Cfg::TN];
  auto fetch = [&](const float* as, const float* bs, int ks, int buf) {
#pragma unroll
    for (int i = 0; i < Cfg::TM; ++i) IA::frag(as, arow + 32 * i, ks, li, lh, a[buf][i].v);
#pragma unroll
    for (int j = 0; j < Cfg::TN; ++j) IB::frag(bs, brow + 32 * j, ks, li, lh, b[buf][j].v);
  };
  auto mma = [&](int buf) {
    if constexpr (Cfg::BF16) {
#pragma unroll
      for (int i = 0; i < Cfg::TM; ++i)
#pragma unroll
        for (int j = 0; j < Cfg::TN; ++j)
          acc[i][j] = __builtin_amdgcn_mfma_f32_32x32x16_bf16(a[buf][i].v, b[buf][j].v, acc[i][j], 0, 0, 0);
    } else {
#pragma unroll
      for (int t = 0; t < 4; ++t)
#pragma unroll
        for (int i = 0; i < Cfg::TM; ++i)
#pragma unroll
          for (int j = 0; j < Cfg::TN; ++j)
            acc[i][j] = __builtin_amdgcn_mfma_f32_32x32x2f32(a[buf][i].v[t], b[buf][j].v[t], acc[i][j], 0, 0, 0);
    }
  };

  lds_barrier();
  if (ktiles <= 0) return;
  __builtin_amdgcn_s_setprio(PCG_CONSUMER_PRIO);
  cs.begin(); cs.phase(1); cs.bar_init();
#ifdef PCG_CLOCK_STAMP
  const unsigned long long loop_t0 = __builtin_amdgcn_s_memtime();
#endif
  fetch(As, Bs, 0, 0);
  int cur = 0;
#if PCG_CONSUMER_ALTERNATE
  const int alt_phase = (int)((blockIdx.x / PCG_CONSUMER_ALTERNATE) & 1u);
#endif
  for (int kt = 0; kt < ktiles; ++kt) {
#if PCG_CONSUMER_ALTERNATE
    if ((kt + alt_phase) & 1) __builtin_amdgcn_s_setprio(2); else __builtin_amdgcn_s_setprio(1);
#endif
    const float* as = As + cur * IA::FLOATS;
    const float* bs = Bs + cur * IB::FLOATS;
#pragma unroll
    for (int ks = 0; ks < KG - 1; ++ks) {
      fetch(as, bs, ks + 1, (ks + 1) & 1);
      mma(ks & 1);
    }
    cs.bar_begin();
    lds_barrier();
    cs.bar_end();
    cur ^= 1;
    if (kt + 1 < ktiles) fetch(As + cur * IA::FLOATS, Bs + cur * IB::FLOATS, 0, KG & 1);
    mma((KG - 1) & 1);
  }
  cs.end(); cs.phase(2);
#ifdef PCG_CLOCK_STAMP
  cs.bar_flush(0, __builtin_amdgcn_s_memtime() - loop_t0);
#endif
  __builtin_amdgcn_s_setprio(0);
}

template <class Cfg>
constexpr int epilogue_smem_floats() { return 4 * Cfg::WTM * (Cfg::WTN + 4); }

enum { EPI_NONE = 0, EPI_MASK = 1, EPI_BNBWD = 2, EPI_ADD = 3, EPI_ADDSUM = 4 };
struct EpiAux {
  int mode;
  float neg;
  int64_t delta_bytes;
  int64_t delta2_bytes;
  const float* mean; const float* invstd; const float* gamma; const float* beta;
  int no_addend;
  int group_rows;
};

__device__ __forceinline__ void epi_store4(float* p, float4 v) { *reinterpret_cast<float4*>(p) = v; }

template <class Cfg, class RowBase>
__device__ __forceinline__ void igemm_store_tile(f32x16 (&acc)[Cfg::TM][Cfg::TN], float* smem, int n_block, int N,
                                                 const float* bias, RowBase row_base, double* stat_row = nullptr, int act = PCG_ACT_NONE,
                                                 float slope = 0.f, const EpiAux* epi = nullptr, int stat_goff = 0) {
  constexpr int LDW = Cfg::WTN + 4;
  constexpr int Q = Cfg::WTN / 4;
  constexpr int RPI = 64 / Q;
  static_assert(Cfg::WTM % RPI == 0, "wave tile rows must be a multiple of the rows stored per instruction");
  const int lane = threadIdx.x & 63, wave = threadIdx.x >> 6;
  const int wm = wave / Cfg::WAVES_N, wn = wave % Cfg::WAVES_N, li = lane & 31, lh = lane >> 5;
  float* reg = smem + wave * (Cfg::WTM * LDW);
#pragma unroll
  for (int i = 0; i < Cfg::TM; ++i)
#pragma unroll
    for (int j = 0; j < Cfg::TN; ++j)
#pragma unroll
      for (int r = 0; r < 16; ++r) reg[(32 * i + acc_row(r, lh)) * LDW + 32 * j + li] = acc[i][j][r];
  asm volatile("s_waitcnt lgkmcnt(0)" ::: "memory");
  const int cq = lane % Q, r0 = lane / Q;
  const int n = n_block + wn * Cfg::WTN + 4 * cq;
  const bool nok = n < N && r0 < RPI;
  float4 bv = make_float4(0.f, 0.f, 0.f, 0.f);
  if (bias && nok) bv = *reinterpret_cast<const float4*>(bias + n);
  double s1[4] = {0.0, 0.0, 0.0, 0.0}, s2[4] = {0.0, 0.0, 0.0, 0.0};
  const bool want_sums = stat_row != nullptr;
  const int emode = epi ? epi->mode : EPI_NONE;
  if (emode == EPI_NONE) {
#pragma unroll
    for (int k = 0; k < Cfg::WTM / RPI; ++k) {
      const int row = r0 + RPI * k;
      float* dst = row_base(wm * Cfg::WTM + row);
      if (dst && nok) {
        float4 v = *reinterpret_cast<const float4*>(reg + row * LDW + 4 * cq);
        v.x += bv.x; v.y += bv.y; v.z += bv.z; v.w += bv.w;
        if (act != PCG_ACT_NONE) {
          v.x = act_neg_scale(v.x, slope); v.y = act_neg_scale(v.y, slope); v.z = act_neg_scale(v.z, slope); v.w = act_neg_scale(v.w, slope);
        }
        epi_store4(dst + wn * Cfg::WTN + 4 * cq, v);
        if (want_sums) {
          const double d0 = v.x, d1 = v.y, d2 = v.z, d3 = v.w;
          s1[0] += d0; s1[1] += d1; s1[2] += d2; s1[3] += d3;
          s2[0] = fma(d0, d0, s2[0]); s2[1] = fma(d1, d1, s2[1]); s2[2] = fma(d2, d2, s2[2]); s2[3] = fma(d3, d3, s2[3]);
        }
      }
    }
  } else {
    const float neg = epi->neg;
    const int64_t delta = epi->delta_bytes;
    float4 sc = make_float4(1.f, 1.f, 1.f, 1.f), sh = make_float4(0.f, 0.f, 0.f, 0.f), mu = sh, is = sc;
    if (emode == EPI_BNBWD && nok) {
      mu = *reinterpret_cast<const float4*>(epi->mean + stat_goff + n);
      is = *reinterpret_cast<const float4*>(epi->invstd + stat_goff + n);
      const float4 ga = *reinterpret_cast<const float4*>(epi->gamma + n), be = *reinterpret_cast<const float4*>(epi->beta + n);
// ... 83 lines not shown
```

Measured before the change: 51520.

## Drive implicit-GEMM producer K iteration from a precomputed tap/chunk list

Adds a host-built K-iteration list (KList) holding per-step A/B address deltas and validity bits for forward and dgrad convolutions. Producer waves walk it through a KSched instead of doing per-step index arithmetic in the loaders, and use scalar-offset buffer loads when there is no K tail. It is on by default through PCG_KITER_LIST and covers the plain, stream-K and skn kernel variants. The aim is to cut address-generation ALU work on the producer side, at the cost of an extra list load from memory each step, a waitcnt in the gather, and a host-side list build on every launch.

```diff
diff --git a/include/pcgan_hip.h b/include/pcgan_hip.h
--- a/include/pcgan_hip.h
+++ b/include/pcgan_hip.h
@@ -584,6 +584,9 @@
 int pcg_conv_reset_scratch(pcg_stream_t stream);
 size_t pcg_conv_pixtab_bytes(const pcg_conv_geom* g);
 int pcg_conv_pixtab_register(const pcg_conv_geom* g, void* host_out, size_t bytes, const void* device_table);
+int pcg_conv_kiter_export(const pcg_conv_geom* g, int32_t op, int32_t korder, int32_t phase, uint32_t* out, size_t out_bytes,
+                          int32_t* n_taps, int32_t* n_chunks);
+int pcg_conv_kiter_walk(const pcg_conv_geom* g, int32_t op, int32_t korder, int32_t phase, int32_t kt_begin, int32_t n_steps, int32_t* out);
 int pcg_debug_stamp_buffer(void* buf, int64_t bytes);
 
 typedef struct pcg_moons_cf_desc {
diff --git a/promptable-counterfactual-gan_amd/_lib.py b/promptable-counterfactual-gan_amd/_lib.py
--- a/promptable-counterfactual-gan_amd/_lib.py
+++ b/promptable-counterfactual-gan_amd/_lib.py
@@ -221,6 +221,8 @@
     "pcg_conv_reset_scratch": (_i, [_vp]),
     "pcg_conv_pixtab_bytes": (_sz, [_gp]),
     "pcg_conv_pixtab_register": (_i, [_gp, _vp, _sz, _vp]),
+    "pcg_conv_kiter_export": (_i, [_gp, _i32, _i32, _i32, _vp, _sz, _vp, _vp]),
+    "pcg_conv_kiter_walk": (_i, [_gp, _i32, _i32, _i32, _i32, _i32, _vp]),
     "pcg_conv2d_fwd_bn_g": (_i, [_gp, _vp, _vp, _vp, _vp, _f, _f, _vp, _vp, _vp, _vp, _vp, _i32, _vp, _sz, _vp]),
     "pcg_bn_apply_act_g": (_i, [_vp, _i64, _i32, _vp, _vp, _vp, _vp, _i, _f, _vp, _i32, _vp]),
     "pcg_conv2d_dgrad_bn_phases": (_i32, [_gp]),
diff --git a/promptable-counterfactual-gan_amd/csrc/conv_igemm.hip b/promptable-counterfactual-gan_amd/csrc/conv_igemm.hip
--- a/promptable-counterfactual-gan_amd/csrc/conv_igemm.hip
+++ b/promptable-counterfactual-gan_amd/csrc/conv_igemm.hip
@@ -16,8 +16,27 @@
   return p.epi.group_rows > 0 ? __builtin_amdgcn_readfirstlane(m_block / p.epi.group_rows) * p.N : 0;
 }
 
-template <class Cfg, bool XF>
-__global__ void __launch_bounds__(IG_THREADS, Cfg::MINW) conv_fwd_kernel(ConvP p) {
+template <class Cfg, bool XF, bool KTAIL>
+__device__ __forceinline__ void fwd_produce_k(const ConvP& p, const KList& L, int m_block, int n_block, int kt_begin, int ktiles, float* smem,
+                                              int tid, ClockStamp cs) {
+  FwdALoaderK<Cfg::BM, XF, KTAIL> la(p, m_block, tid);
+  FwdBLoaderK<Cfg::BN, KTAIL> lb(p, n_block, tid);
+  KSched ks;
+  ks.init(L, 0, kt_begin);
+  igemm_produce<Cfg>(la, lb, ktiles, smem, tid, cs, ks);
+}
+template <class Cfg, bool XF, bool KTAIL>
+__device__ __forceinline__ void dgrad_produce_k(const ConvP& p, const PhaseInfo& f, const KList& L, int py, int m_block, int n_block, int kt_begin,
+                                                int ktiles, float* smem, int tid, ClockStamp cs) {
+  DgradALoaderK<Cfg::BM, XF, KTAIL> la(p, f, m_block, tid);
+  DgradBLoaderK<Cfg::BN, KTAIL> lb(p, f, n_block, tid);
+  KSched ks;
+  ks.init(L, py, kt_begin);
+  igemm_produce<Cfg>(la, lb, ktiles, smem, tid, cs, ks);
+}
+
+template <class Cfg, bool XF, bool KL = false>
+__global__ void __launch_bounds__(IG_THREADS, Cfg::MINW) conv_fwd_kernel(ConvP p, KArg<KL> ka) {
   extern __shared__ __attribute__((aligned(16))) float smem[];
   prio_entry(p);
   const uint32_t tile = xcd_remap(blockIdx.x, gridDim.x);
@@ -29,10 +48,15 @@
 
   if (wave_id() >= 4) {
     const int tid = threadIdx.x - IG_LOADERS;
+    if constexpr (KL) {
+      if (ka.L.ktail) fwd_produce_k<Cfg, XF, true>(p, ka.L, m_block, n_block, kt_begin, ktiles, smem, tid, ClockStamp{p.stamps, p.stamp_slots});
+      else fwd_produce_k<Cfg, XF, false>(p, ka.L, m_block, n_block, kt_begin, ktiles, smem, tid, ClockStamp{p.stamps, p.stamp_slots});
+    } else {
     FwdALoader<Cfg::BM, XF> la(p, m_block, tid);
     FwdBLoader<Cfg::BN> lb(p, n_block, tid);
     if (kt_begin) { la.seek(kt_begin); lb.seek(kt_begin); }
     igemm_produce<Cfg>(la, lb, ktiles, smem, tid, ClockStamp{p.stamps, p.stamp_slots});
+    }
     return;
   }
   f32x16 acc[Cfg::TM][Cfg::TN];
@@ -52,8 +76,8 @@
   cs.phase(3);
 }
 
-template <class Cfg, bool XF>
-__global__ void __launch_bounds__(IG_THREADS, Cfg::MINW) conv_dgrad_kernel(ConvP p, DgradPhases phases) {
+template <class Cfg, bool XF, bool KL = false>
+__global__ void __launch_bounds__(IG_THREADS, Cfg::MINW) conv_dgrad_kernel(ConvP p, DgradPhases phases, KArg<KL> ka) {
   extern __shared__ __attribute__((aligned(16))) float smem[];
   __shared__ int rowpix[Cfg::BM];
   prio_entry(p);
@@ -84,9 +108,14 @@
       }
       rowpix[r] = pix;
     }
+    if constexpr (KL) {
+      if (ka.L.ktail) dgrad_produce_k<Cfg, XF, true>(p, f, ka.L, (int)py, m_block, n_block, 0, ktiles, smem, tid, ClockStamp{p.stamps, p.stamp_slots});
+      else dgrad_produce_k<Cfg, XF, false>(p, f, ka.L, (int)py, m_block, n_block, 0, ktiles, smem, tid, ClockStamp{p.stamps, p.stamp_slots});
+    } else {
     DgradALoader<Cfg::BM, XF> la(p, f, m_block, tid);
     DgradBLoader<Cfg::BN> lb(p, f, n_block, tid);
     igemm_produce<Cfg>(la, lb, ktiles, smem, tid, ClockStamp{p.stamps, p.stamp_slots});
+    }
     return;
   }
   f32x16 acc[Cfg::TM][Cfg::TN];
@@ -191,16 +220,20 @@
                               [&](int blk) { return sk_start(blk, sk) >= j * KT; }, acc);
 }
 
-template <class Cfg, bool XF>
-__device__ __forceinline__ void fwd_sk_segment(const ConvP& p, const SkPlan& sk, const SkSeg& sg, float* smem) {
+template <class Cfg, bool XF, bool KL>
+__device__ __forceinline__ void fwd_sk_segment(const ConvP& p, const SkPlan& sk, const SkSeg& sg, float* smem, const KArg<KL>& ka) {
   const int mt = __builtin_amdgcn_readfirstlane(sg.tile / p.tilesN), nt = sg.tile - mt * p.tilesN;
   const int m_block = mt * Cfg::BM, n_block = nt * Cfg::BN;
   if (wave_id() >= 4) {
     const int tid = threadIdx.x - IG_LOADERS;
+    if constexpr (KL) {
+      fwd_produce_k<Cfg, XF, true>(p, ka.L, m_block, n_block, sg.kt_begin, sg.nkt, smem, tid, ClockStamp{nullptr, 0});
+    } else {
     FwdALoader<Cfg::BM, XF> la(p, m_block, tid);
     FwdBLoader<Cfg::BN> lb(p, n_block, tid);
     if (sg.kt_begin) { la.seek(sg.kt_begin); lb.seek(sg.kt_begin); }
     igemm_produce<Cfg>(la, lb, sg.nkt, smem, tid, ClockStamp{nullptr, 0});
+    }
     return;
   }
   f32x16 acc[Cfg::TM][Cfg::TN];
@@ -211,20 +244,20 @@
       return m < p.M ? p.out + (size_t)m * p.N + n_block : nullptr;
     }, p.stat_partial ? p.stat_partial + (size_t)mt * Cfg::WAVES_M * 2 * p.N : nullptr, p.act, p.slope, &p.epi, epi_group_off(p, m_block));
 }
-template <class Cfg, bool XF>
-__global__ void __launch_bounds__(IG_THREADS, Cfg::MINW) conv_fwd_sk_kernel(ConvP p, SkPlan sk) {
+template <class Cfg, bool XF, bool KL = false>
+__global__ void __launch_bounds__(IG_THREADS, Cfg::MINW) conv_fwd_sk_kernel(ConvP p, SkPlan sk, KArg<KL> ka) {
   extern __shared__ __attribute__((aligned(16))) float smem[];
   SkSeg s0, s1{};
   const int nseg = sk_segments(sk, s0, s1);
-  fwd_sk_segment<Cfg, XF>(p, sk, s0, smem);
+  fwd_sk_segment<Cfg, XF, KL>(p, sk, s0, smem, ka);
   if (nseg == 1) return;
   lds_barrier();
-  fwd_sk_segment<Cfg, XF>(p, sk, s1, smem);
-}
-
-template <class Cfg, bool XF>
+  fwd_sk_segment<Cfg, XF, KL>(p, sk, s1, smem, ka);
+}
+
+template <class Cfg, bool XF, bool KL>
 __device__ __forceinline__ void dgrad_sk_segment(const ConvP& p, const DgradPhases& phases, const SkPlan& sk, const SkSeg& sg, int tiles_per_phase,
-                                                 float* smem, int* rowpix) {
+                                                 float* smem, int* rowpix, const KArg<KL>& ka) {
   const int py = __builtin_amdgcn_readfirstlane(sg.tile / tiles_per_phase), tile = sg.tile - py * tiles_per_phase;
   const PhaseInfo& f = phases.p[py];
   const int mt = __builtin_amdgcn_readfirstlane(tile / p.tilesN), nt = tile - mt * p.tilesN;
@@ -242,10 +275,14 @@
       }
       rowpix[r] = pix;
     }
+    if constexpr (KL) {
+      dgrad_produce_k<Cfg, XF, true>(p, f, ka.L, py, m_block, n_block, sg.kt_begin, sg.nkt, smem, tid, ClockStamp{nullptr, 0});
+    } else {
     DgradALoader<Cfg::BM, XF> la(p, f, m_block, tid);
     DgradBLoader<Cfg::BN> lb(p, f, n_block, tid);
     if (sg.kt_begin) { la.seek(sg.kt_begin); lb.seek(sg.kt_begin); }
     igemm_produce<Cfg>(la, lb, sg.nkt, smem, tid, ClockStamp{nullptr, 0});
+    }
     return;
   }
   f32x16 acc[Cfg::TM][Cfg::TN];
@@ -256,16 +293,16 @@
       return pix >= 0 ? p.out + (size_t)pix * p.Cin + n_block : nullptr;
     }, p.stat_partial ? p.stat_partial + (size_t)(f.prow0 + mt * Cfg::WAVES_M) * 2 * p.N : nullptr, p.act, p.slope, &p.epi, epi_group_off(p, m_block));
 }
-template <class Cfg, bool XF>
-__global__ void __launch_bounds__(IG_THREADS, Cfg::MINW) conv_dgrad_sk_kernel(ConvP p, DgradPhases phases, SkPlan sk, int tiles_per_phase) {
+template <class Cfg, bool XF, bool KL = false>
+__global__ void __launch_bounds__(IG_THREADS, Cfg::MINW) conv_dgrad_sk_kernel(ConvP p, DgradPhases phases, SkPlan sk, int tiles_per_phase, KArg<KL> ka) {
   extern __shared__ __attribute__((aligned(16))) float smem[];
   __shared__ int rowpix[Cfg::BM];
   SkSeg s0, s1{};
   const int nseg = sk_segments(sk, s0, s1);
-  dgrad_sk_segment<Cfg, XF>(p, phases, sk, s0, tiles_per_phase, smem, rowpix);
+  dgrad_sk_segment<Cfg, XF, KL>(p, phases, sk, s0, tiles_per_phase, smem, rowpix, ka);
   if (nseg == 1) return;
   lds_barrier();
-  dgrad_sk_segment<Cfg, XF>(p, phases, sk, s1, tiles_per_phase, smem, rowpix);
+  dgrad_sk_segment<Cfg, XF, KL>(p, phases, sk, s1, tiles_per_phase, smem, rowpix, ka);
 }
 
 template <class Cfg, bool XFA, bool XFB, bool TAB = false>
@@ -332,8 +369,8 @@
   s.mt = __builtin_amdgcn_readfirstlane(s.tin / tilesN); s.nt = s.tin - s.mt * tilesN;
   return s;
 }
-template <class Cfg, bool XF>
-__global__ void __launch_bounds__(IG_THREADS, Cfg::MINW) conv_dgrad_skn_kernel(ConvP p, DgradPhases phases, SkNPlan sk) {
+template <class Cfg, bool XF, bool KL = false>
+__global__ void __launch_bounds__(IG_THREADS, Cfg::MINW) conv_dgrad_skn_kernel(ConvP p, DgradPhases phases, SkNPlan sk, KArg<KL> ka) {
   extern __shared__ __attribute__((aligned(16))) float smem[];
   __shared__ int rowpix[Cfg::BM];
   const int g = (int)xcd_remap(blockIdx.x, (uint32_t)sk.blocks);
@@ -356,10 +393,14 @@
         }
         rowpix[r] = pix;
       }
+      if constexpr (KL) {
+        dgrad_produce_k<Cfg, XF, true>(p, f, ka.L, sg.py, m_block, n_block, sg.kt_begin, sg.nkt, smem, tid, ClockStamp{nullptr, 0});
+      } else {
       DgradALoader<Cfg::BM, XF> la(p, f, m_block, tid);
       DgradBLoader<Cfg::BN> lb(p, f, n_block, tid);
       if (sg.kt_begin) { la.seek(sg.kt_begin); lb.seek(sg.kt_begin); }
       igemm_produce<Cfg>(la, lb, sg.nkt, smem, tid, ClockStamp{nullptr, 0});
+      }
       it = sg.e;
       if (it < it1) lds_barrier();
     }
@@ -512,7 +553,7 @@
   return PCG_OK;
 }
 
-struct Tune { int edge_prio = -1, dgrad_swz3 = -1, wgrad_rounds = -1, korder = -1, wgrad_order = -1, dgrad_interleave = -1, fwd_splits = -1, stream_k = -1, sk_blocks = -1, dgrad_gemm = -1, t64 = -1, wgrad_pixtab = -1; unsigned long long* stamps = nullptr; int stamp_slots = 0; };
+struct Tune { int edge_prio = -1, dgrad_swz3 = -1, wgrad_rounds = -1, korder = -1, wgrad_order = -1, dgrad_interleave = -1, fwd_splits = -1, stream_k = -1, sk_blocks = -1, dgrad_gemm = -1, t64 = -1, wgrad_pixtab = -1, kiter_list = -1; unsigned long long* stamps = nullptr; int stamp_slots = 0; };
 Tune g_tune;
 
 ConvP make_params(const pcg_conv_geom* g) {
@@ -594,6 +635,10 @@
     if (pixtab_same(g_pixtab[i], dev, g)) return g_pixtab[i].tab;
   return nullptr;
 }
+bool kiter_on() {
+  static const int env = getenv("PCG_KITER_LIST") ? atoi(getenv("PCG_KITER_LIST")) : 1;
+  return (g_tune.kiter_list >= 0 ? g_tune.kiter_list : env) != 0;
+}
 int sk_mode() {
   static const int env = getenv("PCG_STREAM_K") ? atoi(getenv("PCG_STREAM_K")) : 1;
   return g_tune.stream_k >= 0 ? g_tune.stream_k : env;
@@ -634,23 +679,28 @@
 }
 int stream_has_sk(hipStream_t s) { return sk_mode() != 0 && sk_scratch_of(s, nullptr) ? 1 : 0; }
 
-template <class Cfg, bool XF>
+template <class Cfg, bool XF, bool KL = false>
 int launch_fwd_x(ConvP p, int splits, hipStream_t s) {
+  if constexpr (!KL) {
+    if (kiter_on()) return launch_fwd_x<Cfg, XF, true>(p, splits, s);
+  }
+  KArg<KL> ka{};
+  if constexpr (KL) klist_build_fwd(p.KH, p.KW, p.IW, p.Cin, p.stride, p.korder, &ka.L);
   p.tilesN = ceil_div(p.N, Cfg::BN);
   const int tilesM = ceil_div(p.M, Cfg::BM);
   constexpr size_t smem = smem_bytes<Cfg, true, true>();
   if constexpr (Cfg::BM == 128 && Cfg::BN == 128) {
     SkPlan sk{};
     if (splits == 1 && plan_sk(tilesM * p.tilesN, p.ktiles, s, &sk)) {
-      static int once_sk = set_smem(conv_fwd_sk_kernel<Cfg, XF>, smem);
+      static int once_sk = set_smem(conv_fwd_sk_kernel<Cfg, XF, KL>, smem);
       if (once_sk != PCG_OK) return once_sk;
-      hipLaunchKernelGGL((conv_fwd_sk_kernel<Cfg, XF>), dim3((unsigned)(sk.dp_tiles + sk.sk_blocks)), dim3(IG_THREADS), smem, s, p, sk);
+      hipLaunchKernelGGL((conv_fwd_sk_kernel<Cfg, XF, KL>), dim3((unsigned)(sk.dp_tiles + sk.sk_blocks)), dim3(IG_THREADS), smem, s, p, sk, ka);
       return launch_status("conv_fwd_sk_kernel");
     }
   }
-  static int once = set_smem(conv_fwd_kernel<Cfg, XF>, smem);
+  static int once = set_smem(conv_fwd_kernel<Cfg, XF, KL>, smem);
   if (once != PCG_OK) return once;
-  hipLaunchKernelGGL((conv_fwd_kernel<Cfg, XF>), dim3((unsigned)tilesM * p.tilesN, splits), dim3(IG_THREADS), smem, s, p);
+  hipLaunchKernelGGL((conv_fwd_kernel<Cfg, XF, KL>), dim3((unsigned)tilesM * p.tilesN, splits), dim3(IG_THREADS), smem, s, p, ka);
   return launch_status("conv_fwd_kernel");
 }
 template <class Cfg>
@@ -712,8 +762,13 @@
   return ok;
 }
 
-template <class Cfg, bool XF>
+template <class Cfg, bool XF, bool KL = false>
 int launch_dgrad_x(ConvP p, const DgradPhases& ph, int nphases, int maxMp, hipStream_t s) {
+  if constexpr (!KL) {
+    if (kiter_on()) return launch_dgrad_x<Cfg, XF, true>(p, ph, nphases, maxMp, s);
+  }
+  KArg<KL> ka{};
+  if constexpr (KL) klist_build_dgrad(ph, nphases, p.OW, p.Cout, p.Cin, p.KH, p.KW, p.stride, p.korder, &ka.L);
   p.tilesN = ceil_div(p.N, Cfg::BN);
   const int tilesM = ceil_div(maxMp, Cfg::BM);
   constexpr size_t smem = smem_bytes<Cfg, true, false>();
@@ -726,26 +781,26 @@
       SkPlan scratch{};
       if (plan_skn_shape(ph, nphases, Cfg::BM, p.tilesN, p.Cout, &sn) && sk_scratch_of(s, &scratch)) {
         sn.parts = scratch.parts; sn.arrivals = scratch.arrivals;
-        static int once_sn = set_smem(conv_dgrad_skn_kernel<Cfg, XF>, smem);
+        static int once_sn = set_smem(conv_dgrad_skn_kernel<Cfg, XF, KL>, smem);
         if (once_sn != PCG_OK) return once_sn;
         DgradPhases phs = ph;
         phs.interleave = 0;
-        hipLaunchKernelGGL((conv_dgrad_skn_kernel<Cfg, XF>), dim3((unsigned)sn.blocks), dim3(IG_THREADS), smem, s, p, phs, sn);
+        hipLaunchKernelGGL((conv_dgrad_skn_kernel<Cfg, XF, KL>), dim3((unsigned)sn.blocks), dim3(IG_THREADS), smem, s, p, phs, sn, ka);
         return launch_status("conv_dgrad_skn_kernel");
       }
     }
     SkPlan sk{};
     const int tpp = tilesM * p.tilesN;
     if (uniform && plan_sk(tpp * nphases, ph.p[0].nth * ph.p[0].ntw * ceil_div(p.Cout, IG_BK), s, &sk)) {
-      static int once_sk = set_smem(conv_dgrad_sk_kernel<Cfg, XF>, smem);
+      static int once_sk = set_smem(conv_dgrad_sk_kernel<Cfg, XF, KL>, smem);
       if (once_sk != PCG_OK) return once_sk;
       DgradPhases phs = ph;
       phs.interleave = 0;
-      hipLaunchKernelGGL((conv_dgrad_sk_kernel<Cfg, XF>), dim3((unsigned)(sk.dp_tiles + sk.sk_blocks)), dim3(IG_THREADS), smem, s, p, phs, sk, tpp);
+      hipLaunchKernelGGL((conv_dgrad_sk_kernel<Cfg, XF, KL>), dim3((unsigned)(sk.dp_tiles + sk.sk_blocks)), dim3(IG_THREADS), smem, s, p, phs, sk, tpp, ka);
       return launch_status("conv_dgrad_sk_kernel");
     }
   }
-  static int once = set_smem(conv_dgrad_kernel<Cfg, XF>, smem);
+  static int once = set_smem(conv_dgrad_kernel<Cfg, XF, KL>, smem);
   if (once != PCG_OK) return once;
   static const int il_env0 = getenv("PCG_DGRAD_INTERLEAVE") ? atoi(getenv("PCG_DGRAD_INTERLEAVE")) : 1;
   const int il_env = g_tune.dgrad_interleave >= 0 ? g_tune.dgrad_interleave : il_env0;
@@ -754,9 +809,9 @@
   for (int i = 1; i < nphases; ++i) same = same && ph.p[i].Mp == ph.p[0].Mp;
   phl.interleave = same ? nphases : 0;
   if (same)
-    hipLaunchKernelGGL((conv_dgrad_kernel<Cfg, XF>), dim3((unsigned)tilesM * p.tilesN * nphases), dim3(IG_THREADS), smem, s, p, phl);
+    hipLaunchKernelGGL((conv_dgrad_kernel<Cfg, XF, KL>), dim3((unsigned)tilesM * p.tilesN * nphases), dim3(IG_THREADS), smem, s, p, phl, ka);
   else
-    hipLaunchKernelGGL((conv_dgrad_kernel<Cfg, XF>), dim3((unsigned)tilesM * p.tilesN, nphases), dim3(IG_THREADS), smem, s, p, phl);
+    hipLaunchKernelGGL((conv_dgrad_kernel<Cfg, XF, KL>), dim3((unsigned)tilesM * p.tilesN, nphases), dim3(IG_THREADS), smem, s, p, phl, ka);
   return launch_status("conv_dgrad_kernel");
 }
 template <class Cfg>
@@ -1590,6 +1645,51 @@
   return PCG_OK;
 }
 
+static int kiter_list_of(const char* who, const pcg_conv_geom* g, int32_t op, int32_t korder, int32_t phase, KList* L) {
+  if (int e = check_geom(g)) return e;
+  PCG_REQUIRE((op == 0 || op == 1) && (korder == 0 || korder == 1), "%s: op %d / korder %d", who, op, korder);
+  if (op == 0) {
+    PCG_REQUIRE(phase == 0, "%s: a forward launch has one phase", who);
+    klist_build_fwd(g->KH, g->KW, g->IW, g->Cin, g->stride, korder, L);
+    return PCG_OK;
+  }
+  PCG_REQUIRE(g->stride <= 2, "%s: grad-input stride %d > 2 unsupported", who, g->stride);
+  DgradPhases ph{};
+  int maxMp = 0;
+  const int nph = build_phases(g, &ph, &maxMp);
+  PCG_REQUIRE(phase >= 0 && phase < nph, "%s: phase %d of %d", who, phase, nph);
+  klist_build_dgrad(ph, nph, g->OW, g->Cout, g->Cin, g->KH, g->KW, g->stride, korder, L);
+  return PCG_OK;
+}
+extern "C" int pcg_conv_kiter_export(const pcg_conv_geom* g, int32_t op, int32_t korder, int32_t phase, uint32_t* out, size_t out_bytes,
+                                     int32_t* n_taps, int32_t* n_chunks) {
+  KList L;
+  if (int e = kiter_list_of("pcg_conv_kiter_export", g, op, korder, phase, &L)) return e;
+  const int n = L.n[phase], f = L.first[phase];
+  PCG_REQUIRE(out && out_bytes >= (size_t)n * 16, "pcg_conv_kiter_export: buffer %zu B (need %zu)", out_bytes, (size_t)n * 16);
+  for (int i = 0; i < n; ++i) {
+    const KTap& t = L.e[f + i];
+    out[4 * i] = t.a_delta; out[4 * i + 1] = t.b_delta; out[4 * i + 2] = t.bit; out[4 * i + 3] = t.meta - (uint32_t)f;
+  }
+  if (n_taps) *n_taps = n;
+  if (n_chunks) *n_chunks = L.nchunks;
+  return PCG_OK;
+}
+extern "C" int pcg_conv_kiter_walk(const pcg_conv_geom* g, int32_t op, int32_t korder, int32_t phase, int32_t kt_begin, int32_t n_steps,
+                                   int32_t* out) {
+  KList L;
+  if (int e = kiter_list_of("pcg_conv_kiter_walk", g, op, korder, phase, &L)) return e;
+  PCG_REQUIRE(out && kt_begin >= 0 && n_steps >= 0 && kt_begin + n_steps <= L.n[phase] * L.nchunks, "pcg_conv_kiter_walk: k-tiles [%d, %d) of %d",
+              kt_begin, kt_begin + n_steps, L.n[phase] * L.nchunks);
+  KCursor c;
+  c.seek(L, phase, kt_begin);
+  for (int i = 0; i < n_steps; ++i) {
+    out[2 * i] = c.idx - L.first[phase]; out[2 * i + 1] = c.chunk;
+    c.advance(L.e[c.idx].meta, L.nchunks);
+  }
+  return PCG_OK;
+}
+
 extern "C" int pcg_tune_set(const char* name, int32_t value) {
   PCG_REQUIRE(name != nullptr, "pcg_tune_set: null name");
   if (!strcmp(name, "korder")) g_tune.korder = value;
@@ -1604,9 +1704,10 @@
   else if (!strcmp(name, "dgrad_gemm")) g_tune.dgrad_gemm = value;
   else if (!strcmp(name, "t64")) g_tune.t64 = value;
   else if (!strcmp(name, "wgrad_pixtab")) g_tune.wgrad_pixtab = value;
+  else if (!strcmp(name, "kiter_list")) g_tune.kiter_list = value;
   else {
     set_error("pcg_tune_set: unknown switch '%s' (korder, edge_prio, dgrad_swz3, wgrad_rounds, wgrad_order, dgrad_interleave, fwd_splits, "
-              "stream_k, sk_blocks, dgrad_gemm, t64); the loader switch wgrad_pixtab is accepted as well", name);
+              "stream_k, sk_blocks, dgrad_gemm, t64); the loader switches wgrad_pixtab and kiter_list are accepted as well", name);
     return PCG_ERR_INVALID;
   }
   return PCG_OK;
diff --git a/promptable-counterfactual-gan_amd/csrc/conv_loaders.h b/promptable-counterfactual-gan_amd/csrc/conv_loaders.h
--- a/promptable-counterfactual-gan_amd/csrc/conv_loaders.h
+++ b/promptable-counterfactual-gan_amd/csrc/conv_loaders.h
@@ -335,6 +335,195 @@
   __device__ __forceinline__ void transform(float4 (&)[NV]) {}
 };
 
+struct KTap {
+  uint32_t a_delta;
+  uint32_t b_delta;
+  uint32_t bit;
+  uint32_t meta;
+};
+constexpr int KLIST_MAX = 32;
+struct KList {
+  KTap e[KLIST_MAX];
+  int first[4], n[4];
+  int nchunks;
+  uint32_t b_chunk;
+  int unit;
+  int ktail;
+};
+template <bool KL> struct KArg { };
+template <> struct KArg<true> { KList L; };
+
+#define PCG_HD __host__ __device__ __forceinline__
+PCG_HD uint32_t ktap_meta(int gfirst, int gcount, bool last) { return (uint32_t)gfirst | (uint32_t)gcount << 8 | (last ? 1u << 16 : 0u); }
+struct KCursor {
+  int idx, chunk;
+  PCG_HD void seek(const KList& L, int ph, int kt) {
+    int i = L.first[ph];
+    const int end = i + L.n[ph];
+    idx = i; chunk = 0;
+    if (L.n[ph] <= 0) return;
+    if (L.unit) {
+      const int t = kt / L.nchunks;
+      idx = i + t; chunk = kt - t * L.nchunks;
+      return;
+    }
+    for (;;) {
+      const int cnt = (int)((L.e[i].meta >> 8) & 255u), in_group = cnt * L.nchunks;
+      if (kt < in_group || i + cnt >= end) {
+        const int c = kt / cnt;
+        idx = i + (kt - c * cnt); chunk = c;
+        return;
+      }
+      kt -= in_group; i += cnt;
+    }
+  }
+  PCG_HD void advance(uint32_t meta, int nchunks) {
+    const bool last = (meta >> 16) & 1u;
+    const bool more = chunk + 1 < nchunks;
+    const int gfirst = (int)(meta & 255u);
+    idx = (last && more) ? gfirst : idx + 1;
+    chunk = last ? (more ? chunk + 1 : 0) : chunk;
+  }
+};
+
+inline void klist_build_fwd(int KH, int KW, int IW, int Cin, int stride, int korder, KList* L) {
+  *L = KList{};
+  const int S = korder ? stride : 1;
+  int n = 0;
+  for (int ch = 0; ch < S && ch < KH; ++ch)
+    for (int cw = 0; cw < S && cw < KW; ++cw) {
+      const int g0 = n;
+      for (int kh = ch; kh < KH; kh += S)
+        for (int kw = cw; kw < KW; kw += S, ++n) {
+          L->e[n].a_delta = (uint32_t)(((kh * IW + kw) * Cin) * 4);
+          L->e[n].b_delta = (uint32_t)(((kh * KW + kw) * Cin) * 4);
+          L->e[n].bit = 1u << (kh * KW + kw);
+        }
+      if (korder) for (int t = g0; t < n; ++t) L->e[t].meta = ktap_meta(g0, n - g0, t == n - 1);
+      else        for (int t = g0; t < n; ++t) L->e[t].meta = ktap_meta(t, 1, true);
+    }
+  L->first[0] = 0; L->n[0] = n;
+  L->nchunks = (Cin + IG_BK - 1) / IG_BK; L->b_chunk = IG_BK * 4;
+  L->unit = korder ? 0 : 1; L->ktail = Cin % IG_BK != 0;
+}
+inline void klist_build_dgrad(const DgradPhases& ph, int nphases, int OW, int Cout, int Cin, int KH, int KW, int stride, int korder, KList* L) {
+  *L = KList{};
+  int n = 0;
+  for (int p = 0; p < nphases && p < 4; ++p) {
+    const PhaseInfo& f = ph.p[p];
+    const int g0 = n;
+    for (int jh = 0; jh < f.nth; ++jh)
+      for (int jw = 0; jw < f.ntw; ++jw, ++n) {
+        L->e[n].a_delta = (uint32_t)(-((jh * OW + jw) * Cout) * 4);
+        L->e[n].b_delta = (uint32_t)((((f.kh0 + stride * jh) * KW + f.kw0 + stride * jw) * Cin) * 4);
+        L->e[n].bit = 1u << (jh * f.ntw + jw);
+      }
+    for (int t = g0; t < n; ++t) L->e[t].meta = korder ? ktap_meta(g0, n - g0, t == n - 1) : ktap_meta(t, 1, true);
+    L->first[p] = g0; L->n[p] = n - g0;
+  }
+  L->nchunks = (Cout + IG_BK - 1) / IG_BK; L->b_chunk = (uint32_t)(IG_BK * KH * KW * Cin * 4);
+  L->unit = korder ? 0 : 1; L->ktail = Cout % IG_BK != 0;
+}
+
+struct KStep { uint32_t a, b, bit; int chunk; };
+struct KSched {
+  static constexpr bool ACTIVE = true;
+  const KList* L;
+  KTap nxt;
+  KCursor c;
+  int nchunks; uint32_t b_chunk;
+  __device__ __forceinline__ void init(const KList& L_, int ph, int kt) {
+    L = &L_; nchunks = L_.nchunks; b_chunk = L_.b_chunk;
+    c.seek(L_, ph, __builtin_amdgcn_readfirstlane(kt));
+    c.idx = __builtin_amdgcn_readfirstlane(c.idx); c.chunk = __builtin_amdgcn_readfirstlane(c.chunk);
+    nxt = L->e[c.idx];
+    landed();
+  }
+  __device__ __forceinline__ KStep take() {
+    const KStep s{nxt.a_delta + (uint32_t)c.chunk * (uint32_t)(IG_BK * 4), nxt.b_delta + (uint32_t)c.chunk * b_chunk, nxt.bit, c.chunk};
+    c.advance(nxt.meta, nchunks);
+    nxt = L->e[c.idx];
+    __builtin_amdgcn_sched_barrier(0);
+    return s;
+  }
+  __device__ __forceinline__ static void landed() { __builtin_amdgcn_s_waitcnt(0xC07F); }
+};
+
+template <int ROWS_, bool XF, bool KTAIL>
+struct FwdALoaderK : FwdALoader<ROWS_, XF> {
+  using P = FwdALoader<ROWS_, XF>;
+  static constexpr int NV = P::NV;
+  using P::P;
+  using P::load_next;
+  __device__ __forceinline__ void load_next(float4 (&v)[NV], const KStep& s) {
+    bool kok = true;
+    uint32_t bit = s.bit;
+    if constexpr (KTAIL) { kok = this->kq4 < this->Cin - IG_BK * s.chunk; bit = kok ? bit : 0u; }
+    uint32_t okbits = 0;
+#pragma unroll
+    for (int i = 0; i < NV; ++i) {
+      const bool ok = (this->mask[i] & bit) != 0u;
+      v[i] = buf_load4(this->rs, ok ? this->base[i] + s.a : OOB_OFF);
+      if constexpr (XF) okbits |= (ok ? 1u : 0u) << i;
+    }
+    if constexpr (XF) { this->xf.ok = okbits; this->xf.fetch((uint32_t)((IG_BK * s.chunk + this->kq4) * 4), kok); }
+  }
+};
+template <int ROWS_, bool KTAIL>
+struct FwdBLoaderK : FwdBLoader<ROWS_> {
+  using P = FwdBLoader<ROWS_>;
+  static constexpr int NV = P::NV;
+  using P::P;
+  using P::load_next;
+  __device__ __forceinline__ void load_next(float4 (&v)[NV], const KStep& s) {
+    if constexpr (KTAIL) {
+      const bool kok = this->kq4 < this->Cin - IG_BK * s.chunk;
+#pragma unroll
+      for (int i = 0; i < NV; ++i) v[i] = buf_load4(this->rs, kok ? this->base[i] + s.b : OOB_OFF);
+    } else {
+#pragma unroll
+      for (int i = 0; i < NV; ++i) v[i] = buf_load4_so(this->rs, this->base[i], s.b);
+    }
+  }
+};
+template <int ROWS_, bool XF, bool KTAIL>
+struct DgradALoaderK : DgradALoader<ROWS_, XF> {
+  using P = DgradALoader<ROWS_, XF>;
+  static constexpr int NV = P::NV;
+  using P::P;
+  using P::load_next;
+  __device__ __forceinline__ void load_next(float4 (&v)[NV], const KStep& s) {
+    bool kok = true;
+    uint32_t bit = s.bit;
+    if constexpr (KTAIL) { kok = this->kq4 < this->Cout - IG_BK * s.chunk; bit = kok ? bit : 0u; }
+    uint32_t okbits = 0;
+#pragma unroll
+    for (int i = 0; i < NV; ++i) {
+      const bool ok = (this->mask[i] & bit) != 0u;
+      v[i] = buf_load4(this->rs, ok ? this->base[i] + s.a : OOB_OFF);
+      if constexpr (XF) okbits |= (ok ? 1u : 0u) << i;
+    }
+    if constexpr (XF) { this->xf.ok = okbits; this->xf.fetch((uint32_t)((IG_BK * s.chunk + this->kq4) * 4), kok); }
+  }
+};
+template <int ROWS_, bool KTAIL>
+struct DgradBLoaderK : DgradBLoader<ROWS_> {
+  using P = DgradBLoader<ROWS_>;
+  static constexpr int NV = P::NV;
+  using P::P;
+  using P::load_next;
+  __device__ __forceinline__ void load_next(float4 (&v)[NV], const KStep& s) {
+    if constexpr (KTAIL) {
+      const int krem = this->it.Cout - IG_BK * s.chunk;
+#pragma unroll
+      for (int i = 0; i < NV; ++i) v[i] = buf_load4(this->rs, mn_krow<NV>(this->kr0, i) < krem ? this->base[i] + s.b : OOB_OFF);
+    } else {
+#pragma unroll
+      for (int i = 0; i < NV; ++i) v[i] = buf_load4_so(this->rs, this->base[i], s.b);
+    }
+  }
+};
+
 template <int ROWS_, bool XF = false>
 struct WgradALoader {
   static constexpr bool KMAJOR = false, XFORM = XF;
diff --git a/promptable-counterfactual-gan_amd/csrc/igemm_core.h b/promptable-counterfactual-gan_amd/csrc/igemm_core.h
--- a/promptable-counterfactual-gan_amd/csrc/igemm_core.h
+++ b/promptable-counterfactual-gan_amd/csrc/igemm_core.h
@@ -14,6 +14,11 @@
 }
 __device__ __forceinline__ float4 buf_load4(rsrc_t r, uint32_t off) {
   const u32x4 v = __builtin_amdgcn_raw_buffer_load_b128(r, off, 0, 0);
+  return make_float4(__uint_as_float(v.x), __uint_as_float(v.y), __uint_as_float(v.z), __uint_as_float(v.w));
+}
+
+__device__ __forceinline__ float4 buf_load4_so(rsrc_t r, uint32_t voff, uint32_t soff) {
+  const u32x4 v = __builtin_amdgcn_raw_buffer_load_b128(r, voff, soff, 0);
   return make_float4(__uint_as_float(v.x), __uint_as_float(v.y), __uint_as_float(v.z), __uint_as_float(v.w));
 }
 
@@ -213,23 +218,34 @@
 #endif
 };
 
-template <class Cfg, class LA, class LB>
-__device__ __forceinline__ void igemm_produce(LA& la, LB& lb, int ktiles, float* smem, int tid, ClockStamp cs = ClockStamp{nullptr, 0}) {
+struct NoKSched { static constexpr bool ACTIVE = false; };
+template <class Cfg, class LA, class LB, class KS = NoKSched>
+__device__ __forceinline__ void igemm_produce(LA& la, LB& lb, int ktiles, float* smem, int tid, ClockStamp cs = ClockStamp{nullptr, 0}, KS ks = KS{}) {
   using IA = LdsImage<Cfg::BM, LA::KMAJOR, Cfg::SWZ, Cfg::BF16>;
   using IB = LdsImage<Cfg::BN, LB::KMAJOR, Cfg::SWZ, Cfg::BF16>;
   static_assert(LA::ROWS == Cfg::BM && LB::ROWS == Cfg::BN, "loader/tile mismatch");
   float* As = smem;
   float* Bs = smem + 2 * IA::FLOATS;
+#define IG_GATHER(a, b)                                                  \
+  do {                                                                   \
+    if constexpr (KS::ACTIVE) {                                          \
+      const auto st = ks.take();                                         \
+      la.load_next(a, st); lb.load_next(b, st);                          \
+      KS::landed();                                                      \
+    } else {                                                             \
+      la.load_next(a); lb.load_next(b);                                  \
+    }                                                                    \
+  } while (0)
   if (PCG_PRODUCER_PRIO) __builtin_amdgcn_s_setprio(PCG_PRODUCER_PRIO);
   if constexpr (Cfg::PF == 2 && !LA::XFORM && !LB::XFORM) {
   float4 ra[2][IA::NV], rb[2][IB::NV];
   if (ktiles > 0) {
-    la.load_next(ra[0]); lb.load_next(rb[0]);
-    if (ktiles > 1) { la.load_next(ra[1]); lb.load_next(rb[1]); }
+    IG_GATHER(ra[0], rb[0]);
+    if (ktiles > 1) { IG_GATHER(ra[1], rb[1]); }
     la.transform(ra[0]); lb.transform(rb[0]);
     IA::store(As, ra[0], tid);
     IB::store(Bs, rb[0], tid);
-    if (ktiles > 2) { la.load_next(ra[0]); lb.load_next(rb[0]); }
+    if (ktiles > 2) { IG_GATHER(ra[0], rb[0]); }
   }
   lds_barrier();
   cs.bar_init();
@@ -246,7 +262,7 @@
     IA::store(As + IA::FLOATS, ra[1], tid);
     IB::store(Bs + IB::FLOATS, rb[1], tid);
     cs.sec_end(0);
-    la.load_next(ra[1]); lb.load_next(rb[1]);
+    IG_GATHER(ra[1], rb[1]);
     cs.sec_end(1);
     cs.bar_begin(); lds_barrier(); cs.bar_end();
     cs.sec_begin();
@@ -257,7 +273,7 @@
     IA::store(As, ra[0], tid);
     IB::store(Bs, rb[0], tid);
     cs.sec_end(0);
-    la.load_next(ra[0]); lb.load_next(rb[0]);
+    IG_GATHER(ra[0], rb[0]);
     cs.sec_end(1);
     cs.bar_begin(); lds_barrier(); cs.bar_end();
   }
@@ -265,14 +281,14 @@
     la.transform(ra[1]); lb.transform(rb[1]);
     IA::store(As + IA::FLOATS, ra[1], tid);
     IB::store(Bs + IB::FLOATS, rb[1], tid);
-    if (kt + 3 < ktiles) { la.load_next(ra[1]); lb.load_next(rb[1]); }
+    if (kt + 3 < ktiles) { IG_GATHER(ra[1], rb[1]); }
     cs.bar_begin(); lds_barrier(); cs.bar_end();
     if (kt + 2 < ktiles) {
       la.transform(ra[0]); lb.transform(rb[0]);
       IA::store(As, ra[0], tid);
       IB::store(Bs, rb[0], tid);
     }
-    if (kt + 4 < ktiles) { la.load_next(ra[0]); lb.load_next(rb[0]); }
+    if (kt + 4 < ktiles) { IG_GATHER(ra[0], rb[0]); }
     cs.bar_begin(); lds_barrier(); cs.bar_end();
   }
   if (kt < ktiles) lds_barrier();
@@ -282,14 +298,12 @@
   } else {
   float4 ra[IA::NV], rb[IB::NV];
   if (ktiles > 0) {
-    la.load_next(ra);
-    lb.load_next(rb);
+    IG_GATHER(ra, rb);
     la.transform(ra); lb.transform(rb);
     IA::store(As, ra, tid);
     IB::store(Bs, rb, tid);
     if (ktiles > 1) {
-      la.load_next(ra);
-      lb.load_next(rb);
+      IG_GATHER(ra, rb);
     }
   }
   lds_barrier();
@@ -302,8 +316,7 @@
       IB::store(Bs + nxt * IB::FLOATS, rb, tid);
     }
     if (kt + 2 < ktiles) {
-      la.load_next(ra);
-      lb.load_next(rb);
+      IG_GATHER(ra, rb);
     }
 #endif
     lds_barrier();
@@ -311,6 +324,8 @@
   }
   }
 }
+
+#undef IG_GATHER
 
 template <bool BF> struct MmaFrag { float v[4]; };
 template <> struct MmaFrag<true> { bf16x8 v; };
```

Result: no change. 51680 (median of 6 runs) (+0.3%).
